# atakan-topaloglu/stable-virtual-camera

Hardware: AMD Instinct MI355X
Metric: denoising steps/sec, 1.3B Seva @ 21x576x576 views (higher is better)
Workload: dtype f16; 1 GPU; Seva 1.3B (1,263,968,004 params, random-init), one 21-view window per GPU, 576x576 px (latent 72x72), CFG batch 42, Euler-EDM step, MultiviewCFG(1.2) cfg 2.0; novel_views_per_sec = value x (T - 1 input view) / 50 steps per window; views=21, latent=72, windows=1

## Files before the change

include/seva_hip.h:

```cpp
#ifndef SEVA_HIP_H
#define SEVA_HIP_H

#include <stdint.h>

#ifdef __cplusplus
extern "C" {
#endif

typedef void* seva_stream_t;

#define SEVA_OK 0
#define SEVA_ERR_ARG (-1)
#define SEVA_ERR_LAUNCH (-2)
#define SEVA_ERR_UNSUPPORTED (-3)

const char* seva_last_error(void);
const char* seva_last_plan(void);
#define SEVA_ABI_VERSION 12
int seva_abi_version(void);
const char* seva_target_arch(void);

#define SEVA_CH_STATS_ROWS 64
#define SEVA_SPLITK_FLAGS 16384
#define SEVA_SPLITK_ERROR_SLOT 16383
#define SEVA_SPLITK_TILE_M 128
#define SEVA_SPLITK_TILE_N 160
#define SEVA_SPLITK_MAX_PIXELS 128
typedef struct seva_gemm_desc {
  const void* a;
  const void* w;
  const float* bias;
  const float* row_add;
  const float* residual;
  float* out_f32;
  void* out_f16;
  int64_t M, N, K;
  int64_t lda, ldr, ldo32, ldo16;
  int64_t rows_per_group;
  int64_t ld_row_add;
  int32_t mode;
  int32_t epilogue;
  int32_t n, ih, iw, cin, oh, ow, stride, upsample;
  float col_scale;
  int32_t col_scale_n;
  int32_t pad_br_only;
  const void* w_exp;
  void* out_f8;
  int64_t ldo8;
  float* ch_stats;
  float* splitk_ws;
  int64_t splitk_ws_bytes;
  const void* a2;
  int64_t lda2;
  int64_t K2;
  int64_t alg_K;
} seva_gemm_desc;
int seva_gemm_f16(const seva_gemm_desc* d, seva_stream_t stream);
int seva_gemm_f16_split_out(const seva_gemm_desc* d, seva_stream_t stream);
int seva_gemm_fp8(const seva_gemm_desc* d, seva_stream_t stream);

typedef struct seva_ff_desc {
  const void* a;
  const void* w1;
  const float* b1;
  const void* w2;
  const float* b2;
  const float* residual;
  float* out_f32;
  void* out_f16;
  int64_t M, lda, ldr, ldo32, ldo16;
  int32_t C;
  const float* ln_x;
  const float* ln_gamma;
  const float* ln_beta;
  int64_t ldx;
  float ln_eps;
  const void* w1_exp;
  const void* w2_exp;
} seva_ff_desc;
int seva_ff_fused_f16(const seva_ff_desc* d, seva_stream_t stream);
int seva_ff_fused_fp8(const seva_ff_desc* d, seva_stream_t stream);

#define SEVA_ATTN_LONG_MIN_LQ 2048
#define SEVA_ATTN_SPLIT_MIN_LK 6144
#define SEVA_ATTN_SPLIT_ROW_FLOATS 66
typedef struct seva_attn_desc {
  const void* q;
  const void* k;
  const void* v;
  void* out;
  int64_t q_sb0, q_sb1, q_sl;
  int64_t k_sb0, k_sb1, k_sl;
  int64_t o_sb0, o_sb1, o_sl;
  int32_t nb0, nb1;
  int32_t heads;
  int32_t lq, lk;
  float scale;
  int32_t q_prescaled;
  float* split_ws;
  int64_t split_ws_bytes;
} seva_attn_desc;
int seva_attention_f16(const seva_attn_desc* d, seva_stream_t stream);

int seva_attn_v_fp8_size(int32_t batch, int32_t heads, int32_t lk, int64_t* v8_bytes, int64_t* scale_bytes);
int seva_attn_quant_v_fp8(const seva_attn_desc* d, void* v8, uint8_t* v8_scale, seva_stream_t stream);
int seva_attention_pv8(const seva_attn_desc* d, const void* v8, const uint8_t* v8_scale, seva_stream_t stream);

#define SEVA_GN_WORKSPACE_SLABS 1024
typedef struct seva_groupnorm_desc {
  const float* x1;
  const float* x2;
  const float* gamma;
  const float* beta;
  const float* dense;
  const float* dense_w;
  const float* dense_b;
  void* out_f16;
  float* workspace;
  int32_t n, hw, c1, c2, groups, dense_c, silu;
  float eps;
  void* raw_f16;
  void* out_f8;
  int64_t ld_out_f8;
  const float* stats1;
  const float* stats2;
  int32_t split_out_f16;
  int32_t split_raw_f16;
} seva_groupnorm_desc;
int seva_groupnorm_f16(const seva_groupnorm_desc* d, seva_stream_t stream);

int seva_layernorm_f16(const float* x, const float* gamma, const float* beta, void* out_f16,
                       int64_t rows, int32_t c, float eps, seva_stream_t stream);
int seva_layernorm_f16_split(const float* x, const float* gamma, const float* beta, void* out_f16,
                             int64_t rows, int32_t c, float eps, seva_stream_t stream);
int seva_layernorm_fp8(const float* x, const float* gamma, const float* beta, void* out_f8, int64_t rows,
                       int32_t c, float eps, int64_t ld_out ,
                       seva_stream_t stream);

int seva_softmax_rows_f16(const float* x, int64_t ldx, void* out_f16, int64_t ldo, int64_t rows,
                          int32_t cols, int32_t cols_pad, float scale, seva_stream_t stream);

int seva_nchw_to_nhwc_f16(const float* x1, int32_t c1, const float* x2, int32_t c2,
                          const float* scale, void* out_f16, int32_t n, int32_t hw, int32_t cpad,
                          seva_stream_t stream);
int seva_nchw_to_nhwc_f16_split(const float* x1, int32_t c1, const float* x2, int32_t c2,
                                const float* scale, void* out_f16, int32_t n, int32_t hw, int32_t cpad,
                                seva_stream_t stream);
int seva_nhwc_to_nchw_f32(const float* x, int64_t ld, float* out, int32_t n, int32_t c,
                          int32_t hw, seva_stream_t stream);
int seva_cast_concat_f16(const float* x1, int32_t c1, const float* x2, int32_t c2, void* out_f16,
                         int64_t rows, seva_stream_t stream);
int seva_cast_concat_f16_split(const float* x1, int32_t c1, const float* x2, int32_t c2, void* out_f16,
                               int64_t rows, seva_stream_t stream);
int seva_bilinear_to_nhwc_f32(const float* src, float* out, int32_t n, int32_t c, int32_t sh,
                              int32_t sw, int32_t oh, int32_t ow, seva_stream_t stream);
int seva_timestep_embedding_f16(const int64_t* t, const float* freqs, void* out_f16, int32_t n,
                                int32_t dim, seva_stream_t stream);
int seva_silu_f16(const float* x, void* out_f16, int64_t count, seva_stream_t stream);
int seva_add_f32(const float* a, const float* b, float* out, int64_t count, seva_stream_t stream);

int seva_replace_blend_f32(const float* x, const float* replace, float* out, int32_t n, int32_t c,
                           int32_t hw, seva_stream_t stream);
int seva_denoiser_combine_f32(const float* net, const float* x, const float* c_out,
                              const float* c_skip, float* out, int32_t n, int64_t chw,
                              seva_stream_t stream);
int seva_add_noise_f32(const float* x, const float* eps, const float* noise_scale, float* out,
                       int32_t n, int64_t chw, seva_stream_t stream);
int seva_cfg_euler_f32(const float* x, const float* den2, const float* scale,
                       const float* sigma_hat, const float* dt, float* out, int32_t n, int64_t chw,
                       seva_stream_t stream);
int seva_cfg_multistep_f32(const float* x, const float* den, const float* scale, const float* old_den,
                           const float* a, const float* b, const float* c, float* out, float* den_out,
                           int32_t n, int64_t chw, seva_stream_t stream);

int seva_cfg_combine_f32(const float* den2, const float* scale, float* out, int32_t n, int64_t chw,
                         seva_stream_t stream);
int seva_euler_step_f32(const float* x, const float* den, const float* sigma_hat, const float* dt,
                        float* out, int32_t n, int64_t chw, seva_stream_t stream);
int seva_to_d_f32(const float* x, const float* den, const float* sigma, float* out, int32_t n,
                  int64_t chw, seva_stream_t stream);
int seva_scale_rows_f32(const float* x, const float* s, float* out, int32_t n, int64_t chw,
                        seva_stream_t stream);

int seva_plucker_f32(const float* kinv, const float* pose_inv, float* out, int32_t views, int32_t h,
                     int32_t w, seva_stream_t stream);
int seva_cond_concat_f32(const float* plucker, const uint8_t* mask, float* c_concat, float* uc_concat,
                         int32_t views, int32_t h, int32_t w, seva_stream_t stream);

int seva_layernorm_f32(const float* x, const float* gamma, const float* beta, float* out_f32, int64_t rows,
                       int32_t c, float eps, seva_stream_t stream);
int seva_clip_preprocess_f16(const float* x, void* patches_f16, int32_t n, int32_t H, int32_t W, int32_t out_size,
                             int32_t patch, int32_t ld_patches, const float* mean, const float* std,
                             int32_t antialias, seva_stream_t stream);
int seva_attention_small_f16(const void* q, const void* k, const void* v, void* out, int64_t q_sb, int64_t q_sl,
                             int64_t k_sb, int64_t k_sl, int64_t o_sb, int64_t o_sl, int32_t batch, int32_t heads,
                             int32_t L, int32_t head_dim, float scale, seva_stream_t stream);

typedef struct seva_image_desc {
  const void* src;
  const float* context_rgb;
  float* out;
  int64_t src_pitch_n;
  int64_t src_pitch_c;
  int64_t src_pitch_row;
  int64_t out_pitch_n;
  int32_t n, h, w, src_c;
  int32_t rh, rw;
  int32_t ct, cl;
  int32_t H, W;
  float pad_value, out_mul, out_add;
} seva_image_desc;
int seva_image_area_crop_u8(const seva_image_desc* d, seva_stream_t stream);
int seva_image_area_crop_f32(const seva_image_desc* d, seva_stream_t stream);
int seva_rgb_to_u8(const float* x, int64_t x_pitch_n, uint8_t* out, int32_t n, int32_t H, int32_t W,
                   seva_stream_t stream);

typedef struct seva_metrics_desc {
  const void* a;
  const void* b;
  int64_t* sse;
  double* ssim_sum;
  float* ssim_map;
  void* workspace;
  int64_t a_pitch_n;
  int64_t b_pitch_n;
  int64_t workspace_bytes;
  int32_t n, H, W;
  int32_t kind;
  int32_t ssim;
} seva_metrics_desc;
int seva_frame_metrics_size(int32_t n, int32_t H, int32_t W, int64_t* workspace_bytes);
int seva_frame_metrics(const seva_metrics_desc* d, seva_stream_t stream);

int seva_lpips_prepare_f16(const void* src, int64_t src_pitch_n, int32_t kind, void* out_f16, int32_t n, int32_t H,
                           int32_t W, seva_stream_t stream);
int seva_lpips_relu_pool_f16(const void* x, void* relu_out, void* pool_out, int32_t n, int32_t h, int32_t w, int32_t c,
                             seva_stream_t stream);
typedef struct seva_lpips_layer_desc {
  const void* fa;
  const void* fb;
  const float* w;
  double* out;
  void* workspace;
  int64_t a_pitch_n;
  int64_t b_pitch_n;
  int64_t workspace_bytes;
  int64_t hw;
  int32_t n, C;
} seva_lpips_layer_desc;
int seva_lpips_layer_size(int32_t n, int64_t hw, int64_t* workspace_bytes);
int seva_lpips_layer(const seva_lpips_layer_desc* d, seva_stream_t stream);

enum { SEVA_RANGE_F32 = 0, SEVA_RANGE_F16 = 1, SEVA_RANGE_E4M3 = 2 };
#define SEVA_RANGE_WORDS 72
#define SEVA_RANGE_WG_ELEMS 32768
#define SEVA_RANGE_MAX_WGS 2048
typedef struct seva_range_desc {
  const void* x;
  int32_t dtype;
  int64_t rows, cols, pitch;
  void* workspace;
  int64_t workspace_bytes;
  uint64_t* out;
} seva_range_desc;
int seva_tensor_range_size(int64_t rows, int64_t cols, int64_t* workspace_bytes);
int seva_tensor_range(const seva_range_desc* d, seva_stream_t stream);

int seva_set_knob(const char* name, int32_t value);
int seva_get_knob(const char* name, int32_t* value);

int seva_graph_begin(seva_stream_t stream);
int seva_graph_end(seva_stream_t stream, void** graph_exec_out);
int seva_graph_launch(void* graph_exec, seva_stream_t stream);
int seva_graph_destroy(void* graph_exec);

#define SEVA_PROF_CLASSES 5
int seva_prof_enable(int on);
int seva_prof_collect(double* ms, int64_t* launches, double* work, double* bytes);

#ifdef __cplusplus
}
#endif
#endif
```

stable-virtual-camera_amd/csrc/ff_fused.hip:

```cpp
#include "gemm_common.h"
#include "ff_fp8.h"

#include <atomic>

namespace {

struct FfArgs {
  const half_t* a;
  const half_t* w1;
  const float* b1;
  const half_t* w2;
  const float* b2;
  const float* residual;
  float* out_f32;
  half_t* out_f16;
  int64_t M, lda, ldr, ldo32, ldo16;
  int32_t tiles_m;
  const float* ln_x;
  const float* ln_gamma;
  const float* ln_beta;
  int64_t ldx;
  float ln_eps;
};

struct Ff8Args {
  FfArgs f;
  const uint8_t* w1_exp;
  const uint8_t* w2_exp;
};

static __device__ __forceinline__ void glds16_sv(const void* sbase, unsigned voff, unsigned lds_wave_base) {
  unsigned keep;
  asm volatile(
      "s_mov_b32 %0, m0\n\ts_mov_b32 m0, %3\n\ts_nop 0\n\tglobal_load_lds_dwordx4 %1, %2\n\ts_mov_b32 m0, %0"
      : "=&s"(keep)
      : "v"(voff), "s"(sbase), "s"(lds_wave_base)
      : "memory");
}


template <int C>
__global__ __launch_bounds__(512, 2) void ff_fused8_kernel(FfArgs p) {
  constexpr int KS = C / 32, NK1 = C / 64, NJ2 = C / 16, NJH = NJ2 / 2, NCH = C / 16;
  constexpr int W1_BYTES = 128 * 128, W2_BYTES = C * 128;
  constexpr int W2_PASSES = C / 64;
  constexpr int W2_PER_KT = (W2_PASSES + NK1 - 1) / NK1;
  static_assert(NJ2 % 2 == 0, "output blocks split over the two waves of a row group");

  extern __shared__ __attribute__((aligned(16))) char smem[];
  constexpr int W1_RING = 3;
  char* const lds_w1 = smem;
  char* const lds_w2 = smem + W1_RING * W1_BYTES;
  float* const lds_b1 = (float*)(smem + W1_RING * W1_BYTES + 2 * W2_BYTES);
  char* const lds_x = smem + W1_RING * W1_BYTES + 2 * W2_BYTES + 8 * C * 4;
  const unsigned lds_base_u32 = __builtin_amdgcn_readfirstlane(lds_addr_u32(smem));

  const int lane = threadIdx.x & 63;
  const int wave = __builtin_amdgcn_readfirstlane(threadIdx.x >> 6);
  const int mr = wave & 3, h = wave >> 2;
  const int fr = lane & 15, fg = lane >> 4;
  const int sr = lane >> 3, sp = lane & 7;

  const int tm = xcd_remap(blockIdx.x, p.tiles_m);
  const int64_t m0 = (int64_t)tm * 128 + mr * 32;

  half8_t areg[2][KS];
  if (p.ln_x) {
#pragma unroll
    for (int i = 0; i < 2; ++i) {
      int64_t m = m0 + 16 * i + fr;
      if (m >= p.M) m = p.M - 1;
      const float* xr = p.ln_x + m * p.ldx + 8 * fg;
      f32x4 v[KS][2];
#pragma unroll
      for (int ks = 0; ks < KS; ++ks) {
        v[ks][0] = first_read(*(const f32x4*)(xr + 32 * ks));
        v[ks][1] = first_read(*(const f32x4*)(xr + 32 * ks + 4));
      }
      float sum = 0.f;
#pragma unroll
      for (int ks = 0; ks < KS; ++ks)
#pragma unroll
        for (int e = 0; e < 2; ++e) sum += v[ks][e][0] + v[ks][e][1] + v[ks][e][2] + v[ks][e][3];
      sum += __shfl_xor(sum, 16, 64);
      asm volatile("" : "+v"(sum));
      sum += __shfl_xor(sum, 32, 64);
      asm volatile("" : "+v"(sum));
      const float mean = sum / (float)C;
      float ss = 0.f;
#pragma unroll
      for (int ks = 0; ks < KS; ++ks)
#pragma unroll
        for (int e = 0; e < 2; ++e)
#pragma unroll
          for (int r = 0; r < 4; ++r) {
            const float dlt = v[ks][e][r] - mean;
            ss += dlt * dlt;
          }
      ss += __shfl_xor(ss, 16, 64);
      asm volatile("" : "+v"(ss));
      ss += __shfl_xor(ss, 32, 64);
      asm volatile("" : "+v"(ss));
      const float rstd = rsqrtf(ss / (float)C + p.ln_eps);
#pragma unroll
      for (int ks = 0; ks < KS; ++ks) {
        half_t y[8];
#pragma unroll
        for (int e = 0; e < 2; ++e) {
          const f32x4 g4 = first_read(*(const f32x4*)(p.ln_gamma + 32 * ks + 8 * fg + 4 * e));
          const f32x4 b4 = first_read(*(const f32x4*)(p.ln_beta + 32 * ks + 8 * fg + 4 * e));
#pragma unroll
          for (int r = 0; r < 4; ++r) y[4 * e + r] = (half_t)((v[ks][e][r] - mean) * rstd * g4[r] + b4[r]);
        }
        areg[i][ks] = half8_t{y[0], y[1], y[2], y[3], y[4], y[5], y[6], y[7]};
      }
    }
  } else {
#pragma unroll
    for (int i = 0; i < 2; ++i) {
      int64_t m = m0 + 16 * i + fr;
      if (m >= p.M) m = p.M - 1;
      const half_t* ap = p.a + m * p.lda + 8 * fg;
#pragma unroll
      for (int ks = 0; ks < KS; ++ks) areg[i][ks] = *(const half8_t*)(ap + 32 * ks);
    }
  }
  f32x4 acc2[2][NJH];
#pragma unroll
  for (int i = 0; i < 2; ++i) {
    int64_t m = m0 + 16 * i + fr;
    if (m >= p.M) m = p.M - 1;
#pragma unroll
    for (int jj = 0; jj < NJH; ++jj)
      acc2[i][jj] = p.residual ? *(const f32x4*)(p.residual + m * p.ldr + 16 * (h * NJH + jj) + 4 * fg) : f32x4{0.f, 0.f, 0.f, 0.f};
  }
  for (int i = threadIdx.x; i < 2 * C; i += 512) *(f32x4*)(lds_b1 + 4 * i) = *(const f32x4*)(p.b1 + 4 * i);
#pragma unroll
  for (int i = 0; i < 2; ++i) {
#pragma unroll
    for (int ks = 0; ks < KS; ++ks) asm volatile("" : "+v"(areg[i][ks]));
#pragma unroll
    for (int jj = 0; jj < NJH; ++jj) asm volatile("" : "+v"(acc2[i][jj]));
  }

  auto w1_key = [](int row) { return ((row >> 1) & 1) | (((row >> 3) & 3) << 1); };
  const half_t* w1_src[2];
#pragma unroll
  for (int i = 0; i < 2; ++i) {
    const int row = wave * 16 + 8 * i + sr;
    w1_src[i] = p.w1 + (int64_t)row * C + (sp ^ w1_key(row)) * 8;
  }
  const half_t* w2_src[2];
#pragma unroll
  for (int i = 0; i < 2; ++i) {
    const int row = wave * (C / 8) + 8 * i + sr;
    w2_src[i] = p.w2 + (int64_t)row * (4 * C) + (sp ^ ((row >> 1) & 7)) * 8;
  }
  auto stage_w1 = [&](int buf, int hc, int kt) {
    const unsigned dst = lds_base_u32 + buf * W1_BYTES + wave * 16 * 128;
    const int64_t off = (int64_t)hc * 128 * C + kt * 64;
#pragma unroll
    for (int i = 0; i < 2; ++i) glds16_raw(w1_src[i] + off, dst + i * 1024);
  };
  auto stage_w2_part = [&](int buf, int hc, int part) {
    const unsigned dst = lds_base_u32 + W1_RING * W1_BYTES + buf * W2_BYTES + wave * (C / 8) * 128;
#pragma unroll
    for (int u = 0; u < W2_PER_KT; ++u) {
      const int i = part * W2_PER_KT + u;
      if (i < W2_PASSES) glds16_raw(w2_src[i & 1] + (int64_t)(i >> 1) * 16 * (4 * C) + hc * 64, dst + i * 1024);
    }
  };

  int w1_off[2], w2_off[2];
#pragma unroll
  for (int s = 0; s < 2; ++s) {
    const int rb = 64 * h + 8 * (fr >> 2) + (fr & 3);
    w1_off[s] = rb * 128 + (((4 * s + fg) ^ w1_key(rb)) << 4);
    const int r2 = 16 * (h * NJH) + fr;
    w2_off[s] = r2 * 128 + (((4 * s + fg) ^ ((r2 >> 1) & 7)) << 4);
  }
  char* const x_mine = lds_x + ((mr * 2 + h) * 2) * 1024 + lane * 16;
  const char* const x_q0 = lds_x + (mr * 2 * 2) * 1024 + lane * 16;

  constexpr int NTILES = NCH * NK1;
  auto stage_w1_seq = [&](int g) { stage_w1(g % W1_RING, g / NK1, g % NK1); };
  auto wait_all_but = [&](int n) {
    if (n >= 3) wait_vm<3>();
    else if (n == 2) wait_vm<2>();
    else if (n == 1) wait_vm<1>();
    else wait_vm<0>();
  };
  __syncthreads();
  stage_w1_seq(0);
#pragma unroll
  for (int part = 0; part < NK1; ++part) stage_w2_part(0, 0, part);
  if (NTILES > 1) stage_w1_seq(1);
  if (NTILES > 1) wait_vm<2>();
  else wait_vm<0>();
  lds_barrier();

  int g = 0;
  for (int hc = 0; hc < NCH; ++hc) {
    f32x4 acc1[2][4];
#pragma unroll
    for (int e = 0; e < 2; ++e) {
      const float* bp = lds_b1 + hc * 128 + 64 * h + 8 * fg + 4 * e;
      acc1[0][e] = acc1[1][e] = *(const f32x4*)bp;
      acc1[0][2 + e] = acc1[1][2 + e] = *(const f32x4*)(bp + 32);
    }
#pragma unroll
    for (int kt = 0; kt < NK1; ++kt) {
      int issued = 0;
      if (g + 2 < NTILES) {
        stage_w1_seq(g + 2);
        issued += 2;
      }
      if (hc + 1 < NCH && kt * W2_PER_KT < W2_PASSES) {
        stage_w2_part((hc + 1) & 1, hc + 1, kt);
        issued += (kt + 1) * W2_PER_KT <= W2_PASSES ? W2_PER_KT : W2_PASSES - kt * W2_PER_KT;
      }
      const char* const tb = lds_w1 + (g % W1_RING) * W1_BYTES;
      half8_t bfr[2][4];
#pragma unroll
      for (int s = 0; s < 2; ++s)
#pragma unroll
        for (int j = 0; j < 4; ++j) bfr[s][j] = *(const half8_t*)(tb + w1_off[s] + (32 * (j >> 1) + 4 * (j & 1)) * 128);
#pragma unroll
      for (int s = 0; s < 2; ++s)
#pragma unroll
        for (int i = 0; i < 2; ++i)
#pragma unroll
          for (int j = 0; j < 4; ++j)
            acc1[i][j] = __builtin_amdgcn_mfma_f32_16x16x32_f16(bfr[s][j], areg[i][2 * kt + s], acc1[i][j], 0, 0, 0);
      wait_all_but(issued);
      lds_barrier();
      ++g;
    }
#pragma unroll
    for (int i = 0; i < 2; ++i) {
      const f32x4 o0 = geglu4(acc1[i][0], acc1[i][2]);
      const f32x4 o1 = geglu4(acc1[i][1], acc1[i][3]);
      *(half8_t*)(x_mine + i * 1024) = half8_t{(half_t)o0[0], (half_t)o0[1], (half_t)o0[2], (half_t)o0[3],
                                               (half_t)o1[0], (half_t)o1[1], (half_t)o1[2], (half_t)o1[3]};
    }
    lds_barrier();
    half8_t hq[2][2];
#pragma unroll
    for (int q = 0; q < 2; ++q)
#pragma unroll
      for (int i = 0; i < 2; ++i) hq[q][i] = *(const half8_t*)(x_q0 + (q * 2 + i) * 1024);
    const char* const t2 = lds_w2 + (hc & 1) * W2_BYTES;
#pragma unroll
    for (int jj = 0; jj < NJH; ++jj) {
      const half8_t w0 = *(const half8_t*)(t2 + w2_off[0] + jj * (16 * 128));
      const half8_t w1f = *(const half8_t*)(t2 + w2_off[1] + jj * (16 * 128));
#pragma unroll
      for (int i = 0; i < 2; ++i) {
        acc2[i][jj] = __builtin_amdgcn_mfma_f32_16x16x32_f16(w0, hq[0][i], acc2[i][jj], 0, 0, 0);
        acc2[i][jj] = __builtin_amdgcn_mfma_f32_16x16x32_f16(w1f, hq[1][i], acc2[i][jj], 0, 0, 0);
      }
    }
    lds_barrier();
  }

#pragma unroll
  for (int i = 0; i < 2; ++i) {
    const int64_t m = m0 + 16 * i + fr;
    const bool ok = m < p.M;
#pragma unroll
    for (int jj = 0; jj < NJH; ++jj) {
      const int f = 16 * (h * NJH + jj) + 4 * fg;
      const f32x4 v = acc2[i][jj] + first_read(*(const f32x4*)(p.b2 + f));
      if (!ok) continue;
      if (p.out_f32) *(f32x4*)(p.out_f32 + m * p.ldo32 + f) = v;
      if (p.out_f16) *(half4_t*)(p.out_f16 + m * p.ldo16 + f) = to_f16x4(v);
    }
  }
}


template <int C>
__global__ __launch_bounds__(512, 2) void ff_fused8_fp8_kernel(Ff8Args q) {
  const FfArgs& p = q.f;
  constexpr int KP = FF8_KP(C), NK1 = KP / 128, NU = C / 64;
  constexpr int NJ2 = C / 16, NJH = NJ2 / 2, NCH = C / 16, NP = NCH / 2, NSC2 = (NJH + 3) / 4;
  constexpr int W1_BYTES = 128 * 128, W2_BYTES = C * 128;
  constexpr int W2_PASSES = C / 64;
  constexpr int W2_PER_KT = (W2_PASSES + 2 * NK1 - 1) / (2 * NK1);
  static_assert(NJ2 % 2 == 0 && NCH % 2 == 0, "output blocks split over two waves; chunks taken in pairs");
  static_assert(2 + W2_PER_KT <= 3, "wait_all_but counts at most 3 loads per K-tile");
  typedef int v4i_t __attribute__((ext_vector_type(4)));

  extern __shared__ __attribute__((aligned(16))) char smem[];
  constexpr int W1_RING = 3;
  char* const lds_w1 = smem;
  char* const lds_w2 = smem + W1_RING * W1_BYTES;
  float* const lds_b1 = (float*)(smem + W1_RING * W1_BYTES + 2 * W2_BYTES);
  int* const lds_s1 = (int*)(smem + W1_RING * W1_BYTES + 2 * W2_BYTES + 8 * C * 4);
  char* const lds_x = smem + W1_RING * W1_BYTES + 2 * W2_BYTES + 8 * C * 4 + NCH * 32 * 4;
  const unsigned lds_base_u32 = __builtin_amdgcn_readfirstlane(lds_addr_u32(smem));

  const int lane = threadIdx.x & 63;
  const int wave = __builtin_amdgcn_readfirstlane(threadIdx.x >> 6);
  const int mr = wave & 3, h = wave >> 2;
  const int fr = lane & 15, fg = lane >> 4;
  const int sr = lane >> 3, sp = lane & 7;

  const int tm = xcd_remap(blockIdx.x, p.tiles_m);
  const int64_t m0 = (int64_t)tm * 128 + mr * 32;

  half8_t areg[2][2 * NK1];
  if (p.ln_x) {
#pragma unroll
    for (int i = 0; i < 2; ++i) {
      int64_t m = m0 + 16 * i + fr;
      if (m >= p.M) m = p.M - 1;
      const float* xr = p.ln_x + m * p.ldx + 16 * fg;
      f32x4 v[NU][4];
#pragma unroll
      for (int u = 0; u < NU; ++u)
#pragma unroll
        for (int e = 0; e < 4; ++e) v[u][e] = first_read(*(const f32x4*)(xr + 64 * u + 4 * e));
      float sum = 0.f;
#pragma unroll
      for (int u = 0; u < NU; ++u)
#pragma unroll
        for (int e = 0; e < 4; ++e) sum += v[u][e][0] + v[u][e][1] + v[u][e][2] + v[u][e][3];
      sum += __shfl_xor(sum, 16, 64);
      asm volatile("" : "+v"(sum));
      sum += __shfl_xor(sum, 32, 64);
      asm volatile("" : "+v"(sum));
      const float mean = sum / (float)C;
      float ss = 0.f;
#pragma unroll
      for (int u = 0; u < NU; ++u)
#pragma unroll
        for (int e = 0; e < 4; ++e)
#pragma unroll
          for (int r = 0; r < 4; ++r) {
            const float dlt = v[u][e][r] - mean;
            ss += dlt * dlt;
          }
      ss += __shfl_xor(ss, 16, 64);
      asm volatile("" : "+v"(ss));
      ss += __shfl_xor(ss, 32, 64);
      asm volatile("" : "+v"(ss));
      const float rstd = rsqrtf(ss / (float)C + p.ln_eps);
#pragma unroll
      for (int u = 0; u < 2 * NK1; ++u) {
        if (u >= NU) {
          areg[i][u] = half8_t{};
          continue;
        }
        v4i_t w;
#pragma unroll
        for (int e = 0; e < 4; ++e) {
          const f32x4 g4 = first_read(*(const f32x4*)(p.ln_gamma + 64 * u + 16 * fg + 4 * e));
          const f32x4 b4 = first_read(*(const f32x4*)(p.ln_beta + 64 * u + 16 * fg + 4 * e));
          float y[4];
#pragma unroll
          for (int r = 0; r < 4; ++r) y[r] = (v[u][e][r] - mean) * rstd * g4[r] + b4[r];
          w[e] = pack_fp8x4(y[0], y[1], y[2], y[3]);
        }
        areg[i][u] = __builtin_bit_cast(half8_t, w);
      }
    }
  } else {
#pragma unroll
    for (int i = 0; i < 2; ++i) {
      int64_t m = m0 + 16 * i + fr;
      if (m >= p.M) m = p.M - 1;
      const uint8_t* ap = (const uint8_t*)p.a + m * p.lda + 16 * fg;
#pragma unroll
      for (int u = 0; u < 2 * NK1; ++u) areg[i][u] = u < NU ? *(const half8_t*)(ap + 64 * u) : half8_t{};
    }
  }
  f32x4 acc2[2][NJH];
#pragma unroll
  for (int i = 0; i < 2; ++i)
#pragma unroll
    for (int jj = 0; jj < NJH; ++jj) acc2[i][jj] = f32x4{0.f, 0.f, 0.f, 0.f};
  for (int i = threadIdx.x; i < 2 * C; i += 512) *(f32x4*)(lds_b1 + 4 * i) = *(const f32x4*)(p.b1 + 4 * i);
  for (int idx = threadIdx.x; idx < NCH * 32; idx += 512) {
    const int hc = idx >> 5, hh = (idx >> 4) & 1, f = idx & 15;
    const int rb = hc * 128 + 64 * hh + 8 * (f >> 2) + (f & 3);
    lds_s1[idx] = (int)q.w1_exp[rb] | ((int)q.w1_exp[rb + 4] << 8) | ((int)q.w1_exp[rb + 32] << 16) | ((int)q.w1_exp[rb + 36] << 24);
  }
  int wsc2[NSC2];
#pragma unroll
  for (int w = 0; w < NSC2; ++w) wsc2[w] = 0;
#pragma unroll
  for (int jj = 0; jj < NJH; ++jj) wsc2[jj >> 2] |= (int)q.w2_exp[16 * (h * NJH + jj) + fr] << (8 * (jj & 3));
#pragma unroll
  for (int i = 0; i < 2; ++i) {
#pragma unroll
    for (int u = 0; u < NU; ++u) asm volatile("" : "+v"(areg[i][u]));
#pragma unroll
    for (int jj = 0; jj < NJH; ++jj) asm volatile("" : "+v"(acc2[i][jj]));
  }
#pragma unroll
  for (int w = 0; w < NSC2; ++w) asm volatile("" : "+v"(wsc2[w]));

  auto w1_key = [](int row) { return ((row >> 1) & 1) | (((row >> 3) & 3) << 1); };
  unsigned w1_voff[2];
#pragma unroll
  for (int i = 0; i < 2; ++i) {
    const int row = wave * 16 + 8 * i + sr;
    w1_voff[i] = (unsigned)(row * KP + (sp ^ w1_key(row)) * 16);
  }
  unsigned w2_voff[2];
#pragma unroll
  for (int i = 0; i < 2; ++i) {
    const int row = wave * (C / 8) + 8 * i + sr;
    w2_voff[i] = (unsigned)(row * (4 * C) + (sp ^ ((row >> 1) & 7)) * 16);
  }
  auto stage_w1 = [&](int buf, int hc, int kt) {
    const unsigned dst = lds_base_u32 + buf * W1_BYTES + wave * 16 * 128;
    const uint8_t* const base = (const uint8_t*)p.w1 + (int64_t)hc * 128 * KP + kt * 128;
#pragma unroll
    for (int i = 0; i < 2; ++i) glds16_sv(base, w1_voff[i], dst + i * 1024);
  };
  auto stage_w2_part = [&](int buf, int pp, int part) {
    const unsigned dst = lds_base_u32 + W1_RING * W1_BYTES + buf * W2_BYTES + wave * (C / 8) * 128;
#pragma unroll
    for (int u = 0; u < W2_PER_KT; ++u) {
      const int i = part * W2_PER_KT + u;
      if (i < W2_PASSES)
        glds16_sv((const uint8_t*)p.w2 + (int64_t)(i >> 1) * 16 * (4 * C) + pp * 128, w2_voff[i & 1], dst + i * 1024);
    }
  };

  int w1_off[2], w2_off[2];
#pragma unroll
  for (int s = 0; s < 2; ++s) {
    const int rb = 64 * h + 8 * (fr >> 2) + (fr & 3);
    w1_off[s] = rb * 128 + (((4 * s + fg) ^ w1_key(rb)) << 4);
    const int r2 = 16 * (h * NJH) + fr;
    w2_off[s] = r2 * 128 + (((4 * s + fg) ^ ((r2 >> 1) & 7)) << 4);
  }
  char* const x_mine = lds_x + ((mr * 2 + h) * 2) * 1024 + lane * 16;
  const char* const x_q0 = lds_x + (mr * 2 * 2) * 1024 + lane * 16;

  constexpr int NTILES = NCH * NK1;
  auto stage_w1_seq = [&](int g) { stage_w1(g % W1_RING, g / NK1, g % NK1); };
  auto wait_all_but = [&](int n) {
    if (n >= 3) wait_vm<3>();
    else if (n == 2) wait_vm<2>();
    else if (n == 1) wait_vm<1>();
    else wait_vm<0>();
  };
  __syncthreads();
  stage_w1_seq(0);
#pragma unroll
  for (int part = 0; part < 2 * NK1; ++part) stage_w2_part(0, 0, part);
  stage_w1_seq(1);
  wait_vm<2>();
  lds_barrier();

  int g = 0;
  for (int pp = 0; pp < NP; ++pp) {
    v4i_t hx[2];
#pragma unroll
    for (int c = 0; c < 2; ++c) {
      const int hc = 2 * pp + c;
      f32x4 acc1[2][4];
#pragma unroll
      for (int i = 0; i < 2; ++i)
#pragma unroll
        for (int j = 0; j < 4; ++j) acc1[i][j] = f32x4{0.f, 0.f, 0.f, 0.f};
      const int sc1 = lds_s1[hc * 32 + h * 16 + fr];
#pragma unroll
      for (int kt = 0; kt < NK1; ++kt) {
        int issued = 0;
        if (g + 2 < NTILES) {
          stage_w1_seq(g + 2);
          issued += 2;
        }
        const int kk = c * NK1 + kt;
        if (pp + 1 < NP && kk * W2_PER_KT < W2_PASSES) {
          stage_w2_part((pp + 1) & 1, pp + 1, kk);
          issued += (kk + 1) * W2_PER_KT <= W2_PASSES ? W2_PER_KT : W2_PASSES - kk * W2_PER_KT;
        }
        const char* const tb = lds_w1 + (g % W1_RING) * W1_BYTES;
#pragma unroll
        for (int jp = 0; jp < 2; ++jp) {
          half8_t bfr[2][2];
#pragma unroll
          for (int s = 0; s < 2; ++s)
#pragma unroll
            for (int e = 0; e < 2; ++e) bfr[s][e] = *(const half8_t*)(tb + w1_off[s] + (32 * jp + 4 * e) * 128);
#pragma unroll
          for (int i = 0; i < 2; ++i)
#pragma unroll
            for (int e = 0; e < 2; ++e)
              acc1[i][2 * jp + e] = mfma_f8(2 * jp + e, bfr[0][e], bfr[1][e], areg[i][2 * kt], areg[i][2 * kt + 1], acc1[i][2 * jp + e], sc1);
          if (jp == 0) __builtin_amdgcn_sched_barrier(0);
        }
#pragma unroll
        for (int i = 0; i < 2; ++i)
#pragma unroll
          for (int j = 0; j < 4; ++j) asm volatile("" : "+v"(acc1[i][j]));
        wait_all_but(issued);
        lds_barrier();
        ++g;
      }
      f32x4 bias[4];
#pragma unroll
      for (int e = 0; e < 2; ++e) {
        const float* bp = lds_b1 + hc * 128 + 64 * h + 8 * fg + 4 * e;
        bias[e] = first_read(*(const f32x4*)bp);
        bias[2 + e] = first_read(*(const f32x4*)(bp + 32));
      }
#pragma unroll
      for (int i = 0; i < 2; ++i) {
        const f32x4 o0 = geglu4(acc1[i][0] + bias[0], acc1[i][2] + bias[2]);
        const f32x4 o1 = geglu4(acc1[i][1] + bias[1], acc1[i][3] + bias[3]);
        hx[i][2 * c] = pack_fp8x4(o0[0], o0[1], o0[2], o0[3]);
        hx[i][2 * c + 1] = pack_fp8x4(o1[0], o1[1], o1[2], o1[3]);
      }
    }
#pragma unroll
    for (int i = 0; i < 2; ++i) *(v4i_t*)(x_mine + i * 1024) = hx[i];
    lds_barrier();
    half8_t hq[2][2];
#pragma unroll
    for (int qq = 0; qq < 2; ++qq)
#pragma unroll
      for (int i = 0; i < 2; ++i) hq[qq][i] = *(const half8_t*)(x_q0 + (qq * 2 + i) * 1024);
    const char* const t2 = lds_w2 + (pp & 1) * W2_BYTES;
#pragma unroll
    for (int jj = 0; jj < NJH; ++jj) {
      const half8_t w0 = *(const half8_t*)(t2 + w2_off[0] + jj * (16 * 128));
      const half8_t w1f = *(const half8_t*)(t2 + w2_off[1] + jj * (16 * 128));
#pragma unroll
      for (int i = 0; i < 2; ++i) acc2[i][jj] = mfma_f8(jj, w0, w1f, hq[0][i], hq[1][i], acc2[i][jj], wsc2[jj >> 2]);
    }
#pragma unroll
    for (int i = 0; i < 2; ++i)
#pragma unroll
      for (int jj = 0; jj < NJH; ++jj) asm volatile("" : "+v"(acc2[i][jj]));
    lds_barrier();
  }

#pragma unroll
  for (int i = 0; i < 2; ++i) {
    const int64_t m = m0 + 16 * i + fr;
    const bool ok = m < p.M;
#pragma unroll
    for (int jj = 0; jj < NJH; ++jj) {
      const int f = 16 * (h * NJH + jj) + 4 * fg;
      if (!ok) continue;
      f32x4 v = acc2[i][jj] + first_read(*(const f32x4*)(p.b2 + f));
      if (p.residual) v += first_read(*(const f32x4*)(p.residual + m * p.ldr + f));
      if (p.out_f32) *(f32x4*)(p.out_f32 + m * p.ldo32 + f) = v;
      if (p.out_f16) *(half4_t*)(p.out_f16 + m * p.ldo16 + f) = to_f16x4(v);
    }
  }
}

template <bool FP8>
int validate_ff(const seva_ff_desc* d, const char* pre) {
  SEVA_REQUIRE(d != nullptr, "%s: null desc", pre);
  SEVA_REQUIRE(d->C == 64 || d->C == 128 || d->C == 256 || d->C == 320, "%s: C=%d unsupported (64, 128, 256, 320)", pre, d->C);
  if constexpr (FP8) {
    SEVA_REQUIRE(d->a || d->ln_x, "%s: neither a nor ln_x given", pre);
    SEVA_REQUIRE(d->w1 && d->b1 && d->w2 && d->b2, "%s: null operand", pre);
    SEVA_REQUIRE(d->w1_exp && d->w2_exp, "%s: w1_exp and w2_exp (per-row E8M0 scale bytes) are required", pre);
  } else {
    SEVA_REQUIRE((d->a || d->ln_x) && d->w1 && d->b1 && d->w2 && d->b2, "%s: null operand", pre);
  }
  SEVA_REQUIRE(!d->ln_x || (d->ln_gamma && d->ln_beta && d->ldx >= d->C && d->ldx % 4 == 0 &&
                            ((uintptr_t)d->ln_x | (uintptr_t)d->ln_gamma | (uintptr_t)d->ln_beta) % 16 == 0),
               "%s: LayerNorm prologue needs gamma, beta, a row pitch >= C (multiple of 4), 16-byte aligned pointers", pre);
  SEVA_REQUIRE(d->out_f32 || d->out_f16, "%s: no output", pre);
  SEVA_REQUIRE(d->M > 0, "%s: empty problem", pre);
  if constexpr (FP8) {
    SEVA_REQUIRE(d->ln_x || (d->lda >= d->C && d->lda % 16 == 0), "%s: lda=%lld invalid (bytes, >= C, multiple of 16)", pre, (long long)d->lda);
  } else {
    SEVA_REQUIRE(d->ln_x || (d->lda >= d->C && d->lda % 8 == 0), "%s: lda=%lld invalid", pre, (long long)d->lda);
  }
  SEVA_REQUIRE((!d->residual || d->ldr % 4 == 0) && (!d->out_f32 || d->ldo32 % 4 == 0) && (!d->out_f16 || d->ldo16 % 4 == 0),
               "%s: row pitches must be multiples of 4", pre);
  SEVA_REQUIRE(((uintptr_t)(FP8 && d->ln_x ? nullptr : d->a) | (uintptr_t)d->w1 | (uintptr_t)d->b1 | (uintptr_t)d->w2 | (uintptr_t)d->b2 |
                (uintptr_t)d->residual | (uintptr_t)d->out_f32 | (uintptr_t)d->out_f16) % 16 == 0,
               "%s: pointers must be 16-byte aligned", pre);
  SEVA_REQUIRE((d->M + 127) / 128 <= 0x7fffffff, "%s: too many rows", pre);
  return 0;
}

FfArgs ff_args(const seva_ff_desc* d) {
  FfArgs a{};
  a.a = (const half_t*)d->a; a.w1 = (const half_t*)d->w1; a.b1 = d->b1; a.w2 = (const half_t*)d->w2; a.b2 = d->b2;
  a.residual = d->residual; a.out_f32 = d->out_f32; a.out_f16 = (half_t*)d->out_f16;
  a.M = d->M; a.lda = d->lda; a.ldr = d->ldr; a.ldo32 = d->ldo32; a.ldo16 = d->ldo16;
  a.ln_x = d->ln_x; a.ln_gamma = d->ln_gamma; a.ln_beta = d->ln_beta; a.ldx = d->ldx; a.ln_eps = d->ln_eps;
  a.tiles_m = (int)((d->M + 127) / 128);
  return a;
}

struct FfWork { double flops, bytes; };
FfWork ff_work(const seva_ff_desc* d, double a_bytes, double w_bytes) {
  const double C = (double)d->C, M = (double)d->M;
  return {2.0 * M * C * (8.0 * C) + 2.0 * M * (4.0 * C) * C,
          M * C * ((d->ln_x ? 4.0 : a_bytes) + (d->residual ? 4.0 : 0.0) + (d->out_f32 ? 4.0 : 0.0) + (d->out_f16 ? 2.0 : 0.0)) + w_bytes};
}

template <class Args>
int ff_launch(void (*kernel)(Args), const char* name, int lds, std::atomic<uint64_t>& attr_devs, const Args& a, int tiles_m, hipStream_t s) {
  seva_max_dynamic_lds_once(attr_devs, lds, {(const void*)kernel});
  hipLaunchKernelGGL(kernel, dim3((unsigned)tiles_m), dim3(512), lds, s, a);
  return seva_check_launch(name);
}
template <int C>
int ff_launch8(const FfArgs& a, hipStream_t s) {
  static std::atomic<uint64_t> attr_devs{0};
  return ff_launch(ff_fused8_kernel<C>, "ff_fused8_kernel", 3 * 128 * 128 + 2 * C * 128 + 8 * C * 4 + 16 * 1024, attr_devs, a, a.tiles_m, s);
}
template <int C>
int ff_launch8_fp8(const Ff8Args& a, hipStream_t s) {
  constexpr int lds = 3 * 128 * 128 + 2 * C * 128 + 8 * C * 4 + (C / 16) * 32 * 4 + 16 * 1024;
  static_assert(lds <= 160 * 1024, "LDS budget of one workgroup per CU");
  static std::atomic<uint64_t> attr_devs{0};
  return ff_launch(ff_fused8_fp8_kernel<C>, "ff_fused8_fp8_kernel", lds, attr_devs, a, a.f.tiles_m, s);
}

}

extern "C" int seva_ff_fused_f16(const seva_ff_desc* d, seva_stream_t stream) {
  if (const int rc = validate_ff<false>(d, "ff_fused")) return rc;
  const FfArgs a = ff_args(d);
  hipStream_t s = (hipStream_t)stream;
  const double C = (double)d->C;
  const FfWork w = ff_work(d, 2.0, 2.0 * (8.0 * C * C + 4.0 * C * C));
  SevaProfScope prof(0, w.flops, s, w.bytes);
  switch (d->C) {
    case 64: return ff_launch8<64>(a, s);
    case 128: return ff_launch8<128>(a, s);
    case 256: return ff_launch8<256>(a, s);
    default: return ff_launch8<320>(a, s);
  }
}

extern "C" int seva_ff_fused_fp8(const seva_ff_desc* d, seva_stream_t stream) {
  if (const int rc = validate_ff<true>(d, "ff_fused_fp8")) return rc;
  Ff8Args a{ff_args(d), (const uint8_t*)d->w1_exp, (const uint8_t*)d->w2_exp};
  hipStream_t s = (hipStream_t)stream;
  const double C = (double)d->C;
  const FfWork w = ff_work(d, 1.0, 8.0 * C * FF8_KP(d->C) + 4.0 * C * C);
  SevaProfScope prof(0, w.flops, s, w.bytes);
  switch (d->C) {
    case 64: return ff_launch8_fp8<64>(a, s);
    case 128: return ff_launch8_fp8<128>(a, s);
    case 256: return ff_launch8_fp8<256>(a, s);
    default: return ff_launch8_fp8<320>(a, s);
  }
}
```

stable-virtual-camera_amd/csrc/norm.hip:

```cpp
#include "seva_common.h"

#include <stdlib.h>

namespace {

constexpr int GN_THREADS = 256;
constexpr int GN_MAX_THREADS = 1024;
constexpr int GN_MAX_SLABS = SEVA_GN_WORKSPACE_SLABS;
constexpr int GN_BASE_SLABS = 64;
constexpr int GN_MAX_GROUPS = 32;
constexpr int GN_MAX_DENSE = 8;

struct GnArgs {
  const float* x1;
  const float* x2;
  const float* gamma;
  const float* beta;
  const float* dense;
  const float* dense_w;
  const float* dense_b;
  half_t* out;
  uint8_t* out8;
  int64_t ld8;
  half_t* raw_out;
  int32_t split_out, split_raw;
  float* ws;
  const float* stats1;
  const float* stats2;
  int32_t n, hw, c1, c2, groups, dense_c, silu;
  int32_t nslab_stats;
  int32_t qpb;
  int64_t final_off;
  float eps;
};

struct GnMap {
  int cq, tpp, pl_count, pl, q0, qstep;
  bool active;
  __device__ GnMap(int C) {
    const int nthreads = blockDim.x;
    cq = C >> 2;
    tpp = cq < nthreads ? cq : nthreads;
    pl_count = nthreads / tpp;
    const int t = threadIdx.x;
    pl = t / tpp;
    q0 = t - pl * tpp;
    qstep = tpp;
    active = pl < pl_count;
  }
};

__device__ __forceinline__ f32x4 load_quad(const GnArgs& p, int n, int pix, int c) {
  if (c < p.c1) return *(const f32x4*)(p.x1 + ((int64_t)n * p.hw + pix) * p.c1 + c);
  return *(const f32x4*)(p.x2 + ((int64_t)n * p.hw + pix) * p.c2 + (c - p.c1));
}

__global__ __launch_bounds__(GN_MAX_THREADS) void gn_stats_kernel(GnArgs p) {
  extern __shared__ __attribute__((aligned(16))) float lds[];
  const int C = p.c1 + p.c2;
  const GnMap mp(C);
  const int n = blockIdx.y, slab = blockIdx.x, nslab = gridDim.x;
  const int p_begin = (int)((int64_t)slab * p.hw / nslab);
  const int p_end = (int)((int64_t)(slab + 1) * p.hw / nslab);
  float* const lsum = lds;
  float* const lsq = lds + mp.pl_count * C;
  if (mp.active) {
    for (int q = mp.q0; q < mp.cq; q += mp.qstep) {
      f32x4 s = {0.f, 0.f, 0.f, 0.f}, ss = {0.f, 0.f, 0.f, 0.f};
      for (int pix = p_begin + mp.pl; pix < p_end; pix += mp.pl_count) {
        const f32x4 v = first_read(load_quad(p, n, pix, q * 4));
        s += v;
        ss += v * v;
      }
      *(f32x4*)(lsum + mp.pl * C + q * 4) = s;
      *(f32x4*)(lsq + mp.pl * C + q * 4) = ss;
    }
  }
  __syncthreads();
  const int g = threadIdx.x;
  if (g < p.groups) {
    const int cpg = C / p.groups;
    float s = 0.f, ss = 0.f;
    for (int pl = 0; pl < mp.pl_count; ++pl)
      for (int c = g * cpg; c < (g + 1) * cpg; ++c) {
        s += first_read(lsum[pl * C + c]);
        ss += first_read(lsq[pl * C + c]);
      }
    float* o = p.ws + (((int64_t)n * nslab + slab) * p.groups + g) * 2;
    o[0] = s;
    o[1] = ss;
  }
}

__global__ void gn_finalize_kernel(GnArgs p) {
  const int n = blockIdx.x, g = blockIdx.y, l = threadIdx.x;
  const int C = p.c1 + p.c2, cpg = C / p.groups;
  double s = 0.0, ss = 0.0;
  for (int sl = l; sl < p.nslab_stats; sl += 64) {
    const float* o = p.ws + (((int64_t)n * p.nslab_stats + sl) * p.groups + g) * 2;
    s += (double)o[0];
    ss += (double)o[1];
  }
#pragma unroll
  for (int off = 32; off > 0; off >>= 1) {
    s += __shfl_xor(s, off, 64);
    ss += __shfl_xor(ss, off, 64);
  }
  if (l != 0) return;
  const double cnt = (double)cpg * (double)p.hw;
  const double mean = s / cnt;
  double var = ss / cnt - mean * mean;
  if (var < 0.0) var = 0.0;
  float* f = p.ws + p.final_off + ((int64_t)n * p.groups + g) * 2;
  f[0] = (float)mean;
  f[1] = (float)(1.0 / sqrt(var + (double)p.eps));
}

__global__ __launch_bounds__(256) void gn_finalize_ch_kernel(GnArgs p) {
  __shared__ double red[4][2];
  const int n = blockIdx.x, g = blockIdx.y, t = threadIdx.x;
  const int C = p.c1 + p.c2, cpg = C / p.groups;
  static_assert(SEVA_CH_STATS_ROWS == 64, "row blocks of the producers' statistics");
  const int nb = p.hw >> 6;
  const int64_t rb0 = (int64_t)n * nb;
  const int total = cpg * nb;
  double s = 0.0, ss = 0.0;
  for (int idx = t; idx < total; idx += 256) {
    const int b = idx / cpg, c = g * cpg + (idx - b * cpg);
    const bool first = c < p.c1;
    const int cs = first ? p.c1 : p.c2, cl = first ? c : c - p.c1;
    const float* o = (first ? p.stats1 : p.stats2) + (rb0 + b) * 2 * cs + cl;
    s += (double)o[0];
    ss += (double)o[cs];
  }
#pragma unroll
  for (int off = 32; off > 0; off >>= 1) {
    s += __shfl_xor(s, off, 64);
    ss += __shfl_xor(ss, off, 64);
  }
  if ((t & 63) == 0) {
    red[t >> 6][0] = s;
    red[t >> 6][1] = ss;
  }
  __syncthreads();
  if (t != 0) return;
  s = ((red[0][0] + red[1][0]) + red[2][0]) + red[3][0];
  ss = ((red[0][1] + red[1][1]) + red[2][1]) + red[3][1];
  const double cnt = (double)cpg * (double)p.hw;
  const double mean = s / cnt;
  double var = ss / cnt - mean * mean;
  if (var < 0.0) var = 0.0;
  float* f = p.ws + p.final_off + ((int64_t)n * p.groups + g) * 2;
  f[0] = (float)mean;
  f[1] = (float)(1.0 / sqrt(var + (double)p.eps));
}

template <bool DENSE, bool DC6 = false, bool SPLIT = false>
__global__ __launch_bounds__(GN_THREADS) void gn_apply_kernel(GnArgs p) {
  constexpr int ND = DC6 ? 6 : GN_MAX_DENSE;
  __shared__ float g_mean[GN_MAX_GROUPS], g_rstd[GN_MAX_GROUPS];
  const int C = p.c1 + p.c2;
  const int n = blockIdx.y, slab = blockIdx.x, nslab = gridDim.x;
  const int cpg = C / p.groups;
  const int cq = C >> 2;
  int pl, pl_count, q;
  bool active;
  if (gridDim.z == 1) {
    pl_count = blockDim.x / cq;
    pl = threadIdx.x / cq;
    q = threadIdx.x - pl * cq;
    active = pl < pl_count;
  } else {
    pl_count = 1;
    pl = 0;
    q = blockIdx.z * p.qpb + threadIdx.x;
    active = (int)threadIdx.x < p.qpb && q < cq;
  }
  if ((int)threadIdx.x < p.groups) {
    const float* f = p.ws + p.final_off + ((int64_t)n * p.groups + threadIdx.x) * 2;
    g_mean[threadIdx.x] = f[0];
    g_rstd[threadIdx.x] = f[1];
  }
  __syncthreads();
  if (!active) return;
  const int p_begin = (int)((int64_t)slab * p.hw / nslab);
  const int p_end = (int)((int64_t)(slab + 1) * p.hw / nslab);
  const int dc = DENSE ? (DC6 ? 6 : p.dense_c) : 0;
  {
    const int c0 = q * 4;
    float a[4], b[4];
    f32x2 wmod[4][ND], bmod[4];
#pragma unroll
    for (int r = 0; r < 4; ++r) {
      const int c = c0 + r, g = c / cpg;
      a[r] = first_read(g_rstd[g]) * first_read(p.gamma[c]);
      b[r] = first_read(p.beta[c]) - first_read(g_mean[g]) * a[r];
      bmod[r] = f32x2{1.0f + (dc ? first_read(p.dense_b[c]) : 0.f), dc ? first_read(p.dense_b[C + c]) : 0.f};
#pragma unroll
      for (int j = 0; j < ND; ++j) wmod[r][j] = f32x2{0.f, 0.f};
    }
    if (DENSE && DC6) {
      f32x4 ws4[6], wh4[6];
#pragma unroll
      for (int t = 0; t < 6; ++t) {
        ws4[t] = first_read(*(const f32x4*)(p.dense_w + (int64_t)c0 * 6 + 4 * t));
        wh4[t] = first_read(*(const f32x4*)(p.dense_w + (int64_t)(C + c0) * 6 + 4 * t));
      }
#pragma unroll
      for (int r = 0; r < 4; ++r)
#pragma unroll
        for (int j = 0; j < 6; ++j) {
          const int e = 6 * r + j;
          wmod[r][j] = f32x2{ws4[e >> 2][e & 3], wh4[e >> 2][e & 3]};
        }
    } else if (DENSE) {
#pragma unroll
      for (int r = 0; r < 4; ++r)
#pragma unroll
        for (int j = 0; j < ND; ++j) {
          const int c = c0 + r;
          const int jj = j < dc ? j : (dc > 0 ? dc - 1 : 0);
          const float w0 = p.dense_w[(int64_t)c * dc + jj];
          const float w1 = p.dense_w[(int64_t)(C + c) * dc + jj];
          wmod[r][j] = f32x2{j < dc ? w0 : 0.f, j < dc ? w1 : 0.f};
        }
    }
    constexpr int U = DENSE ? 3 : 2;
    for (int pix0 = p_begin + pl; pix0 < p_end; pix0 += U * pl_count) {
      f32x4 v[U];
      float dn[U][ND];
#pragma unroll
      for (int u = 0; u < U; ++u) {
        int pix = pix0 + u * pl_count;
        if (pix >= p_end) pix = p_end - 1;
        v[u] = load_quad(p, n, pix, c0);
        if (dc) {
          const float* dp = p.dense + ((int64_t)n * p.hw + pix) * dc;
#pragma unroll
          for (int j = 0; j < ND; ++j) dn[u][j] = (j < dc) ? dp[j] : 0.f;
        }
      }
      f32x2 dn2[U][ND];
      if (dc) {
#pragma unroll
        for (int u = 0; u < U; ++u)
#pragma unroll
          for (int j = 0; j < ND; ++j) {
            dn2[u][j] = f32x2{dn[u][j], dn[u][j]};
            asm volatile("" : "+v"(dn2[u][j]));
          }
      }
#pragma unroll
      for (int u = 0; u < U; ++u) {
        const int pix = pix0 + u * pl_count;
        half4_t h;
        float y4[4];
#pragma unroll
        for (int r = 0; r < 4; ++r) {
          float y = v[u][r] * a[r] + b[r];
          if (p.silu) y = silu_f(y);
          if (dc) {
            f32x2 m = bmod[r];
#pragma unroll
            for (int j = 0; j < ND; ++j) m = __builtin_elementwise_fma(wmod[r][j], dn2[u][j], m);
            y = y * m[0] + m[1];
          }
          h[r] = (half_t)y;
          y4[r] = y;
        }
        if (pix < p_end) {
          const int64_t ldo = (SPLIT && p.split_out) ? 2 * C : C, ldr = (SPLIT && p.split_raw) ? 2 * C : C;
          if (p.out) {
            *(half4_t*)(p.out + ((int64_t)n * p.hw + pix) * ldo + c0) = h;
            if (SPLIT && p.split_out) {
              *(half4_t*)(p.out + ((int64_t)n * p.hw + pix) * ldo + C + c0) = lo_f16x4(f32x4{y4[0], y4[1], y4[2], y4[3]}, h);
            }
          }
          if (p.out8) *(int*)(p.out8 + ((int64_t)n * p.hw + pix) * p.ld8 + c0) = pack_fp8x4(y4[0], y4[1], y4[2], y4[3]);
          if (p.raw_out) {
            const half4_t hr = to_f16x4(v[u]);
            *(half4_t*)(p.raw_out + ((int64_t)n * p.hw + pix) * ldr + c0) = hr;
            if (SPLIT && p.split_raw) *(half4_t*)(p.raw_out + ((int64_t)n * p.hw + pix) * ldr + C + c0) = lo_f16x4(v[u], hr);
          }
        }
      }
    }
  }
}

constexpr int LN_MAXV = 20;

__device__ __forceinline__ float group16_sum(float v) {
#pragma unroll
  for (int o = 8; o > 0; o >>= 1) v += __shfl_xor(v, o, 64);
  return v;
}

template <int NV, int LN_ROWS, int OUT = 0, bool SPLIT = false>
__global__ __launch_bounds__(256) void layernorm_kernel(const float* __restrict__ x,
                                                        const float* __restrict__ gamma,
                                                        const float* __restrict__ beta,
                                                        half_t* __restrict__ out, int64_t rows,
                                                        int c, float eps, int64_t ld_out) {
  const int sub = threadIdx.x & 15;
  const int cq = c >> 2;
  const int64_t base = (int64_t)blockIdx.x * (16 * LN_ROWS) + (threadIdx.x >> 4);
  constexpr bool HOIST = NV <= 10;
  f32x4 gm[HOIST ? NV : 1], bt[HOIST ? NV : 1];
  if (HOIST) {
#pragma unroll
    for (int k = 0; k < NV; ++k) {
      const int i = sub + 16 * k < cq ? sub + 16 * k : cq - 1;
      gm[HOIST ? k : 0] = first_read(*(const f32x4*)(gamma + i * 4));
      bt[HOIST ? k : 0] = first_read(*(const f32x4*)(beta + i * 4));
    }
  }
  auto load_row = [&](int64_t row, f32x4 (&v)[NV]) {
    if (row >= rows) row = rows - 1;
    const float* xr = x + row * c;
#pragma unroll
    for (int k = 0; k < NV; ++k) {
      const int i = sub + 16 * k < cq ? sub + 16 * k : cq - 1;
      v[k] = *(const f32x4*)(xr + i * 4);
    }
  };
  f32x4 v[NV], nxt[NV];
  load_row(base, v);
#pragma unroll
  for (int it = 0; it < LN_ROWS; ++it) {
    const int64_t row = base + 16 * it;
    if (it + 1 < LN_ROWS) load_row(row + 16, nxt);
    float s = 0.f;
#pragma unroll
    for (int k = 0; k < NV; ++k)
      if (sub + 16 * k < cq) s += v[k][0] + v[k][1] + v[k][2] + v[k][3];
    const float mean = group16_sum(s) / (float)c;
    float ss = 0.f;
#pragma unroll
    for (int k = 0; k < NV; ++k)
      if (sub + 16 * k < cq) {
#pragma unroll
        for (int r = 0; r < 4; ++r) {
          const float d = v[k][r] - mean;
          ss += d * d;
        }
      }
    const float rstd = rsqrtf(group16_sum(ss) / (float)c + eps);
    if (row < rows) {
      half_t* orow = out + row * ld_out;
#pragma unroll
      for (int k = 0; k < NV; ++k) {
        const int i = sub + 16 * k;
        if (i < cq) {
          const f32x4 g4 = HOIST ? gm[HOIST ? k : 0] : first_read(*(const f32x4*)(gamma + i * 4));
          const f32x4 b4 = HOIST ? bt[HOIST ? k : 0] : first_read(*(const f32x4*)(beta + i * 4));
          if constexpr (OUT != 0) {
            float y[4];
#pragma unroll
            for (int r = 0; r < 4; ++r) y[r] = (v[k][r] - mean) * rstd * g4[r] + b4[r];
            if constexpr (OUT == 1) *(int*)((uint8_t*)out + row * ld_out + i * 4) = pack_fp8x4(y[0], y[1], y[2], y[3]);
            else *(f32x4*)((float*)out + row * ld_out + i * 4) = f32x4{y[0], y[1], y[2], y[3]};
          } else {
            half4_t h, l;
#pragma unroll
            for (int r = 0; r < 4; ++r) {
              const float y = (v[k][r] - mean) * rstd * g4[r] + b4[r];
              h[r] = (half_t)y;
              if constexpr (SPLIT) l[r] = (half_t)(y - (float)h[r]);
            }
            *(half4_t*)(orow + i * 4) = h;
            if constexpr (SPLIT) *(half4_t*)(orow + c + i * 4) = l;
          }
        }
      }
    }
    if (it + 1 < LN_ROWS) {
#pragma unroll
      for (int k = 0; k < NV; ++k) v[k] = nxt[k];
    }
  }
}

__global__ __launch_bounds__(256) void softmax_rows_kernel(const float* __restrict__ x, int64_t ldx,
                                                           half_t* __restrict__ out, int64_t ldo,
                                                           int cols, int cols_pad, float scale_log2) {
  __shared__ float red[4];
  const float* xr = x + (int64_t)blockIdx.x * ldx;
  half_t* orow = out + (int64_t)blockIdx.x * ldo;
  const int lane = threadIdx.x & 63, wave = threadIdx.x >> 6;
  float mx = -1e30f;
  for (int c = threadIdx.x; c < cols; c += 256) mx = fmaxf(mx, first_read(xr[c]) * scale_log2);
  mx = wave_max(mx);
  if (lane == 0) red[wave] = mx;
  __syncthreads();
  mx = fmaxf(fmaxf(red[0], red[1]), fmaxf(red[2], red[3]));
  __syncthreads();
  float s = 0.f;
  for (int c = threadIdx.x; c < cols; c += 256) s += __builtin_amdgcn_exp2f(first_read(xr[c]) * scale_log2 - mx);
  s = wave_sum(s);
  if (lane == 0) red[wave] = s;
  __syncthreads();
  const float inv = 1.0f / (red[0] + red[1] + red[2] + red[3]);
  for (int c = threadIdx.x; c < cols_pad; c += 256)
    orow[c] = (half_t)(c < cols ? __builtin_amdgcn_exp2f(first_read(xr[c]) * scale_log2 - mx) * inv : 0.f);
}

int clampi(int v, int lo, int hi) { return v < lo ? lo : (v > hi ? hi : v); }

}

extern "C" int seva_groupnorm_f16(const seva_groupnorm_desc* d, seva_stream_t stream) {
  SEVA_REQUIRE(d != nullptr, "groupnorm: null desc");
  SEVA_REQUIRE(d->x1 && d->gamma && d->beta && (d->out_f16 || d->out_f8) && d->workspace, "groupnorm: null pointer");
  SEVA_REQUIRE(d->n > 0 && d->hw > 0 && d->c1 > 0 && d->c2 >= 0, "groupnorm: bad shape");
  SEVA_REQUIRE(d->c2 == 0 || d->x2 != nullptr, "groupnorm: c2 > 0 needs x2");
  const int C = d->c1 + d->c2;
  SEVA_REQUIRE(d->c1 % 4 == 0 && d->c2 % 4 == 0, "groupnorm: c1=%d c2=%d must be multiples of 4", d->c1, d->c2);
  SEVA_REQUIRE(d->groups > 0 && d->groups <= GN_MAX_GROUPS && C % d->groups == 0,
               "groupnorm: %d channels / %d groups unsupported", C, d->groups);
  SEVA_REQUIRE(!d->dense || (d->dense_c > 0 && d->dense_c <= GN_MAX_DENSE && d->dense_w && d->dense_b),
               "groupnorm: bad dense modulation args (dense_c=%d)", d->dense_c);
  SEVA_REQUIRE(C <= 4 * GN_MAX_THREADS, "groupnorm: C=%d too large", C);
  GnArgs a{};
  a.x1 = d->x1; a.x2 = d->x2; a.gamma = d->gamma; a.beta = d->beta;
  a.dense = d->dense; a.dense_w = d->dense_w; a.dense_b = d->dense_b;
  a.out = (half_t*)d->out_f16; a.out8 = (uint8_t*)d->out_f8; a.raw_out = (half_t*)d->raw_f16; a.ws = d->workspace;
  a.ld8 = d->ld_out_f8 > 0 ? d->ld_out_f8 : C;
  SEVA_REQUIRE(a.ld8 >= C && a.ld8 % 4 == 0, "groupnorm: ld_out_f8=%lld invalid", (long long)a.ld8);
  a.n = d->n; a.hw = d->hw; a.c1 = d->c1; a.c2 = d->c2; a.groups = d->groups;
  a.dense_c = d->dense_c; a.silu = d->silu; a.eps = d->eps;
  a.stats1 = d->stats1; a.stats2 = d->stats2;
  a.split_out = d->split_out_f16 != 0; a.split_raw = d->split_raw_f16 != 0;
  SEVA_REQUIRE((!a.split_out || d->out_f16) && (!a.split_raw || d->raw_f16), "groupnorm: split_* needs the output it splits");
  SEVA_REQUIRE(!d->stats2 || d->stats1, "groupnorm: stats2 without stats1");
  if (d->stats1) {
    SEVA_REQUIRE(d->hw % SEVA_CH_STATS_ROWS == 0, "groupnorm: producer statistics need hw %% 64 == 0 (hw=%d)", d->hw);
    SEVA_REQUIRE(d->c2 == 0 || d->stats2, "groupnorm: statistics must be given for BOTH sources (or none)");
  }
  const int cq = C / 4;
  const int nthreads = cq <= GN_THREADS ? GN_THREADS : (cq >= GN_MAX_THREADS ? GN_MAX_THREADS : 64 * ((cq + 63) / 64));
  const int tpp = cq < nthreads ? cq : nthreads;
  const int plc = nthreads / tpp;
  const int slab_cap = clampi(d->hw / 128, GN_BASE_SLABS - 1, GN_MAX_SLABS - 1);
  a.nslab_stats = clampi(d->hw / (plc * 16), 1, slab_cap);
  a.final_off = (int64_t)d->n * (GN_MAX_SLABS - 1) * d->groups * 2;
  const int plc_apply = cq <= GN_THREADS ? GN_THREADS / cq : 1;
  const int zchunks = cq <= GN_THREADS ? 1 : (cq + GN_THREADS - 1) / GN_THREADS;
  a.qpb = (cq + zchunks - 1) / zchunks;
  int apply_threads = zchunks == 1 ? plc_apply * cq : a.qpb;
  if (apply_threads < 64) apply_threads = 64;
  int min_iter = d->dense ? 24 : 4;
  if (g_seva_knobs.gn_min_iter > 0) min_iter = g_seva_knobs.gn_min_iter;
  const int nslab_apply = clampi(8192 / (d->n * zchunks), 1, clampi(d->hw / (min_iter * plc_apply), 1, 1024));
  hipStream_t s = (hipStream_t)stream;
  const double bytes = (double)d->n * d->hw * C * ((d->stats1 ? 0.0 : 4.0) + 4.0 + 2.0);
  SevaProfScope prof(3, bytes, s);
  const size_t lds = (size_t)plc * C * 2 * sizeof(float);
  int rc;
  if (a.stats1) {
    hipLaunchKernelGGL(gn_finalize_ch_kernel, dim3(d->n, d->groups), dim3(256), 0, s, a);
    rc = seva_check_launch("gn_finalize_ch_kernel");
    if (rc) return rc;
  } else {
    hipLaunchKernelGGL(gn_stats_kernel, dim3(a.nslab_stats, d->n), dim3(nthreads), lds, s, a);
    rc = seva_check_launch("gn_stats_kernel");
    if (rc) return rc;
    hipLaunchKernelGGL(gn_finalize_kernel, dim3(d->n, d->groups), dim3(64), 0, s, a);
    rc = seva_check_launch("gn_finalize_kernel");
    if (rc) return rc;
  }
  const bool split = a.split_out || a.split_raw;
  if (split && d->dense && d->dense_c == 6)
    hipLaunchKernelGGL((gn_apply_kernel<true, true, true>), dim3(nslab_apply, d->n, zchunks), dim3(apply_threads), 0, s, a);
  else if (split && !d->dense)
    hipLaunchKernelGGL((gn_apply_kernel<false, false, true>), dim3(nslab_apply, d->n, zchunks), dim3(apply_threads), 0, s, a);
  else if (split) {
    seva_set_error("groupnorm: split-precision outputs with a %d-component modulation are not instantiated", d->dense_c);
    return SEVA_ERR_ARG;
  } else if (d->dense && d->dense_c == 6)
    hipLaunchKernelGGL((gn_apply_kernel<true, true>), dim3(nslab_apply, d->n, zchunks), dim3(apply_threads), 0, s, a);
  else if (d->dense)
    hipLaunchKernelGGL(gn_apply_kernel<true>, dim3(nslab_apply, d->n, zchunks), dim3(apply_threads), 0, s, a);
  else
    hipLaunchKernelGGL(gn_apply_kernel<false>, dim3(nslab_apply, d->n, zchunks), dim3(apply_threads), 0, s, a);
  return seva_check_launch("gn_apply_kernel");
}

namespace {
template <int OUT, bool SPLIT = false>
int layernorm_entry(const float* x, const float* gamma, const float* beta, void* out, int64_t rows, int32_t c, float eps,
                    seva_stream_t stream, int64_t ld_out = 0) {
  SEVA_REQUIRE(x && gamma && beta && out, "layernorm: null pointer");
  if (ld_out <= 0) ld_out = SPLIT ? 2 * (int64_t)c : c;
  SEVA_REQUIRE(ld_out >= c && ld_out % 4 == 0, "layernorm: output row pitch %lld invalid", (long long)ld_out);
  SEVA_REQUIRE(rows > 0 && c > 0 && c % 4 == 0 && c <= 16 * 4 * LN_MAXV,
               "layernorm: rows=%lld c=%d unsupported", (long long)rows, c);
  hipStream_t s = (hipStream_t)stream;
  SevaProfScope prof(3, (double)rows * c * (OUT == 1 ? 5.0 : OUT == 2 || SPLIT ? 8.0 : 6.0), s);
  const int lr = rows >= 64 * 1024 ? 4 : 1;
  const int64_t blocks = (rows + 16 * lr - 1) / (16 * lr);
  SEVA_REQUIRE(blocks <= 0x7fffffff, "layernorm: too many rows");
  const int nv = (c / 4 + 15) / 16;
#define SEVA_LN_LAUNCH(NV)                                                                                  \
  do {                                                                                                      \
    if (lr == 4)                                                                                            \
      hipLaunchKernelGGL((layernorm_kernel<NV, 4, OUT, SPLIT>), dim3((unsigned)blocks), dim3(256), 0, s, x, gamma,  \
                         beta, (half_t*)out, rows, c, eps, ld_out);                                         \
    else                                                                                                    \
      hipLaunchKernelGGL((layernorm_kernel<NV, 1, OUT, SPLIT>), dim3((unsigned)blocks), dim3(256), 0, s, x, gamma,  \
                         beta, (half_t*)out, rows, c, eps, ld_out);                                         \
  } while (0)
  if (nv <= 2) SEVA_LN_LAUNCH(2);
  else if (nv <= 5) SEVA_LN_LAUNCH(5);
  else if (nv <= 10) SEVA_LN_LAUNCH(10);
  else SEVA_LN_LAUNCH(20);
#undef SEVA_LN_LAUNCH
  return seva_check_launch("layernorm_kernel");
}
}

extern "C" int seva_layernorm_f16(const float* x, const float* gamma, const float* beta,
                                  void* out_f16, int64_t rows, int32_t c, float eps,
                                  seva_stream_t stream) {
  return layernorm_entry<0>(x, gamma, beta, out_f16, rows, c, eps, stream);
}

extern "C" int seva_layernorm_f16_split(const float* x, const float* gamma, const float* beta,
                                        void* out_f16, int64_t rows, int32_t c, float eps,
                                        seva_stream_t stream) {
  return layernorm_entry<0, true>(x, gamma, beta, out_f16, rows, c, eps, stream);
}

extern "C" int seva_layernorm_fp8(const float* x, const float* gamma, const float* beta,
                                  void* out_f8, int64_t rows, int32_t c, float eps, int64_t ld_out,
                                  seva_stream_t stream) {
  return layernorm_entry<1>(x, gamma, beta, out_f8, rows, c, eps, stream, ld_out);
}

extern "C" int seva_layernorm_f32(const float* x, const float* gamma, const float* beta,
                                  float* out_f32, int64_t rows, int32_t c, float eps,
                                  seva_stream_t stream) {
  return layernorm_entry<2>(x, gamma, beta, out_f32, rows, c, eps, stream);
}

extern "C" int seva_softmax_rows_f16(const float* x, int64_t ldx, void* out_f16, int64_t ldo,
                                     int64_t rows, int32_t cols, int32_t cols_pad, float scale,
                                     seva_stream_t stream) {
  SEVA_REQUIRE(x && out_f16 && rows > 0 && cols > 0 && cols_pad >= cols && ldx >= cols && ldo >= cols_pad,
               "softmax_rows: bad args");
  SEVA_REQUIRE(rows <= 0x7fffffff, "softmax_rows: too many rows");
  hipStream_t s = (hipStream_t)stream;
  SevaProfScope prof(3, (double)rows * cols * 6.0, s);
  hipLaunchKernelGGL(softmax_rows_kernel, dim3((unsigned)rows), dim3(256), 0, s, x, ldx,
                     (half_t*)out_f16, ldo, cols, cols_pad, scale * 1.44269504088896340736f);
  return seva_check_launch("softmax_rows_kernel");
}
```

stable-virtual-camera_amd/seva/_engine.py:

```python

from __future__ import annotations

import math
import os

import torch

from . import _native, audit, ops
from ._arch import Layout
from ._native import SevaNativeError, require_cuda
from .ops import audit_mark
from .ops import SPLITK_ERROR_SLOT, SPLITK_MAX_PIXELS, splitk_tiles, splitk_workspace_numel

F16, F32, U8 = torch.float16, torch.float32, torch.uint8
QK_SCALE_LOG2E = 0.125 * 1.4426950408889634
CIN_PAD = 64


def _pad128(k: int) -> int:
    return 128 * ((k + 127) // 128)


def pack_conv3x3(w: torch.Tensor, cin_pad: int | None = None) -> torch.Tensor:
    cout, cin = w.shape[:2]
    cin_pad = cin_pad or cin
    out = torch.zeros((cout, 3, 3, cin_pad), dtype=F16, device=w.device)
    out[..., :cin] = w.permute(0, 2, 3, 1).to(F16)
    return out.reshape(cout, 9 * cin_pad).contiguous()


def combine_up_phases(w: torch.Tensor, dtype: torch.dtype = F16) -> torch.Tensor:
    fold = ((0,), (1, 2)), ((0, 1), (2,))
    w64 = w.double()
    cout, cin = w.shape[:2]
    out = torch.empty((4, cout, 2, 2, cin), dtype=dtype, device=w.device)
    for py in range(2):
        for px in range(2):
            for a in range(2):
                for b in range(2):
                    out[2 * py + px, :, a, b] = w64[:, :, list(fold[py][a])][:, :, :, list(fold[px][b])].sum((2, 3)).to(dtype)
    return out.reshape(4, cout, 4 * cin).contiguous()


def interleave_geglu(w: torch.Tensor, b: torch.Tensor):
    nh = w.shape[0] // 2
    g = nh // 32
    wi = torch.stack([w[:nh].reshape(g, 32, -1), w[nh:].reshape(g, 32, -1)], 1).reshape(2 * nh, -1)
    bi = torch.stack([b[:nh].reshape(g, 32), b[nh:].reshape(g, 32)], 1).reshape(2 * nh)
    return wi.contiguous(), bi.contiguous()


SPLIT_TOKENS = ("stem", "head", "skip", "skip_deep", "conv", "resample", "proj_in", "proj_out", "qkv", "ff")
SPLIT_ALL = frozenset(t for t in SPLIT_TOKENS if t != "skip_deep")
SPLIT_DEFAULT = "stem,head,skip_deep"


def parse_split(spec, strict: bool = False) -> set:
    toks = [t.strip() for t in (spec.split(",") if isinstance(spec, str) else list(spec))]
    toks = [t for t in toks if t]
    if strict:
        bad = [t for t in toks if t not in SPLIT_TOKENS + ("all", "none")]
        if bad:
            raise ValueError(f"unknown split-precision token(s) {bad} (any of {', '.join(SPLIT_TOKENS)}, or all / none)")
    out = set(toks)
    if "all" in out:
        out = (out - {"all"}) | SPLIT_ALL
    return out


def dup_k(w: torch.Tensor) -> torch.Tensor:
    return torch.cat([w, w], 1).contiguous()


class _Arena:

    def __init__(self, device):
        self.device = device
        self.bufs: dict = {}
        audit.register_arena(self)

    def get(self, name: str, shape, dtype, zero: bool = False) -> torch.Tensor:
        key = (name, tuple(int(s) for s in shape), dtype)
        t = self.bufs.get(key)
        if t is None:
            t = self.bufs[key] = (torch.zeros if zero else torch.empty)(key[1], dtype=dtype, device=self.device)
        return t

    def nbytes(self) -> int:
        return sum(t.numel() * t.element_size() for t in self.bufs.values())


def env_flag(name: str, rule: str, default: bool = False) -> bool:
    v = os.environ.get(name)
    return default if v is None else (v != "0" if rule == "not0" else v == "1")


def env_int(name: str, default: int) -> int:
    return int(os.environ.get(name, default))


class _EngineBase:

    NEEDS_GPU = ""

    @staticmethod
    def _resolve_device(module):
        params = list(module.parameters())
        if not params or params[0].device.type != "cuda":
            return None
        _native.load()
        return params[0].device

    def __init__(self, module, group_norms: bool = True):
        self.device = self._resolve_device(module)
        if self.device is None:
            raise SevaNativeError(self.NEEDS_GPU)
        self.arena = _Arena(self.device)
        if group_norms:
            self.gn_fused_stats = env_int("SEVA_GN_FUSED_STATS", 1)
            self._stats: dict = {}

    def _buf(self, name, shape, dtype, zero=False):
        return self.arena.get(name, shape, dtype, zero)

    def _stats_buf(self, name, rows, hw, c):
        if not self.gn_fused_stats or hw % ops.STATS_ROWS or c < 128 or c % 4:
            return None
        if self.gn_fused_stats < 2 and (hw // 128) * ((c + 159) // 160) < 16:
            return None
        return self._buf("st:" + name, ops.channel_stats_shape(rows, c), F32)

    def _produced(self, out, st):
        if st is None:
            self._stats.pop(out.data_ptr(), None)
        else:
            self._stats[out.data_ptr()] = st

    def _gn_stats(self, x1, x2=None):
        s1 = self._stats.get(x1.data_ptr())
        s2 = None if x2 is None else self._stats.get(x2.data_ptr())
        if s1 is None or (x2 is not None and s2 is None):
            return None, None
        return s1, s2


class SevaEngine(_EngineBase):
    NEEDS_GPU = "Seva.forward runs only on an AMD GPU: move the module to a cuda device first (there is no CPU fallback)."
    split: frozenset = frozenset()
    _resolve_device = staticmethod(_EngineBase._resolve_device)

    def __init__(self, model, precision: str | None = None, attention: str | None = None, ff: str | None = None, split=None):
        super().__init__(model)
        self.precision = precision or os.environ.get("SEVA_PRECISION", "f16")
        if self.precision not in ("f16", "fp8"):
            raise ValueError(f"unknown precision {self.precision!r} (f16 | fp8)")
        self.fp8 = self.precision == "fp8"
        self.attention = self._fp8_option("attention", attention, "SEVA_FP8_ATTENTION")
        self.pv8 = self.attention == "fp8"
        self.fp8_pad = env_flag("SEVA_FP8_PAD", "is1")
        self.ff_fused = env_flag("SEVA_FF_FUSED", "not0", True)
        self.ff = self._fp8_option("ff", ff, "SEVA_FP8_FF")
        self.ff8 = self.ff == "fp8"
        self.conv_splitk = env_flag("SEVA_CONV_SPLITK", "not0", True)
        self.attn_split = env_flag("SEVA_ATTN_SPLIT_KV", "not0", True)
        self.attn_split_max = max(2, min(4, env_int("SEVA_ATTN_SPLIT", 2)))
        self.fold_skip = env_flag("SEVA_FOLD_SKIP", "not0") and not self.fp8
        if split is not None:
            if self.fp8:
                raise ValueError('split precision needs precision "f16" (the fp8 mode has no split operands)')
            self.split = parse_split(split, strict=True)
        else:
            self.split = parse_split(os.environ.get("SEVA_SPLIT_PRECISION", SPLIT_DEFAULT)) if not self.fp8 else set()
        self.p = model.params
        self.layout: Layout = model._layout
        self._pack(model)
        self.use_graph = env_flag("SEVA_HIPGRAPH", "not0", True)
        self._graphs: dict = {}
        self.slice_frames = env_int("SEVA_SLICE_FRAMES", 0)
        self.slice_min_bytes = int(float(os.environ.get("SEVA_SLICE_MIN_MB", "96")) * (1 << 20))
        self.slice_attn = env_flag("SEVA_SLICE_ATTN", "is1")

    def _fp8_option(self, name: str, value, switch: str) -> str:
        if value is None:
            value = "fp8" if self.fp8 and env_flag(switch, "is1") else "f16"
        if value not in ("f16", "fp8"):
            raise ValueError(f"unknown {name} {value!r} (f16 | fp8)")
        if value == "fp8" and not self.fp8:
            raise ValueError(f'{name}="fp8" needs precision "fp8" (the f16 parity mode stays pure)')
        return value

    def _ff_fused_fp8(self, c: int) -> bool:
        return self.ff8 and self.ff_fused and c in ops.FF_FUSED_CHANNELS and c % 128 != 0

    def _split_skip(self, cout: int) -> bool:
        return "skip" in self.split or ("skip_deep" in self.split and cout >= 2 * self.p.model_channels)

    def _pack(self, model) -> None:
        sd = {k: v.detach() for k, v in model.state_dict().items()}
        dev = self.device
        W: dict[str, torch.Tensor] = {}

        def f16(k):
            return sd[k].to(device=dev, dtype=F16).contiguous()

        def f32(k):
            return sd[k].to(device=dev, dtype=F32).contiguous()

        mc = self.p.model_channels
        half = mc // 2
        W["freqs"] = torch.exp(
            -math.log(10000) * torch.arange(start=0, end=half, dtype=torch.float32) / half
        ).to(dev)
        for k in ("time_embed.0", "time_embed.2"):
            W[k + ".w"], W[k + ".b"] = f16(k + ".weight"), f32(k + ".bias")

        emb_w, emb_b, ctx_w, ctx_b = [], [], [], []
        self.emb_off: dict[str, int] = {}
        self.ctx_off: dict[str, int] = {}
        emb_total = ctx_total = 0

        def q8(name, w):
            if not (self.fp8 and w.shape[0] % 16 == 0 and w.shape[0] > 32):
                return
            k = w.shape[1]
            kp = _pad128(k)
            if kp != k and (not self.fp8_pad or kp * 4 > k * 5):
                return
            if kp != k:
                w = torch.cat([w, w.new_zeros((w.shape[0], kp - k))], 1)
            W[name + "8"], W[name + "8e"] = ops.quantize_weight_fp8(w)

        sp = self.split

        def pack_attn_self(pfx):
            def qkv(conv):
                return torch.cat([conv(pfx + ".to_q.weight"), conv(pfx + ".to_k.weight"), conv(pfx + ".to_v.weight")], 0)

            W[pfx + ".qkv"] = dup_k(qkv(f16)) if "qkv" in sp else qkv(f16)
            if self.fp8:
                q8(pfx + ".qkv", qkv(f32))
            W[pfx + ".out.w"], W[pfx + ".out.b"] = f16(pfx + ".to_out.0.weight"), f32(pfx + ".to_out.0.bias")

        def pack_attn_cross(pfx):
            nonlocal ctx_total
            wv, wo, bo = f32(pfx + ".to_v.weight"), f32(pfx + ".to_out.0.weight"), f32(pfx + ".to_out.0.bias")
            ctx_w.append((wo.double() @ wv.double()).to(F16))
            ctx_b.append(bo)
            self.ctx_off[pfx] = ctx_total
            ctx_total += wo.shape[0]
            W[pfx + ".q"] = f16(pfx + ".to_q.weight")
            W[pfx + ".kv"] = torch.cat([f16(pfx + ".to_k.weight"), f16(pfx + ".to_v.weight")], 0).contiguous()
            W[pfx + ".out.w"], W[pfx + ".out.b"] = f16(pfx + ".to_out.0.weight"), bo

        def pack_ff(pfx):
            b1 = f32(pfx + ".net.0.proj.bias")
            wi, bi = interleave_geglu(f16(pfx + ".net.0.proj.weight"), b1)
            W[pfx + ".w1"], W[pfx + ".b1"] = wi, bi
            W[pfx + ".w2"], W[pfx + ".b2"] = f16(pfx + ".net.2.weight"), f32(pfx + ".net.2.bias")
            if "ff" in sp:
                W[pfx + ".w1"], W[pfx + ".w2"] = dup_k(W[pfx + ".w1"]), dup_k(W[pfx + ".w2"])
            if not self.fp8:
                return
            wi32 = interleave_geglu(f32(pfx + ".net.0.proj.weight"), b1)[0]
            if self._ff_fused_fp8(wi.shape[1]):
                W[pfx + ".w1f8"], W[pfx + ".w1f8e"], W[pfx + ".w2f8"], W[pfx + ".w2f8e"] = ops.pack_ff_fp8(wi32, f32(pfx + ".net.2.weight"))
            else:
                q8(pfx + ".w1", wi32)
                if pfx + ".w18" in W:
                    q8(pfx + ".w2", f32(pfx + ".net.2.weight"))

        def pack_ln(pfx):
            W[pfx + ".g"], W[pfx + ".b"] = f32(pfx + ".weight"), f32(pfx + ".bias")

        for spec in self.layout.all_specs():
            pfx = spec.prefix
            if spec.kind == "conv":
                wc = f32(pfx + ".weight")
                if "stem" in self.split and 2 * spec.cin <= CIN_PAD:
                    wc = dup_k(wc)
                W[pfx + ".w"] = pack_conv3x3(wc, CIN_PAD * ((wc.shape[1] + CIN_PAD - 1) // CIN_PAD))
                W[pfx + ".b"] = f32(pfx + ".bias")
            elif spec.kind == "res":
                assert spec.cin % 64 == 0 and spec.cout % 64 == 0, "channel counts must be multiples of 64"
                pack_ln(pfx + ".in_layers.0")
                pack_ln(pfx + ".out_layers.0")
                wc1, wc2 = f32(pfx + ".in_layers.2.weight"), f32(pfx + ".out_layers.3.weight")
                W[pfx + ".conv1.w"] = pack_conv3x3(dup_k(wc1) if "conv" in sp else wc1)
                W[pfx + ".conv1.b"] = f32(pfx + ".in_layers.2.bias")
                W[pfx + ".conv2.w"] = pack_conv3x3(dup_k(wc2) if "conv" in sp else wc2)
                W[pfx + ".conv2.b"] = f32(pfx + ".out_layers.3.bias")
                if self.fp8:
                    for tag, wc, ch in (("conv1", wc1, spec.cin), ("conv2", wc2, spec.cout)):
                        cp = _pad128(ch)
                        if cp == ch or (self.fp8_pad and cp * 4 <= ch * 5):
                            q8(f"{pfx}.{tag}.w", pack_conv3x3(wc, cp).float())
                W[pfx + ".dense.w"] = f32(pfx + ".dense_emb_layers.0.weight").reshape(2 * spec.cin, -1).contiguous()
                W[pfx + ".dense.b"] = f32(pfx + ".dense_emb_layers.0.bias")
                emb_w.append(f16(pfx + ".emb_layers.1.weight"))
                emb_b.append(f32(pfx + ".emb_layers.1.bias"))
                self.emb_off[pfx] = emb_total
                emb_total += spec.cout
                if spec.cin != spec.cout:
                    ws = f16(pfx + ".skip_connection.weight").reshape(spec.cout, spec.cin)
                    W[pfx + ".skip.w"] = dup_k(ws) if self._split_skip(spec.cout) else ws.contiguous()
                    W[pfx + ".skip.b"] = f32(pfx + ".skip_connection.bias")
                    if self.fold_skip:
                        W[pfx + ".conv2.wf"] = torch.cat([W[pfx + ".conv2.w"], W[pfx + ".skip.w"]], 1).contiguous()
                        W[pfx + ".conv2.bf"] = (W[pfx + ".conv2.b"] + W[pfx + ".skip.b"]).contiguous()
            elif spec.kind == "mvt":
                pack_ln(pfx + ".norm")
                W[pfx + ".proj_in.w"], W[pfx + ".proj_in.b"] = f16(pfx + ".proj_in.weight"), f32(pfx + ".proj_in.bias")
                W[pfx + ".proj_out.w"], W[pfx + ".proj_out.b"] = f16(pfx + ".proj_out.weight"), f32(pfx + ".proj_out.bias")
                if "proj_in" in sp:
                    W[pfx + ".proj_in.w"] = dup_k(W[pfx + ".proj_in.w"])
                if "proj_out" in sp:
                    W[pfx + ".proj_out.w"] = dup_k(W[pfx + ".proj_out.w"])
                for i in range(spec.depth):
                    b = f"{pfx}.transformer_blocks.{i}"
                    pack_attn_self(b + ".attn1")
                    pack_attn_cross(b + ".attn2")
                    pack_ff(b + ".ff")
                    for n in ("norm1", "norm2", "norm3"):
                        pack_ln(f"{b}.{n}")
                    m = f"{pfx}.time_mix_blocks.{i}"
                    pack_attn_self(m + ".attn1")
                    pack_attn_cross(m + ".attn2")
                    pack_ff(m + ".ff_in")
                    pack_ff(m + ".ff")
                    for n in ("norm_in", "norm1", "norm2", "norm3"):
                        pack_ln(f"{m}.{n}")
            elif spec.kind == "down":
                wr = f32(pfx + ".op.weight")
                W[pfx + ".w"], W[pfx + ".b"] = pack_conv3x3(dup_k(wr) if "resample" in sp else wr), f32(pfx + ".op.bias")
            elif spec.kind == "up":
                wr = f32(pfx + ".conv.weight")
                if "resample" in sp:
                    wr = dup_k(wr)
                W[pfx + ".w"], W[pfx + ".b"] = pack_conv3x3(wr), f32(pfx + ".conv.bias")
                W[pfx + ".w4"] = combine_up_phases(wr)
        pack_ln("out.0")
        wh = f32("out.2.weight")
        W["out.2.w"] = pack_conv3x3(dup_k(wh) if "head" in self.split else wh)
        W["out.2.b"] = f32("out.2.bias")
        W["emb_all.w"], W["emb_all.b"] = torch.cat(emb_w, 0).contiguous(), torch.cat(emb_b, 0).contiguous()
        W["ctx_all.w"], W["ctx_all.b"] = torch.cat(ctx_w, 0).contiguous(), torch.cat(ctx_b, 0).contiguous()
        self.emb_total, self.ctx_total = emb_total, ctx_total
        self.W = W

    def _sk(self, rows=0, hw=0, c=0):
        if not self.conv_splitk:
            return None
        tiles = max(512, splitk_tiles(rows, c)) if hw and hw <= SPLITK_MAX_PIXELS else 512
        tiles = min(tiles, SPLITK_ERROR_SLOT - 1)
        return self._buf("sk_ws", (splitk_workspace_numel(tiles),), F32, zero=True)

    def _ln(self, x, pfx, rows, c, fp8=False, split=False):
        if split:
            out = self._buf("ln16s", (rows, 2 * c), F16)
            ops.layernorm_split(x, self.W[pfx + ".g"], self.W[pfx + ".b"], out)
            return out
        if fp8:
            out = self._buf("ln8", (rows, _pad128(c)), U8, zero=True)
        else:
            out = self._buf("ln16", (rows, c), F16)
        ops.layernorm(x, self.W[pfx + ".g"], self.W[pfx + ".b"], out)
        return out

    def _slice_rows(self, rows: int, c: int, unit: int) -> int:
        if self.slice_frames <= 0 or rows * c * 2 < self.slice_min_bytes:
            return rows
        step = self.slice_frames * unit
        return step if step < rows else rows

    def _ff(self, x32, ln_pfx, ff_pfx, rows, c, *, residual, out_f32=None, out_f16=None, unit=1):
        W = self.W
        if ff_pfx + ".w1f8" in W:
            ops.ff_fused_fp8(None, W[ff_pfx + ".w1f8"], W[ff_pfx + ".w1f8e"], W[ff_pfx + ".b1"], W[ff_pfx + ".w2f8"],
                             W[ff_pfx + ".w2f8e"], W[ff_pfx + ".b2"], residual=residual, out_f32=out_f32, out_f16=out_f16,
                             ln_x=x32, ln_gamma=W[ln_pfx + ".g"], ln_beta=W[ln_pfx + ".b"], ln_eps=1e-5)
            return
        if ff_pfx + ".w18" in W:
            a8 = self._ln(x32, ln_pfx, rows, c, fp8=True)
            h8 = self._buf("ffh8", (rows, 4 * c), U8)
            ops.gemm(a8, W[ff_pfx + ".w18"], w_exp=W[ff_pfx + ".w18e"], bias=W[ff_pfx + ".b1"], out_f8=h8, geglu=True)
            ops.gemm(h8, W[ff_pfx + ".w28"], w_exp=W[ff_pfx + ".w28e"], bias=W[ff_pfx + ".b2"], residual=residual,
                     out_f32=out_f32, out_f16=out_f16)
            return
        sp_ff = "ff" in self.split
        sp_o16 = out_f16 is not None and "proj_out" in self.split
        if sp_ff or sp_o16:
            if self._slice_rows(rows, c, unit) < rows:
                raise SevaNativeError("split-precision feed-forwards do not run frame-sliced (SEVA_SLICE_FRAMES)")
            a = self._ln(x32, ln_pfx, rows, c, split=sp_ff)
            hidden = self._buf("ffhs" if sp_ff else "ffh", (rows, (8 if sp_ff else 4) * c), F16)
            (ops.gemm_split_out if sp_ff else ops.gemm)(a, W[ff_pfx + ".w1"], bias=W[ff_pfx + ".b1"], out_f16=hidden, geglu=True,
                                                      alg_k=c if sp_ff else 0)
            (ops.gemm_split_out if sp_o16 else ops.gemm)(hidden, W[ff_pfx + ".w2"], bias=W[ff_pfx + ".b2"], residual=residual,
                                                       out_f32=out_f32, out_f16=out_f16, alg_k=4 * c if sp_ff else 0)
            return
        if self.ff_fused and c in ops.FF_FUSED_CHANNELS:
            ops.ff_fused(None, W[ff_pfx + ".w1"], W[ff_pfx + ".b1"], W[ff_pfx + ".w2"], W[ff_pfx + ".b2"],
                         residual=residual, out_f32=out_f32, out_f16=out_f16,
                         ln_x=x32, ln_gamma=W[ln_pfx + ".g"], ln_beta=W[ln_pfx + ".b"], ln_eps=1e-5)
            return
        step = self._slice_rows(rows, c, unit)
        a_buf = self._buf("ln16", (step, c), F16)
        h_buf = self._buf("ffh", (step, 4 * c), F16)
        for r0 in range(0, rows, step):
            r1 = min(r0 + step, rows)
            a, hidden = a_buf[: r1 - r0], h_buf[: r1 - r0]
            ops.layernorm(x32[r0:r1], W[ln_pfx + ".g"], W[ln_pfx + ".b"], a)
            ops.gemm(a, W[ff_pfx + ".w1"], bias=W[ff_pfx + ".b1"], out_f16=hidden, geglu=True)
            ops.gemm(hidden, W[ff_pfx + ".w2"], bias=W[ff_pfx + ".b2"],
                     residual=None if residual is None else residual[r0:r1],
                     out_f32=None if out_f32 is None else out_f32[r0:r1],
                     out_f16=None if out_f16 is None else out_f16[r0:r1])

    def _resblock(self, spec, x1, x2, n, h, w, dense, emb_all):
        audit_mark(spec.prefix)
        W, pfx, hw = self.W, spec.prefix, h * w
        cin, cout = spec.cin, spec.cout
        f8_1, f8_2 = pfx + ".conv1.w8" in W, pfx + ".conv2.w8" in W
        sp_conv = "conv" in self.split
        k1, k2 = (2 * cin, 2 * cout) if sp_conv else (cin, cout)
        a16 = None if f8_1 else self._buf("gn16", (n, hw, k1), F16)
        cin8, cout8 = _pad128(cin), _pad128(cout)
        a8 = self._buf("gn8", (n, hw, cin8), U8, zero=True) if f8_1 else None
        sp_skip = cin != cout and self._split_skip(cout)
        xs16 = self._buf("skip16", (n * hw, (2 if sp_skip else 1) * cin), F16) if cin != cout else None
        s1, s2 = self._gn_stats(x1, x2)
        ops.groupnorm(x1, x2, W[pfx + ".in_layers.0.g"], W[pfx + ".in_layers.0.b"], a16, self.gn_ws,
                      eps=1e-5, silu=True, dense=dense, dense_w=W[pfx + ".dense.w"], dense_b=W[pfx + ".dense.b"],
                      raw_f16=xs16, out_f8=a8, stats1=s1, stats2=s2, split_raw=sp_skip, split_out=sp_conv)
        hmid = self._buf("res_mid", (n, hw, cout), F32)
        st_mid = self._stats_buf("res_mid", n * hw, hw, cout)
        off = self.emb_off[pfx]
        if f8_1:
            ops.conv3x3(a8.view(n, h, w, cin8), W[pfx + ".conv1.w8"], w_exp=W[pfx + ".conv1.w8e"], bias=W[pfx + ".conv1.b"],
                        row_add=emb_all[:, off:], rows_per_group=hw, ld_row_add=self.emb_total, out_f32=hmid, ch_stats=st_mid)
        else:
            ops.conv3x3(a16.view(n, h, w, k1), W[pfx + ".conv1.w"], bias=W[pfx + ".conv1.b"],
                        row_add=emb_all[:, off:], rows_per_group=hw, ld_row_add=self.emb_total, out_f32=hmid, ch_stats=st_mid,
                        splitk_ws=self._sk(n * hw, hw, cout), alg_k=9 * cin if sp_conv else 0)
        b16 = None if f8_2 else self._buf("gn16", (n, hw, k2), F16)
        b8 = self._buf("gn8", (n, hw, cout8), U8, zero=True) if f8_2 else None
        ops.groupnorm(hmid, None, W[pfx + ".out_layers.0.g"], W[pfx + ".out_layers.0.b"], b16, self.gn_ws,
                      eps=1e-5, silu=True, out_f8=b8, stats1=st_mid, split_out=sp_conv)
        fold = cin != cout and self.fold_skip and not f8_2 and (hw > 128 or not self.conv_splitk)
        if fold:
            res = None
        elif cin != cout:
            res = self._buf("skip32", (n * hw, cout), F32)
            ops.gemm(xs16, W[pfx + ".skip.w"], bias=W[pfx + ".skip.b"], out_f32=res, alg_k=cin)
        else:
            assert x2 is None
            res = x1
        out = self._buf("out:" + pfx, (n, hw, cout), F32)
        st_out = self._stats_buf("out:" + pfx, n * hw, hw, cout)
        if fold:
            ops.conv3x3(b16.view(n, h, w, k2), W[pfx + ".conv2.wf"], bias=W[pfx + ".conv2.bf"], a2=xs16, out_f32=out,
                        ch_stats=st_out)
        elif f8_2:
            ops.conv3x3(b8.view(n, h, w, cout8), W[pfx + ".conv2.w8"], w_exp=W[pfx + ".conv2.w8e"], bias=W[pfx + ".conv2.b"],
                        residual=res, out_f32=out, ch_stats=st_out)
        else:
            ops.conv3x3(b16.view(n, h, w, k2), W[pfx + ".conv2.w"], bias=W[pfx + ".conv2.b"],
                        residual=res, out_f32=out, ch_stats=st_out, splitk_ws=self._sk(n * hw, hw, cout),
                        alg_k=9 * cout if sp_conv else 0)
        self._produced(out, st_out)
        return out

    def _self_attention(self, x32, ln_pfx, at_pfx, rows, c, heads, *, regime, n, hw, T, residual,
                        row_add, rpg, ldra, out_f32):
        W = self.W
        c3 = 3 * c
        sp_qkv = "qkv" in self.split
        if sp_qkv and regime == "frame" and self.slice_attn and self._slice_rows(rows, c, hw) < rows:
            raise SevaNativeError("the split-precision QKV projection does not run frame-sliced (SEVA_SLICE_ATTN)")
        if regime == "frame" and self.slice_attn and self._slice_rows(rows, c, hw) < rows:
            step = self._slice_rows(rows, c, hw)
            a_buf = self._buf("ln16", (step, c), F16)
            qkv_buf = self._buf("qkv", (step, c3), F16)
            att_buf = self._buf("att", (step, c), F16)
            for r0 in range(0, rows, step):
                r1 = min(r0 + step, rows)
                nr, f0, nf = r1 - r0, r0 // hw, (r1 - r0) // hw
                a, qkv, att = a_buf[:nr], qkv_buf[:nr], att_buf[:nr]
                ops.layernorm(x32[r0:r1], W[ln_pfx + ".g"], W[ln_pfx + ".b"], a)
                ops.gemm(a, W[at_pfx + ".qkv"], out_f16=qkv, col_scale=QK_SCALE_LOG2E, col_scale_n=c)
                ops.attention(qkv[:, :c], qkv[:, c:2 * c], qkv[:, 2 * c:], att, nb0=nf, nb1=1, heads=heads, lq=hw, lk=hw,
                              q_strides=(hw * c3, 0, c3), k_strides=(hw * c3, 0, c3), o_strides=(hw * c, 0, c),
                              q_prescaled=True)
                ops.gemm(att, W[at_pfx + ".out.w"], bias=W[at_pfx + ".out.b"], residual=residual[r0:r1],
                         row_add=None if row_add is None else row_add[f0:], rows_per_group=rpg, ld_row_add=ldra,
                         out_f32=out_f32[r0:r1])
            return
        qkv = self._buf("qkv", (rows, 3 * c), F16)
        if at_pfx + ".qkv8" in W:
            a8 = self._ln(x32, ln_pfx, rows, c, fp8=True)
            ops.gemm(a8, W[at_pfx + ".qkv8"], w_exp=W[at_pfx + ".qkv8e"], out_f16=qkv, col_scale=QK_SCALE_LOG2E, col_scale_n=c)
        else:
            a = self._ln(x32, ln_pfx, rows, c, split=sp_qkv)
            ops.gemm(a, W[at_pfx + ".qkv"], out_f16=qkv, col_scale=QK_SCALE_LOG2E, col_scale_n=c, alg_k=c if sp_qkv else 0)
        att = self._buf("att", (rows, c), F16)
        q, k, v = qkv[:, :c], qkv[:, c:2 * c], qkv[:, 2 * c:]
        if regime == "frame":
            self._attention_long(q, k, v, att, nb0=n, heads=heads, L=hw, q_strides=(hw * c3, 0, c3),
                                 k_strides=(hw * c3, 0, c3), o_strides=(hw * c, 0, c), split_ws=None)
        elif regime == "joint":
            sws = None
            if self.attn_split and T * hw >= ops.ATTN_SPLIT_MIN_LK:
                sws = self._buf("attn_split", (ops.attention_split_workspace_numel(n // T, heads, T * hw, self.attn_split_max),), F32)
            self._attention_long(q, k, v, att, nb0=n // T, heads=heads, L=T * hw, q_strides=(T * hw * c3, 0, c3),
                                 k_strides=(T * hw * c3, 0, c3), o_strides=(T * hw * c, 0, c), split_ws=sws)
        else:
            ops.attention(q, k, v, att, nb0=n // T, nb1=hw, heads=heads, lq=T, lk=T,
                          q_strides=(T * hw * c3, c3, hw * c3), k_strides=(T * hw * c3, c3, hw * c3),
                          o_strides=(T * hw * c, c, hw * c), q_prescaled=True)
        ops.gemm(att, W[at_pfx + ".out.w"], bias=W[at_pfx + ".out.b"], residual=residual,
                 row_add=row_add, rows_per_group=rpg, ld_row_add=ldra, out_f32=out_f32)

    def _attention_long(self, q, k, v, att, *, nb0, heads, L, q_strides, k_strides, o_strides, split_ws):
        if self.pv8 and L >= ops.PV8_MIN_LQ:
            ws = self._buf("v_fp8", (ops.v_fp8_workspace_numel(nb0, heads, L),), U8)
            ops.quantize_v_fp8(v, ws, nb0=nb0, nb1=1, heads=heads, lk=L, k_strides=k_strides)
            ops.attention_pv8(q, k, ws, att, nb0=nb0, nb1=1, heads=heads, lq=L, lk=L, q_strides=q_strides,
                              k_strides=k_strides, o_strides=o_strides, split_ws=split_ws)
            return
        ops.attention(q, k, v, att, nb0=nb0, nb1=1, heads=heads, lq=L, lk=L, q_strides=q_strides, k_strides=k_strides,
                      o_strides=o_strides, q_prescaled=True, split_ws=split_ws)

    def _cross_attention_general(self, x32, ln_pfx, at_pfx, rows, c, heads, ctx16, lc, *, nb0, nb1,
                                 lq, q_strides, o_strides, ctx_batch_stride, out_f32):
        W = self.W
        a = self._ln(x32, ln_pfx, rows, c)
        q = self._buf("xq", (rows, c), F16)
        ops.gemm(a, W[at_pfx + ".q"], out_f16=q)
        kv = self._buf("xkv", (ctx16.shape[0], 2 * c), F16)
        ops.gemm(ctx16, W[at_pfx + ".kv"], out_f16=kv)
        att = self._buf("att", (rows, c), F16)
        ops.attention(q, kv[:, :c], kv[:, c:], att, nb0=nb0, nb1=nb1, heads=heads, lq=lq, lk=lc,
                      q_strides=q_strides, k_strides=(ctx_batch_stride * 2 * c, 0, 2 * c),
                      o_strides=o_strides)
        ops.gemm(att, W[at_pfx + ".out.w"], bias=W[at_pfx + ".out.b"], residual=x32, out_f32=out_f32)

    def _transformer(self, spec, x, n, h, w, T, ctxvec, ctx16, lc):
        audit_mark(spec.prefix)
        W, pfx, hw, c, heads = self.W, spec.prefix, h * w, spec.channels, spec.heads
        rows = n * hw
        sp_in, sp_out = "proj_in" in self.split, "proj_out" in self.split
        cs = 2 * c if sp_in else c
        g16 = self._buf("gn16", (n, hw, cs), F16)
        ops.groupnorm(x, None, W[pfx + ".norm.g"], W[pfx + ".norm.b"], g16, self.gn_ws, eps=1e-6, silu=False,
                      stats1=self._gn_stats(x)[0], split_out=sp_in)
        cur = self._buf("t_h", (rows, c), F32)
        ops.gemm(g16.view(rows, cs), W[pfx + ".proj_in.w"], bias=W[pfx + ".proj_in.b"], out_f32=cur, alg_k=c if sp_in else 0)
        collapse = lc == 1
        ldra_frame, ldra_scene = self.ctx_total, T * self.ctx_total
        last16 = None
        for i in range(spec.depth):
            b = f"{pfx}.transformer_blocks.{i}"
            m = f"{pfx}.time_mix_blocks.{i}"
            regime = "joint" if spec.joint else "frame"
            audit_mark(b)
            h1 = self._buf("t_h1", (rows, c), F32)
            if collapse:
                ra = ctxvec[:, self.ctx_off[b + ".attn2"]:]
                rpg, ldra = (T * hw, ldra_scene) if spec.joint else (hw, ldra_frame)
                self._self_attention(cur, b + ".norm1", b + ".attn1", rows, c, heads, regime=regime, n=n,
                                     hw=hw, T=T, residual=cur, row_add=ra, rpg=rpg, ldra=ldra, out_f32=h1)
            else:
                h0 = self._buf("t_h0", (rows, c), F32)
                self._self_attention(cur, b + ".norm1", b + ".attn1", rows, c, heads, regime=regime, n=n,
                                     hw=hw, T=T, residual=cur, row_add=None, rpg=0, ldra=0, out_f32=h0)
                if spec.joint:
                    self._cross_attention_general(
                        h0, b + ".norm2", b + ".attn2", rows, c, heads, ctx16, lc, nb0=n // T, nb1=1,
                        lq=T * hw, q_strides=(T * hw * c, 0, c), o_strides=(T * hw * c, 0, c),
                        ctx_batch_stride=T * lc, out_f32=h1)
                else:
                    self._cross_attention_general(
                        h0, b + ".norm2", b + ".attn2", rows, c, heads, ctx16, lc, nb0=n, nb1=1, lq=hw,
                        q_strides=(hw * c, 0, c), o_strides=(hw * c, 0, c), ctx_batch_stride=lc, out_f32=h1)
            h2 = self._buf("t_h2", (rows, c), F32)
            self._ff(h1, b + ".norm3", b + ".ff", rows, c, residual=h1, out_f32=h2, unit=hw)
            audit_mark(m)
            m1 = self._buf("t_m1", (rows, c), F32)
            self._ff(h2, m + ".norm_in", m + ".ff_in", rows, c, residual=h2, out_f32=m1, unit=hw)
            m2 = self._buf("t_m2", (rows, c), F32)
            if collapse:
                ra = ctxvec[:, self.ctx_off[m + ".attn2"]:]
                self._self_attention(m1, m + ".norm1", m + ".attn1", rows, c, heads, regime="temporal", n=n,
                                     hw=hw, T=T, residual=m1, row_add=ra, rpg=T * hw, ldra=ldra_scene, out_f32=m2)
            else:
                m0 = self._buf("t_m0", (rows, c), F32)
                self._self_attention(m1, m + ".norm1", m + ".attn1", rows, c, heads, regime="temporal", n=n,
                                     hw=hw, T=T, residual=m1, row_add=None, rpg=0, ldra=0, out_f32=m0)
                self._cross_attention_general(
                    m0, m + ".norm2", m + ".attn2", rows, c, heads, ctx16, lc, nb0=n // T, nb1=hw, lq=T,
                    q_strides=(T * hw * c, c, hw * c), o_strides=(T * hw * c, c, hw * c),
                    ctx_batch_stride=T * lc, out_f32=m2)
            final = i == spec.depth - 1
            nxt = None if final else self._buf("t_h", (rows, c), F32)
            last16 = self._buf("t_h16", (rows, 2 * c if sp_out else c), F16)
            self._ff(m2, m + ".norm3", m + ".ff", rows, c, residual=h2, out_f32=nxt, out_f16=last16, unit=hw)
            cur = nxt
        audit_mark(pfx)
        out = self._buf("out:" + pfx, (n, hw, c), F32)
        st_out = self._stats_buf("out:" + pfx, rows, hw, c)
        ops.gemm(last16, W[pfx + ".proj_out.w"], bias=W[pfx + ".proj_out.b"], residual=x.view(rows, c),
                 out_f32=out.view(rows, c), ch_stats=st_out, alg_k=c if sp_out else 0)
        self._produced(out, st_out)
        return out

    def _resample(self, spec, x, n, h, w):
        audit_mark(spec.prefix)
        c = spec.channels
        sp_rs = "resample" in self.split
        x16 = self._buf("rs16", (n, h, w, 2 * c if sp_rs else c), F16)
        (ops.cast_concat_f16_split if sp_rs else ops.cast_concat_f16)(x, None, x16)
        alg_k = 9 * c if sp_rs else 0
        if spec.kind == "down":
            oh, ow = (h - 1) // 2 + 1, (w - 1) // 2 + 1
            out = self._buf("out:" + spec.prefix, (n, oh * ow, c), F32)
            st_out = self._stats_buf("out:" + spec.prefix, n * oh * ow, oh * ow, c)
            ops.conv3x3(x16, self.W[spec.prefix + ".w"], stride=2, bias=self.W[spec.prefix + ".b"], out_f32=out, ch_stats=st_out,
                        splitk_ws=self._sk(n * oh * ow, oh * ow, c), alg_k=alg_k)
        else:
            oh, ow = 2 * h, 2 * w
            out = self._buf("out:" + spec.prefix, (n, oh * ow, c), F32)
            phases = getattr(ops, "conv3x3_up_phases", None)
            if phases is not None and c % 160 == 0 and env_flag("SEVA_UPSAMPLE_PHASES", "not0", True):
                st_out = None
                phases(x16, self.W[spec.prefix + ".w4"], bias=self.W[spec.prefix + ".b"], out_f32=out, ch_stats=None, alg_k=9 * c)
            else:
                st_out = self._stats_buf("out:" + spec.prefix, n * oh * ow, oh * ow, c)
                ops.conv3x3(x16, self.W[spec.prefix + ".w"], upsample=True, bias=self.W[spec.prefix + ".b"], out_f32=out,
                            ch_stats=st_out, alg_k=alg_k)
        self._produced(out, st_out)
        return out, oh, ow

    @torch.no_grad()
    def forward_graphed(self, x, concat, t, y, dense_y, num_frames):
        require_cuda(x, t, y, dense_y)
        if concat is not None and concat.numel() == 0:
            concat = None
        key = (tuple(x.shape), None if concat is None else tuple(concat.shape), tuple(y.shape),
               tuple(dense_y.shape), int(num_frames))
        ent = self._graphs.get(key)
        if ent is None:
            with torch.inference_mode(False):
                st = {
                    "x": torch.empty(x.shape, dtype=F32, device=self.device),
                    "concat": None if concat is None else torch.empty(concat.shape, dtype=F32, device=self.device),
                    "t": torch.empty(t.shape, dtype=torch.int64, device=self.device),
                    "y": torch.empty(y.shape, dtype=F32, device=self.device),
                    "dense": torch.empty(dense_y.shape, dtype=F32, device=self.device),
                }
                out = torch.empty((x.shape[0], self.p.out_channels) + tuple(x.shape[2:]), dtype=F32, device=self.device)
            self._copy_inputs(st, x, concat, t, y, dense_y)
            self.forward(st["x"], st["concat"], st["t"], st["y"], st["dense"], num_frames, out=out)
            side = torch.cuda.Stream(device=self.device)
            side.wait_stream(torch.cuda.current_stream(self.device))
            graph = ops.Graph()
            with torch.cuda.stream(side):
                graph.capture_begin(self.device)
                try:
                    self.forward(st["x"], st["concat"], st["t"], st["y"], st["dense"], num_frames, out=out)
                except BaseException:
                    try:
                        graph.capture_end(self.device)
                    except Exception:
                        pass
                    self.use_graph = False
                    raise
                graph.capture_end(self.device)
            torch.cuda.current_stream(self.device).wait_stream(side)
            ent = (graph, st, out)
            self._graphs[key] = ent
        graph, st, out = ent
        self._copy_inputs(st, x, concat, t, y, dense_y)
        graph.launch(self.device)
        return out.clone()

    @staticmethod
    def _copy_inputs(st, x, concat, t, y, dense_y):
        st["x"].copy_(x)
        if st["concat"] is not None:
            st["concat"].copy_(concat)
        st["t"].copy_(t)
        st["y"].copy_(y)
        st["dense"].copy_(dense_y)

    @audit.first_call
    def __call__(self, x, concat, t, y, dense_y, num_frames):
        if self.use_graph and not _native.network_eager_forced() and not torch.cuda.is_current_stream_capturing():
            return self.forward_graphed(x, concat, t, y, dense_y, num_frames)
        return self.forward(x, concat, t, y, dense_y, num_frames)

    @torch.no_grad()
    def forward(self, x, concat, t, y, dense_y, num_frames, out=None):
        require_cuda(x, t, y, dense_y)
        W, p, lay = self.W, self.p, self.layout
        x = x.to(F32).contiguous()
        concat = None if concat is None or concat.numel() == 0 else concat.to(F32).contiguous()
        dense_y = dense_y.to(F32).contiguous()
        n, cx, h, w = x.shape
        T = int(num_frames)
        cin = cx + (concat.shape[1] if concat is not None else 0)
        if cin != p.in_channels:
            raise ValueError(f"expected {p.in_channels} input channels, got {cin}")
        if n % T:
            raise ValueError(f"batch {n} is not a multiple of num_frames {T}")
        assert y.ndim == 3
        lc = y.shape[1]
        t = t.to(torch.int64).contiguous()
        self.gn_ws = self._buf("gn_ws", (n * ops.GN_WORKSPACE_SLABS * 32 * 2,), F32)
        self._stats = {}

        audit_mark("time_embed")
        mc, ed = p.model_channels, lay.time_embed_dim
        te16 = self._buf("te16", (n, mc), F16)
        ops.timestep_embedding_f16(t, W["freqs"], te16)
        e1 = self._buf("te_h", (n, ed), F32)
        ops.gemm(te16, W["time_embed.0.w"], bias=W["time_embed.0.b"], out_f32=e1)
        e1a = self._buf("te_h16", (n, ed), F16)
        ops.silu_f16(e1, e1a)
        emb = self._buf("emb", (n, ed), F32)
        ops.gemm(e1a, W["time_embed.2.w"], bias=W["time_embed.2.b"], out_f32=emb)
        emb_a = self._buf("emb16", (n, ed), F16)
        ops.silu_f16(emb, emb_a)
        emb_all = self._buf("emb_all", (n, self.emb_total), F32)
        ops.gemm(emb_a, W["emb_all.w"], bias=W["emb_all.b"], out_f32=emb_all)
        ctx16 = self._buf("ctx16", (n * lc, y.shape[2]), F16)
        ops.cast_concat_f16(y.to(F32).contiguous().view(n * lc, -1), None, ctx16)
        ctxvec = None
        if lc == 1:
            ctxvec = self._buf("ctxvec", (n, self.ctx_total), F32)
            ops.gemm(ctx16, W["ctx_all.w"], bias=W["ctx_all.b"], out_f32=ctxvec)

        dense_cache: dict = {}

        def dense_at(hh, ww):
            key = (hh, ww)
            if key not in dense_cache:
                d = self._buf("dense", (n, hh * ww, dense_y.shape[1]), F32)
                ops.bilinear_to_nhwc(dense_y, d, hh, ww)
                dense_cache[key] = d
            return dense_cache[key]

        stem = lay.input_blocks[0][0]
        audit_mark(stem.prefix)
        sp_stem = "stem" in self.split and 2 * cin <= CIN_PAD
        cpad = CIN_PAD * (((2 if sp_stem else 1) * cin + CIN_PAD - 1) // CIN_PAD)
        x16 = self._buf("x16", (n, h, w, cpad), F16)
        ops.nchw_to_nhwc_f16(x, concat, x16, split=sp_stem)
        cur = self._buf("out:" + stem.prefix, (n, h * w, stem.cout), F32)
        st_stem = self._stats_buf("out:" + stem.prefix, n * h * w, h * w, stem.cout)
        ops.conv3x3(x16, W[stem.prefix + ".w"], bias=W[stem.prefix + ".b"], out_f32=cur, ch_stats=st_stem,
                    alg_k=9 * cin)
        self._produced(cur, st_stem)
        ch, cw = h, w
        hs = [(cur, ch, cw)]

        def run(block, cur, x2, ch, cw):
            for spec in block:
                if spec.kind == "res":
                    cur = self._resblock(spec, cur, x2, n, ch, cw, dense_at(ch, cw), emb_all)
                    x2 = None
                elif spec.kind == "mvt":
                    cur = self._transformer(spec, cur, n, ch, cw, T, ctxvec, ctx16, lc)
                else:
                    cur, ch, cw = self._resample(spec, cur, n, ch, cw)
            return cur, ch, cw

        for block in lay.input_blocks[1:]:
            cur, ch, cw = run(block, cur, None, ch, cw)
            hs.append((cur, ch, cw))
        cur, ch, cw = run(lay.middle, cur, None, ch, cw)
        for block in lay.output_blocks:
            skip, sh, sw = hs.pop()
            assert (sh, sw) == (ch, cw)
            cur, ch, cw = run(block, cur, skip, ch, cw)

        audit_mark("out")
        cfin = lay.final_channels
        sp_head = "head" in self.split
        cf2 = (2 if sp_head else 1) * cfin
        g16 = self._buf("gn16", (n, ch * cw, cf2), F16)
        ops.groupnorm(cur, None, W["out.0.g"], W["out.0.b"], g16, self.gn_ws, eps=1e-5, silu=True,
                      stats1=self._gn_stats(cur)[0], split_out=sp_head)
        o_nhwc = self._buf("head", (n, ch * cw, p.out_channels), F32)
        ops.conv3x3(g16.view(n, ch, cw, cf2), W["out.2.w"], bias=W["out.2.b"], out_f32=o_nhwc, alg_k=9 * cfin)
        if out is None:
            out = torch.empty((n, p.out_channels, ch, cw), dtype=F32, device=self.device)
        ops.nhwc_to_nchw_f32(o_nhwc, out)
        return out
```

stable-virtual-camera_amd/seva/_native.py:

```python

from __future__ import annotations

import ctypes as C
import os
from ctypes import POINTER, c_char_p, c_double, c_float, c_int, c_int32, c_int64, c_void_p

import torch

_HERE = os.path.dirname(os.path.abspath(__file__))
LIB_PATH = os.environ.get("SEVA_HIP_LIB") or os.path.join(os.path.dirname(_HERE), "libseva_hip.so")
ABI_VERSION = 12
PROF_CLASSES = 5
PROF_NAMES = ("gemm", "conv", "attention", "norm", "elementwise")


class SevaNativeError(RuntimeError):
    pass


class GemmDesc(C.Structure):
    _fields_ = [
        ("a", c_void_p), ("w", c_void_p), ("bias", c_void_p), ("row_add", c_void_p),
        ("residual", c_void_p), ("out_f32", c_void_p), ("out_f16", c_void_p),
        ("M", c_int64), ("N", c_int64), ("K", c_int64),
        ("lda", c_int64), ("ldr", c_int64), ("ldo32", c_int64), ("ldo16", c_int64),
        ("rows_per_group", c_int64), ("ld_row_add", c_int64),
        ("mode", c_int32), ("epilogue", c_int32),
        ("n", c_int32), ("ih", c_int32), ("iw", c_int32), ("cin", c_int32),
        ("oh", c_int32), ("ow", c_int32), ("stride", c_int32), ("upsample", c_int32),
        ("col_scale", c_float), ("col_scale_n", c_int32), ("pad_br_only", c_int32),
        ("w_exp", c_void_p), ("out_f8", c_void_p), ("ldo8", c_int64),
        ("ch_stats", c_void_p), ("splitk_ws", c_void_p), ("splitk_ws_bytes", c_int64),
        ("a2", c_void_p), ("lda2", c_int64), ("K2", c_int64),
        ("alg_K", c_int64),
    ]


class FfDesc(C.Structure):
    _fields_ = [
        ("a", c_void_p), ("w1", c_void_p), ("b1", c_void_p), ("w2", c_void_p), ("b2", c_void_p),
        ("residual", c_void_p), ("out_f32", c_void_p), ("out_f16", c_void_p),
        ("M", c_int64), ("lda", c_int64), ("ldr", c_int64), ("ldo32", c_int64), ("ldo16", c_int64),
        ("C", c_int32),
        ("ln_x", c_void_p), ("ln_gamma", c_void_p), ("ln_beta", c_void_p), ("ldx", c_int64), ("ln_eps", c_float),
        ("w1_exp", c_void_p), ("w2_exp", c_void_p),
    ]


class AttnDesc(C.Structure):
    _fields_ = [
        ("q", c_void_p), ("k", c_void_p), ("v", c_void_p), ("out", c_void_p),
        ("q_sb0", c_int64), ("q_sb1", c_int64), ("q_sl", c_int64),
        ("k_sb0", c_int64), ("k_sb1", c_int64), ("k_sl", c_int64),
        ("o_sb0", c_int64), ("o_sb1", c_int64), ("o_sl", c_int64),
        ("nb0", c_int32), ("nb1", c_int32), ("heads", c_int32),
        ("lq", c_int32), ("lk", c_int32), ("scale", c_float), ("q_prescaled", c_int32),
        ("split_ws", c_void_p), ("split_ws_bytes", c_int64),
    ]


class GroupNormDesc(C.Structure):
    _fields_ = [
        ("x1", c_void_p), ("x2", c_void_p), ("gamma", c_void_p), ("beta", c_void_p),
        ("dense", c_void_p), ("dense_w", c_void_p), ("dense_b", c_void_p),
        ("out_f16", c_void_p), ("workspace", c_void_p),
        ("n", c_int32), ("hw", c_int32), ("c1", c_int32), ("c2", c_int32),
        ("groups", c_int32), ("dense_c", c_int32), ("silu", c_int32), ("eps", c_float),
        ("raw_f16", c_void_p), ("out_f8", c_void_p), ("ld_out_f8", c_int64),
        ("stats1", c_void_p), ("stats2", c_void_p),
        ("split_out_f16", c_int32), ("split_raw_f16", c_int32),
    ]


class ImageDesc(C.Structure):
    _fields_ = [
        ("src", c_void_p), ("context_rgb", c_void_p), ("out", c_void_p),
        ("src_pitch_n", c_int64), ("src_pitch_c", c_int64), ("src_pitch_row", c_int64), ("out_pitch_n", c_int64),
        ("n", c_int32), ("h", c_int32), ("w", c_int32), ("src_c", c_int32),
        ("rh", c_int32), ("rw", c_int32), ("ct", c_int32), ("cl", c_int32), ("H", c_int32), ("W", c_int32),
        ("pad_value", c_float), ("out_mul", c_float), ("out_add", c_float),
    ]


class MetricsDesc(C.Structure):
    _fields_ = [
        ("a", c_void_p), ("b", c_void_p), ("sse", c_void_p), ("ssim_sum", c_void_p), ("ssim_map", c_void_p),
        ("workspace", c_void_p),
        ("a_pitch_n", c_int64), ("b_pitch_n", c_int64), ("workspace_bytes", c_int64),
        ("n", c_int32), ("H", c_int32), ("W", c_int32), ("kind", c_int32), ("ssim", c_int32),
    ]


class LpipsLayerDesc(C.Structure):
    _fields_ = [
        ("fa", c_void_p), ("fb", c_void_p), ("w", c_void_p), ("out", c_void_p), ("workspace", c_void_p),
        ("a_pitch_n", c_int64), ("b_pitch_n", c_int64), ("workspace_bytes", c_int64), ("hw", c_int64),
        ("n", c_int32), ("C", c_int32),
    ]


class RangeDesc(C.Structure):
    _fields_ = [
        ("x", c_void_p), ("dtype", c_int32), ("rows", c_int64), ("cols", c_int64), ("pitch", c_int64),
        ("workspace", c_void_p), ("workspace_bytes", c_int64), ("out", c_void_p),
    ]


SYMBOLS = {
    "seva_last_error": (c_char_p, []),
    "seva_last_plan": (c_char_p, []),
    "seva_abi_version": (c_int, []),
    "seva_target_arch": (c_char_p, []),
    "seva_gemm_f16": (c_int, [POINTER(GemmDesc), c_void_p]),
    "seva_gemm_f16_split_out": (c_int, [POINTER(GemmDesc), c_void_p]),
    "seva_gemm_fp8": (c_int, [POINTER(GemmDesc), c_void_p]),
    "seva_ff_fused_f16": (c_int, [POINTER(FfDesc), c_void_p]),
    "seva_ff_fused_fp8": (c_int, [POINTER(FfDesc), c_void_p]),
    "seva_attention_f16": (c_int, [POINTER(AttnDesc), c_void_p]),
    "seva_attn_v_fp8_size": (c_int, [c_int32, c_int32, c_int32, POINTER(c_int64), POINTER(c_int64)]),
    "seva_attn_quant_v_fp8": (c_int, [POINTER(AttnDesc), c_void_p, c_void_p, c_void_p]),
    "seva_attention_pv8": (c_int, [POINTER(AttnDesc), c_void_p, c_void_p, c_void_p]),
    "seva_groupnorm_f16": (c_int, [POINTER(GroupNormDesc), c_void_p]),
    "seva_layernorm_f16": (c_int, [c_void_p, c_void_p, c_void_p, c_void_p, c_int64, c_int32, c_float, c_void_p]),
    "seva_layernorm_f16_split": (c_int, [c_void_p, c_void_p, c_void_p, c_void_p, c_int64, c_int32, c_float, c_void_p]),
    "seva_layernorm_fp8": (c_int, [c_void_p, c_void_p, c_void_p, c_void_p, c_int64, c_int32, c_float, c_int64, c_void_p]),
    "seva_layernorm_f32": (c_int, [c_void_p, c_void_p, c_void_p, c_void_p, c_int64, c_int32, c_float, c_void_p]),
    "seva_clip_preprocess_f16": (c_int, [c_void_p, c_void_p, c_int32, c_int32, c_int32, c_int32, c_int32, c_int32,
                                         c_void_p, c_void_p, c_int32, c_void_p]),
    "seva_attention_small_f16": (c_int, [c_void_p, c_void_p, c_void_p, c_void_p, c_int64, c_int64, c_int64, c_int64,
                                         c_int64, c_int64, c_int32, c_int32, c_int32, c_int32, c_float, c_void_p]),
    "seva_softmax_rows_f16": (c_int, [c_void_p, c_int64, c_void_p, c_int64, c_int64, c_int32, c_int32, c_float, c_void_p]),
    "seva_nchw_to_nhwc_f16": (c_int, [c_void_p, c_int32, c_void_p, c_int32, c_void_p, c_void_p, c_int32, c_int32, c_int32, c_void_p]),
    "seva_nchw_to_nhwc_f16_split": (c_int, [c_void_p, c_int32, c_void_p, c_int32, c_void_p, c_void_p, c_int32, c_int32, c_int32, c_void_p]),
    "seva_nhwc_to_nchw_f32": (c_int, [c_void_p, c_int64, c_void_p, c_int32, c_int32, c_int32, c_void_p]),
    "seva_cast_concat_f16": (c_int, [c_void_p, c_int32, c_void_p, c_int32, c_void_p, c_int64, c_void_p]),
    "seva_cast_concat_f16_split": (c_int, [c_void_p, c_int32, c_void_p, c_int32, c_void_p, c_int64, c_void_p]),
    "seva_bilinear_to_nhwc_f32": (c_int, [c_void_p, c_void_p, c_int32, c_int32, c_int32, c_int32, c_int32, c_int32, c_void_p]),
    "seva_timestep_embedding_f16": (c_int, [c_void_p, c_void_p, c_void_p, c_int32, c_int32, c_void_p]),
    "seva_silu_f16": (c_int, [c_void_p, c_void_p, c_int64, c_void_p]),
    "seva_add_f32": (c_int, [c_void_p, c_void_p, c_void_p, c_int64, c_void_p]),
    "seva_replace_blend_f32": (c_int, [c_void_p, c_void_p, c_void_p, c_int32, c_int32, c_int32, c_void_p]),
    "seva_denoiser_combine_f32": (c_int, [c_void_p, c_void_p, c_void_p, c_void_p, c_void_p, c_int32, c_int64, c_void_p]),
    "seva_add_noise_f32": (c_int, [c_void_p, c_void_p, c_void_p, c_void_p, c_int32, c_int64, c_void_p]),
    "seva_cfg_euler_f32": (c_int, [c_void_p, c_void_p, c_void_p, c_void_p, c_void_p, c_void_p, c_int32, c_int64, c_void_p]),
    "seva_cfg_multistep_f32": (c_int, [c_void_p, c_void_p, c_void_p, c_void_p, c_void_p, c_void_p, c_void_p, c_void_p, c_void_p,
                                       c_int32, c_int64, c_void_p]),
    "seva_cfg_combine_f32": (c_int, [c_void_p, c_void_p, c_void_p, c_int32, c_int64, c_void_p]),
    "seva_euler_step_f32": (c_int, [c_void_p, c_void_p, c_void_p, c_void_p, c_void_p, c_int32, c_int64, c_void_p]),
    "seva_to_d_f32": (c_int, [c_void_p, c_void_p, c_void_p, c_void_p, c_int32, c_int64, c_void_p]),
    "seva_scale_rows_f32": (c_int, [c_void_p, c_void_p, c_void_p, c_int32, c_int64, c_void_p]),
    "seva_plucker_f32": (c_int, [c_void_p, c_void_p, c_void_p, c_int32, c_int32, c_int32, c_void_p]),
    "seva_cond_concat_f32": (c_int, [c_void_p, c_void_p, c_void_p, c_void_p, c_int32, c_int32, c_int32, c_void_p]),
    "seva_image_area_crop_u8": (c_int, [POINTER(ImageDesc), c_void_p]),
    "seva_image_area_crop_f32": (c_int, [POINTER(ImageDesc), c_void_p]),
    "seva_rgb_to_u8": (c_int, [c_void_p, c_int64, c_void_p, c_int32, c_int32, c_int32, c_void_p]),
    "seva_frame_metrics_size": (c_int, [c_int32, c_int32, c_int32, POINTER(c_int64)]),
    "seva_frame_metrics": (c_int, [POINTER(MetricsDesc), c_void_p]),
    "seva_lpips_prepare_f16": (c_int, [c_void_p, c_int64, c_int32, c_void_p, c_int32, c_int32, c_int32, c_void_p]),
    "seva_lpips_relu_pool_f16": (c_int, [c_void_p, c_void_p, c_void_p, c_int32, c_int32, c_int32, c_int32, c_void_p]),
    "seva_lpips_layer_size": (c_int, [c_int32, c_int64, POINTER(c_int64)]),
    "seva_lpips_layer": (c_int, [POINTER(LpipsLayerDesc), c_void_p]),
    "seva_tensor_range_size": (c_int, [c_int64, c_int64, POINTER(c_int64)]),
    "seva_tensor_range": (c_int, [POINTER(RangeDesc), c_void_p]),
    "seva_set_knob": (c_int, [c_char_p, c_int32]),
    "seva_get_knob": (c_int, [c_char_p, POINTER(c_int32)]),
    "seva_graph_begin": (c_int, [c_void_p]),
    "seva_graph_end": (c_int, [c_void_p, POINTER(c_void_p)]),
    "seva_graph_launch": (c_int, [c_void_p, c_void_p]),
    "seva_graph_destroy": (c_int, [c_void_p]),
    "seva_prof_enable": (c_int, [c_int]),
    "seva_prof_collect": (c_int, [POINTER(c_double), POINTER(c_int64), POINTER(c_double), POINTER(c_double)]),
}

_lib = None

_EAGER_DEPTH = 0


class eager_network:
    def __enter__(self):
        global _EAGER_DEPTH
        _EAGER_DEPTH += 1

    def __exit__(self, *exc):
        global _EAGER_DEPTH
        _EAGER_DEPTH -= 1
        return False


def network_eager_forced() -> bool:
    return _EAGER_DEPTH > 0


def load() -> C.CDLL:
    global _lib
    if _lib is not None:
        return _lib
    if not os.path.exists(LIB_PATH):
        raise SevaNativeError(
            f"{LIB_PATH} not found: build it with `make -C stable-virtual-camera_amd/csrc` "
            "(or `python -c 'import __graft_entry__ as g; g.build()'`). There is no CPU fallback."
        )
    try:
        lib = C.CDLL(LIB_PATH)
    except OSError as e:
        raise SevaNativeError(f"cannot load {LIB_PATH}: {e}") from e
    for name, (res, args) in SYMBOLS.items():
        try:
            fn = getattr(lib, name)
        except AttributeError as e:
            raise SevaNativeError(f"{LIB_PATH} does not export {name}") from e
        fn.restype = res
        fn.argtypes = args
    if lib.seva_abi_version() != ABI_VERSION:
        raise SevaNativeError(
            f"ABI mismatch: library {lib.seva_abi_version()} vs binding {ABI_VERSION}"
        )
    _lib = lib
    return lib


def check(rc: int, what: str = "") -> None:
    if rc != 0:
        msg = load().seva_last_error().decode("utf-8", "replace")
        raise SevaNativeError(f"{what or 'seva native call'} failed (rc={rc}): {msg}")


def stream_ptr(device=None) -> int:
    return torch.cuda.current_stream(device).cuda_stream


def ptr(t: torch.Tensor | None) -> int | None:
    return None if t is None else t.data_ptr()


def require_cuda(*tensors: torch.Tensor) -> None:
    for t in tensors:
        if t is not None and not t.is_cuda:
            raise SevaNativeError(
                "seva HIP operators need tensors on an AMD GPU (cuda device); "
                "there is no CPU fallback path."
            )
```

stable-virtual-camera_amd/seva/ops.py:

```python

from __future__ import annotations

import ctypes as C
import functools
import inspect

import torch

from . import _native as nv
from ._native import AttnDesc, GemmDesc, GroupNormDesc, ImageDesc, LpipsLayerDesc, MetricsDesc, check, ptr, require_cuda, stream_ptr

F16, F32 = torch.float16, torch.float32
U8 = torch.uint8


def _lib():
    return nv.load()


RANGE_WORDS = 72
RANGE_WG_ELEMS = 32768
RANGE_MAX_WGS = 2048
RANGE_DTYPES = {F32: 0, F16: 1, U8: 2}

AUDITED: dict = {}
NOT_AUDITED = {
    "tensor_range": "the audit's own instrument (uint64 words)",
    "tensor_range_workspace_numel": "size query",
    "_up_phases": "shared body of conv3x3_up_phases / conv3x3_up_phases128, which are audited",
    "_v_fp8_parts": "size query",
    "rgb_to_u8": "uint8 output",
    "frame_metrics_workspace_numel": "size query",
    "frame_metrics": "integer and fp64 sums",
    "lpips_layer_workspace_numel": "size query",
    "lpips_layer": "fp64 sums",
    "set_knob": "knob",
    "get_knob": "knob",
    "last_plan": "plan name of the last launch",
    "prof_enable": "profiling switch",
    "prof_collect": "profiling counters",
}
_AUDIT = None


def audit_mark(scope: str) -> None:
    if _AUDIT is not None:
        _AUDIT.scope = scope


def _audited(*outputs: str):
    def deco(fn):
        AUDITED[fn.__name__] = outputs
        sig = inspect.signature(fn)

        @functools.wraps(fn)
        def wrapper(*a, **kw):
            if _AUDIT is None:
                return fn(*a, **kw)
            r = fn(*a, **kw)
            bound = sig.bind(*a, **kw)
            bound.apply_defaults()
            audit_outputs(fn.__name__, bound.arguments)
            return r

        return wrapper

    return deco


def audit_outputs(op: str, a: dict) -> None:
    if _AUDIT is None:
        return
    for name in AUDITED[op]:
        t = a.get(name)
        if t is not None:
            for label, off, rows, cols, pitch in _audit_views(op, name, t, a):
                _AUDIT.output(op, label, t, off, rows, cols, pitch)


def _as_2d(t: torch.Tensor) -> list:
    if t.dim() == 0 or t.numel() == 0:
        return [] if t.numel() == 0 else [(0, 1, 1, 1)]
    assert t.stride(-1) == 1 or t.shape[-1] == 1, "audited outputs have unit inner stride"
    shape, stride = list(t.shape), list(t.stride())
    cols, j = 1, len(shape) - 1
    while j >= 0 and (shape[j] == 1 or stride[j] == cols):
        cols *= shape[j]
        j -= 1
    if j < 0:
        return [(0, t.numel() // shape[-1], shape[-1], shape[-1])]
    if all(shape[i + 1] == 1 or stride[i] == stride[i + 1] * shape[i + 1] for i in range(j)):
        rows = 1
        for i in range(j + 1):
            rows *= shape[i]
        return [(0, rows, cols, stride[j])]
    return [(i * stride[0] + o, r, c, p) for i in range(shape[0]) for o, r, c, p in _as_2d(t[i])]


def _audit_views(op: str, name: str, t: torch.Tensor, a: dict) -> list:
    def lastdim(cols, split=False, rows=None):
        rows = t.numel() // t.shape[-1] if rows is None else rows
        pitch = t.stride(-2) if t.dim() >= 2 else t.shape[-1]
        if split:
            return [(name + ".hi", 0, rows, cols, pitch), (name + ".lo", cols, rows, cols, pitch)]
        return [(name, 0, rows, cols, pitch)]

    if op == "gemm":
        no = a["w"].shape[0] // (2 if a["geglu"] else 1)
        return lastdim(no, split=a["split_out"] and name == "out_f16", rows=a["a"].shape[0])
    if op == "conv3x3":
        return lastdim(a["w"].shape[0])
    if op in ("conv3x3_up_phases", "conv3x3_up_phases128"):
        return lastdim(a["w4"].shape[1])
    if op in ("ff_fused", "ff_fused_fp8"):
        return lastdim(a["w2"].shape[0])
    if op == "groupnorm":
        c = a["x1"].shape[2] + (a["x2"].shape[2] if a["x2"] is not None else 0)
        return lastdim(c, split=(name == "out_f16" and a["split_out"]) or (name == "raw_f16" and a["split_raw"]),
                       rows=a["x1"].shape[0] * a["x1"].shape[1])
    if op == "layernorm":
        c = a["x"].shape[-1]
        return lastdim(c, rows=a["x"].numel() // c)
    if op in ("layernorm_split", "cast_concat_f16_split"):
        return lastdim(t.shape[-1] // 2, split=True)
    if op == "nchw_to_nhwc_f16":
        return lastdim(a["x1"].shape[1] + (a["x2"].shape[1] if a["x2"] is not None else 0), split=a["split"])
    if op == "softmax_rows":
        return lastdim(a["cols"])
    if op == "clip_preprocess":
        return lastdim(3 * a["patch"] * a["patch"])
    if op == "quantize_v_fp8":
        return [(name, 0, 1, _v_fp8_parts(a["nb0"] * a["nb1"], a["heads"], a["lk"])[0], t.numel())]
    return [(name, off, rows, cols, pitch) for off, rows, cols, pitch in _as_2d(t)]


def _size_query(fn, *dims: int) -> int:
    size = C.c_int64()
    check(fn(*(int(d) for d in dims), C.byref(size)), fn.__name__)
    return size.value


def _workspace(workspace: torch.Tensor | None, need: int, device, who: str) -> torch.Tensor:
    if workspace is None:
        workspace = torch.empty(need, dtype=U8, device=device)
    assert workspace.dtype == U8 and workspace.is_contiguous() and workspace.numel() >= need, f"{who} workspace too small"
    return workspace


def _dense_planes(x: torch.Tensor, what: str) -> None:
    H, W = x.shape[2:]
    assert x.stride(3) == 1 and x.stride(2) == W and x.stride(1) == H * W, f"{what} planes must be dense"


def _frame_layout(x: torch.Tensor) -> tuple[int, int, int, int]:
    if x.dtype == U8:
        n, H, W, c = x.shape
        assert c == 3 and x.stride(3) == 1 and x.stride(2) == 3 and x.stride(1) == 3 * W, "uint8 frames: (n,H,W,3) with dense images"
        return 0, n, H, W
    n, c, H, W = x.shape
    assert c == 3 and x.stride(3) == 1 and x.stride(2) == W and x.stride(1) == H * W, "fp32 frames: (n,3,H,W) with dense planes"
    return 1, n, H, W


def tensor_range_workspace_numel(rows: int, cols: int) -> int:
    return _size_query(_lib().seva_tensor_range_size, rows, cols)


def tensor_range(x: torch.Tensor, out: torch.Tensor | None = None, *, rows: int | None = None, cols: int | None = None,
                 workspace: torch.Tensor | None = None) -> torch.Tensor:
    require_cuda(x, out, workspace)
    if x.dtype not in RANGE_DTYPES:
        raise nv.SevaNativeError(f"tensor_range: dtype {x.dtype} (float32, float16, or uint8 holding e4m3 bytes)")
    if x.dim() == 1:
        x = x.unsqueeze(0)
    if x.dim() != 2 or (x.stride(1) != 1 and x.shape[1] != 1):
        raise nv.SevaNativeError(f"tensor_range: a 2-D view with unit inner stride (got shape {tuple(x.shape)}, strides {x.stride()})")
    rows = x.shape[0] if rows is None else int(rows)
    cols = x.shape[1] if cols is None else int(cols)
    if not (0 < rows <= x.shape[0] and 0 < cols <= x.shape[1]):
        raise nv.SevaNativeError(f"tensor_range: rows x cols = {rows} x {cols} outside the view {tuple(x.shape)}")
    pitch = x.stride(0) if rows > 1 else cols
    if pitch < cols:
        raise nv.SevaNativeError(f"tensor_range: row pitch {pitch} below cols {cols} (overlapping rows)")
    if out is None:
        out = torch.empty(RANGE_WORDS, dtype=torch.int64, device=x.device)
    assert out.dtype == torch.int64 and out.numel() == RANGE_WORDS and out.is_contiguous()
    workspace = _workspace(workspace, tensor_range_workspace_numel(rows, cols), x.device, "tensor_range")
    d = nv.RangeDesc()
    d.x, d.dtype, d.rows, d.cols, d.pitch = x.data_ptr(), RANGE_DTYPES[x.dtype], rows, cols, pitch
    d.workspace, d.workspace_bytes, d.out = workspace.data_ptr(), workspace.numel(), out.data_ptr()
    check(_lib().seva_tensor_range(C.byref(d), stream_ptr(x.device)), "seva_tensor_range")
    return out


@_audited("out_f32", "out_f16", "out_f8")
def gemm(
    a: torch.Tensor,
    w: torch.Tensor,
    *,
    bias: torch.Tensor | None = None,
    row_add: torch.Tensor | None = None,
    rows_per_group: int = 0,
    ld_row_add: int = 0,
    residual: torch.Tensor | None = None,
    out_f32: torch.Tensor | None = None,
    out_f16: torch.Tensor | None = None,
    geglu: bool = False,
    col_scale: float = 1.0,
    col_scale_n: int = 0,
    w_exp: torch.Tensor | None = None,
    out_f8: torch.Tensor | None = None,
    ch_stats: torch.Tensor | None = None,
    splitk_ws: torch.Tensor | None = None,
    alg_k: int = 0,
    split_out: bool = False,
) -> None:
    fp8 = w_exp is not None
    require_cuda(a, w)
    if split_out and (fp8 or out_f8 is not None or ch_stats is not None or out_f16 is None):
        raise ValueError("gemm(split_out=True) is the f16 GEMM with an out_f16 (no fp8 operands, out_f8 or ch_stats)")
    assert a.dim() == 2 and w.dim() == 2 and a.dtype == w.dtype == (U8 if fp8 else F16)
    M, K = a.shape
    N = w.shape[0]
    d = _gemm_desc(a, w, (M, N, K), lda=a.stride(0), pitch_dim=0, fp8=fp8, geglu=geglu, col_scale=col_scale, col_scale_n=col_scale_n,
                   bias=bias, row_add=row_add, rows_per_group=rows_per_group, ld_row_add=ld_row_add, residual=residual, out_f32=out_f32,
                   out_f16=out_f16, w_exp=w_exp, out_f8=out_f8, ch_stats=ch_stats, splitk_ws=splitk_ws, alg_k=alg_k)
    if fp8:
        assert w_exp.dtype == U8 and w_exp.numel() == N and (out_f8 is None or out_f8.dtype == U8)
        check(_lib().seva_gemm_fp8(C.byref(d), stream_ptr(a.device)), "seva_gemm_fp8")
    elif split_out:
        assert out_f16.dtype == F16 and out_f16.stride(-1) == 1
        check(_lib().seva_gemm_f16_split_out(C.byref(d), stream_ptr(w.device)), "seva_gemm_f16_split_out")
    else:
        assert out_f8 is None
        check(_lib().seva_gemm_f16(C.byref(d), stream_ptr(w.device)), "seva_gemm_f16")


def gemm_split_out(a: torch.Tensor, w: torch.Tensor, **kw) -> None:
    gemm(a, w, split_out=True, **kw)


STATS_ROWS = 64


def channel_stats_shape(rows: int, channels: int) -> tuple[int, int, int]:
    return ((rows + STATS_ROWS - 1) // STATS_ROWS, 2, channels)


SPLITK_FLAGS = 16384
SPLITK_ERROR_SLOT = 16383
SPLITK_TILE_M = 128
SPLITK_TILE_N = 160
SPLITK_MAX_PIXELS = 128
_handoff_ws: dict = {}


def _register_handoff_ws(ws: torch.Tensor) -> None:
    if ws.data_ptr() not in _handoff_ws:
        import weakref

        _handoff_ws[ws.data_ptr()] = weakref.ref(ws)


def check_handoffs() -> None:
    bad = []
    for key, ref in list(_handoff_ws.items()):
        ws = ref()
        if ws is None or ws.data_ptr() != key:
            _handoff_ws.pop(key, None)
            continue
        if torch.cuda.is_current_stream_capturing():
            return
        n = int(ws[SPLITK_ERROR_SLOT:SPLITK_ERROR_SLOT + 1].view(torch.int32).item())
        if n:
            ws[:SPLITK_FLAGS].zero_()
            bad.append(n)
    if bad:
        raise nv.SevaNativeError(
            f"split-K hand-off: {sum(bad)} consumer workgroup(s) gave up waiting for their producer; the outputs of the "
            "affected launches are wrong (flags re-armed; rerun, or set SEVA_CONV_SPLITK=0)")


def splitk_tiles(rows: int, channels: int) -> int:
    return ((rows + SPLITK_TILE_M - 1) // SPLITK_TILE_M) * ((channels + 127) // 128)


def splitk_workspace_numel(tiles: int) -> int:
    return SPLITK_FLAGS + tiles * SPLITK_TILE_M * SPLITK_TILE_N


def splitk_workspace(max_rows: int, max_channels: int, device) -> torch.Tensor:
    return torch.zeros(splitk_workspace_numel(max(512, splitk_tiles(max_rows, max_channels))), dtype=F32, device=device)


def _stats_ptr(ch_stats, M, N, out_f32):
    if ch_stats is None:
        return None
    assert out_f32 is not None and ch_stats.dtype == F32 and ch_stats.is_contiguous()
    assert ch_stats.numel() >= ((M + STATS_ROWS - 1) // STATS_ROWS) * 2 * N
    return ch_stats.data_ptr()


def _pitch(t, dim: int) -> int:
    return t.stride(dim) if t is not None else 0


def _gemm_desc(a, w, mnk, *, lda, pitch_dim, conv=None, a2=None, fp8=False, geglu=False, col_scale=0.0, col_scale_n=0, bias=None,
               row_add=None, rows_per_group=0, ld_row_add=0, residual=None, out_f32=None, out_f16=None, w_exp=None, out_f8=None,
               ch_stats=None, splitk_ws=None, alg_k=0) -> GemmDesc:
    d = GemmDesc()
    d.a, d.w = a.data_ptr(), w.data_ptr()
    d.bias, d.row_add, d.residual = ptr(bias), ptr(row_add), ptr(residual)
    d.out_f32, d.out_f16 = ptr(out_f32), ptr(out_f16)
    d.M, d.N, d.K = mnk
    d.alg_K = alg_k
    d.lda = lda
    d.ldr, d.ldo32, d.ldo16 = _pitch(residual, pitch_dim), _pitch(out_f32, pitch_dim), _pitch(out_f16, pitch_dim)
    d.rows_per_group, d.ld_row_add = rows_per_group, ld_row_add
    d.mode, d.epilogue = 0 if conv is None else 1, 1 if geglu else 0
    d.col_scale, d.col_scale_n = col_scale, col_scale_n
    if conv is not None:
        d.n, d.ih, d.iw, d.cin, d.oh, d.ow, d.stride, d.upsample, d.pad_br_only = conv
    if a2 is not None:
        d.a2, d.lda2, d.K2 = a2.data_ptr(), a2.stride(0), a2.shape[1]
    d.ch_stats = _stats_ptr(ch_stats, mnk[0], mnk[1], out_f32)
    if splitk_ws is not None and not fp8:
        assert splitk_ws.dtype == F32 and splitk_ws.is_contiguous()
        d.splitk_ws, d.splitk_ws_bytes = splitk_ws.data_ptr(), splitk_ws.numel() * 4
        _register_handoff_ws(splitk_ws)
    if fp8:
        d.w_exp, d.out_f8, d.ldo8 = w_exp.data_ptr(), ptr(out_f8), _pitch(out_f8, pitch_dim)
    return d


FF_FUSED_CHANNELS = (64, 128, 256, 320)


def _ff_desc(a, w1, b1, w2, b2, M, c, residual, out_f32, out_f16, ln_x, ln_gamma, ln_beta, ln_eps, w1_exp=None, w2_exp=None) -> nv.FfDesc:
    d = nv.FfDesc()
    d.w1, d.b1, d.w2, d.b2 = w1.data_ptr(), b1.data_ptr(), w2.data_ptr(), b2.data_ptr()
    d.w1_exp, d.w2_exp = ptr(w1_exp), ptr(w2_exp)
    if ln_x is not None:
        d.ln_x, d.ln_gamma, d.ln_beta, d.ldx, d.ln_eps = ln_x.data_ptr(), ln_gamma.data_ptr(), ln_beta.data_ptr(), ln_x.stride(0), ln_eps
    else:
        d.a, d.lda = ptr(a), a.stride(0)
    d.residual, d.out_f32, d.out_f16 = ptr(residual), ptr(out_f32), ptr(out_f16)
    d.M, d.C = M, c
    d.ldr, d.ldo32, d.ldo16 = _pitch(residual, 0), _pitch(out_f32, 0), _pitch(out_f16, 0)
    return d


@_audited("out_f32", "out_f16")
def ff_fused(a: torch.Tensor | None, w1: torch.Tensor, b1: torch.Tensor, w2: torch.Tensor, b2: torch.Tensor, *,
             residual: torch.Tensor | None = None, out_f32: torch.Tensor | None = None,
             out_f16: torch.Tensor | None = None, ln_x: torch.Tensor | None = None,
             ln_gamma: torch.Tensor | None = None, ln_beta: torch.Tensor | None = None, ln_eps: float = 1e-5) -> None:
    src = ln_x if ln_x is not None else a
    require_cuda(src, w1, w2)
    M, c = src.shape
    assert (ln_x is not None and ln_x.dtype == F32 and ln_gamma is not None and ln_beta is not None) or a.dtype == F16
    assert w1.dtype == F16 and w2.dtype == F16 and w1.shape == (8 * c, c) and w2.shape == (c, 4 * c)
    assert w1.is_contiguous() and w2.is_contiguous() and c in FF_FUSED_CHANNELS
    d = _ff_desc(a, w1, b1, w2, b2, M, c, residual, out_f32, out_f16, ln_x, ln_gamma, ln_beta, ln_eps)
    check(_lib().seva_ff_fused_f16(C.byref(d), stream_ptr(src.device)), "seva_ff_fused_f16")


FF8_STEP = 128


def ff8_feature_of(pos: torch.Tensor) -> torch.Tensor:
    return 64 * ((pos >> 3) & 1) + 32 * (pos >> 6) + 8 * ((pos >> 4) & 3) + (pos & 7)


def pack_ff_fp8(w1: torch.Tensor, w2: torch.Tensor):
    c = w1.shape[1]
    assert w1.shape == (8 * c, c) and w2.shape == (c, 4 * c) and c in FF_FUSED_CHANNELS
    kp = (c + 127) // 128 * 128
    w1p = torch.cat([w1.float(), w1.new_zeros((8 * c, kp - c), dtype=torch.float32)], 1) if kp != c else w1.float()
    w1_8, w1_exp = quantize_weight_fp8(w1p)
    w2_8, w2_exp = quantize_weight_fp8(w2)
    perm = (torch.arange(4 * c, device=w2.device) // FF8_STEP) * FF8_STEP + ff8_feature_of(torch.arange(4 * c, device=w2.device) % FF8_STEP)
    return w1_8, w1_exp, w2_8[:, perm].contiguous(), w2_exp


@_audited("out_f32", "out_f16")
def ff_fused_fp8(a: torch.Tensor | None, w1: torch.Tensor, w1_exp: torch.Tensor, b1: torch.Tensor, w2: torch.Tensor,
                 w2_exp: torch.Tensor, b2: torch.Tensor, *, residual: torch.Tensor | None = None,
                 out_f32: torch.Tensor | None = None, out_f16: torch.Tensor | None = None, ln_x: torch.Tensor | None = None,
                 ln_gamma: torch.Tensor | None = None, ln_beta: torch.Tensor | None = None, ln_eps: float = 1e-5) -> None:
    src = ln_x if ln_x is not None else a
    require_cuda(src, w1, w2)
    M = src.shape[0]
    c = w2.shape[0]
    kp = (c + 127) // 128 * 128
    assert (ln_x is not None and ln_x.dtype == F32 and ln_x.shape[1] == c and ln_gamma is not None and ln_beta is not None) or \
        (a is not None and a.dtype == U8 and a.shape[1] >= c and a.stride(1) == 1)
    assert w1.dtype == U8 and w2.dtype == U8 and w1.shape == (8 * c, kp) and w2.shape == (c, 4 * c)
    assert w1_exp.dtype == U8 and w2_exp.dtype == U8 and w1_exp.numel() == 8 * c and w2_exp.numel() == c
    assert w1.is_contiguous() and w2.is_contiguous() and c in FF_FUSED_CHANNELS
    d = _ff_desc(a, w1, b1, w2, b2, M, c, residual, out_f32, out_f16, ln_x, ln_gamma, ln_beta, ln_eps, w1_exp, w2_exp)
    check(_lib().seva_ff_fused_fp8(C.byref(d), stream_ptr(src.device)), "seva_ff_fused_fp8")


@_audited("out_f32", "out_f16", "out_f8")
def conv3x3(
    x: torch.Tensor,
    w: torch.Tensor,
    *,
    stride: int = 1,
    upsample: bool = False,
    bias: torch.Tensor | None = None,
    row_add: torch.Tensor | None = None,
    rows_per_group: int = 0,
    ld_row_add: int = 0,
    residual: torch.Tensor | None = None,
    out_f32: torch.Tensor | None = None,
    out_f16: torch.Tensor | None = None,
    pad_br_only: bool = False,
    w_exp: torch.Tensor | None = None,
    ch_stats: torch.Tensor | None = None,
    splitk_ws: torch.Tensor | None = None,
    a2: torch.Tensor | None = None,
    alg_k: int = 0,
    out_f8: torch.Tensor | None = None,
) -> None:
    require_cuda(x, w)
    fp8 = w_exp is not None
    assert x.dtype == w.dtype == (U8 if fp8 else F16) and x.dim() == 4 and x.is_contiguous()
    n, ih, iw, cin = x.shape
    eh, ew = (2 * ih, 2 * iw) if upsample else (ih, iw)
    ps = 1 if pad_br_only else 2
    oh, ow = (eh + ps - 3) // stride + 1, (ew + ps - 3) // stride + 1
    M, N, K = n * oh * ow, w.shape[0], 9 * cin
    if a2 is not None:
        assert not fp8 and not upsample and a2.dtype == F16 and a2.dim() == 2 and a2.stride(1) == 1 and a2.shape[0] == M
        K += a2.shape[1]
    assert w.shape[1] == K
    if fp8:
        assert w_exp.dtype == U8 and w_exp.numel() == N
        if out_f8 is not None:
            assert out_f8.dtype == U8 and out_f8.stride(-1) == 1 and out_f8.shape[-1] >= N
            assert not upsample, "out_f8 and the fused upsample are not available together"
    else:
        assert out_f8 is None, "out_f8 belongs to the fp8 conv (w_exp)"
    d = _gemm_desc(x, w, (M, N, K), lda=cin, pitch_dim=-2, a2=a2, fp8=fp8, bias=bias, row_add=row_add, rows_per_group=rows_per_group,
                   ld_row_add=ld_row_add, residual=residual, out_f32=out_f32, out_f16=out_f16, w_exp=w_exp, out_f8=out_f8,
                   ch_stats=ch_stats, splitk_ws=splitk_ws, alg_k=alg_k,
                   conv=(n, ih, iw, cin, oh, ow, stride, 1 if upsample else 0, 1 if pad_br_only else 0))
    if fp8:
        check(_lib().seva_gemm_fp8(C.byref(d), stream_ptr(x.device)), "seva_gemm_fp8(conv)")
    else:
        check(_lib().seva_gemm_f16(C.byref(d), stream_ptr(x.device)), "seva_gemm_f16(conv)")


def _up_phases(name: str, code: int, what: str, x, w4, bias, out_f32, ch_stats, alg_k) -> None:
    require_cuda(x, w4)
    assert x.dtype == w4.dtype == F16 and x.dim() == 4 and x.is_contiguous() and w4.is_contiguous()
    n, ih, iw, cin = x.shape
    assert w4.dim() == 3 and w4.shape[0] == 4 and w4.shape[2] == 4 * cin, "w4: [4, cout, 4 * cin]"
    if code == 2 and ch_stats is not None:
        raise ValueError(f"{name} emits no GroupNorm statistics (ch_stats must be None)")
    if out_f32 is None:
        raise ValueError(f"{name} needs out_f32")
    oh, ow = 2 * ih, 2 * iw
    d = _gemm_desc(x, w4, (n * oh * ow, w4.shape[1], 4 * cin), lda=cin, pitch_dim=-2, conv=(n, ih, iw, cin, oh, ow, 1, code, 0),
                   bias=bias, out_f32=out_f32, ch_stats=ch_stats, alg_k=alg_k)
    check(_lib().seva_gemm_f16(C.byref(d), stream_ptr(x.device)), what)


@_audited("out_f32")
def conv3x3_up_phases(x: torch.Tensor, w4: torch.Tensor, *, bias: torch.Tensor | None = None, out_f32: torch.Tensor | None = None,
                      ch_stats: torch.Tensor | None = None, alg_k: int = 0) -> None:
    _up_phases("conv3x3_up_phases", 2, "seva_gemm_f16(conv, upsample phases)", x, w4, bias, out_f32, ch_stats, alg_k)


@_audited("out_f32")
def conv3x3_up_phases128(x: torch.Tensor, w4: torch.Tensor, *, bias: torch.Tensor | None = None, out_f32: torch.Tensor | None = None,
                         ch_stats: torch.Tensor | None = None, alg_k: int = 0) -> None:
    _up_phases("conv3x3_up_phases128", 4, "seva_gemm_f16(conv, upsample phases, 128 columns)", x, w4, bias, out_f32, ch_stats, alg_k)


@_audited("out")
def attention(
    q: torch.Tensor,
    k: torch.Tensor,
    v: torch.Tensor,
    out: torch.Tensor,
    *,
    nb0: int,
    nb1: int,
    heads: int,
    lq: int,
    lk: int,
    q_strides: tuple[int, int, int],
    k_strides: tuple[int, int, int],
    o_strides: tuple[int, int, int],
    scale: float = 0.125,
    q_prescaled: bool = False,
    split_ws: torch.Tensor | None = None,
) -> None:
    require_cuda(q, k, v, out)
    d = _attn_desc(q, k, v, out, nb0, nb1, heads, lq, lk, q_strides, k_strides, o_strides, split_ws, scale, q_prescaled)
    check(_lib().seva_attention_f16(C.byref(d), stream_ptr(q.device)), "seva_attention_f16")


ATTN_SPLIT_MIN_LK = 6144
ATTN_SPLIT_ROW_FLOATS = 66


def attention_split_workspace_numel(batch: int, heads: int, lq: int, nsplit: int = 2) -> int:
    return nsplit * batch * heads * lq * ATTN_SPLIT_ROW_FLOATS


PV8_MIN_LQ = 2048


def _v_fp8_parts(batch: int, heads: int, lk: int) -> tuple[int, int]:
    v8, sc = C.c_int64(), C.c_int64()
    check(_lib().seva_attn_v_fp8_size(batch, heads, lk, C.byref(v8), C.byref(sc)), "seva_attn_v_fp8_size")
    return v8.value, sc.value


def v_fp8_workspace_numel(batch: int, heads: int, lk: int) -> int:
    v8, sc = _v_fp8_parts(batch, heads, lk)
    return v8 + sc


def _v_fp8_ptrs(ws: torch.Tensor, batch: int, heads: int, lk: int) -> tuple[int, int]:
    v8, sc = _v_fp8_parts(batch, heads, lk)
    assert ws.dtype == U8 and ws.is_contiguous() and ws.numel() >= v8 + sc, "v_fp8 workspace too small"
    return ws.data_ptr(), ws.data_ptr() + v8


def _attn_desc(q, k, v, out, nb0, nb1, heads, lq, lk, q_strides, k_strides, o_strides, split_ws, scale=0.0, q_prescaled=True) -> AttnDesc:
    d = AttnDesc()
    d.q, d.k, d.v, d.out = ptr(q), ptr(k), ptr(v), ptr(out)
    d.q_sb0, d.q_sb1, d.q_sl = q_strides
    d.k_sb0, d.k_sb1, d.k_sl = k_strides
    d.o_sb0, d.o_sb1, d.o_sl = o_strides
    d.nb0, d.nb1, d.heads, d.lq, d.lk, d.scale = nb0, nb1, heads, lq, lk, scale
    d.q_prescaled = 1 if q_prescaled else 0
    if split_ws is not None:
        assert split_ws.dtype == F32 and split_ws.is_contiguous()
        d.split_ws, d.split_ws_bytes = split_ws.data_ptr(), split_ws.numel() * 4
    return d


@_audited("ws")
def quantize_v_fp8(v: torch.Tensor, ws: torch.Tensor, *, nb0: int, nb1: int, heads: int, lk: int,
                   k_strides: tuple[int, int, int]) -> None:
    require_cuda(v, ws)
    v8, sc = _v_fp8_ptrs(ws, nb0 * nb1, heads, lk)
    d = _attn_desc(None, None, v, None, nb0, nb1, heads, lk, lk, (0, 0, 0), k_strides, (0, 0, 0), None)
    check(_lib().seva_attn_quant_v_fp8(C.byref(d), v8, sc, stream_ptr(v.device)), "seva_attn_quant_v_fp8")


@_audited("out")
def attention_pv8(q: torch.Tensor, k: torch.Tensor, ws: torch.Tensor, out: torch.Tensor, *, nb0: int, nb1: int, heads: int,
                  lq: int, lk: int, q_strides: tuple[int, int, int], k_strides: tuple[int, int, int],
                  o_strides: tuple[int, int, int], split_ws: torch.Tensor | None = None) -> None:
    require_cuda(q, k, ws, out)
    v8, sc = _v_fp8_ptrs(ws, nb0 * nb1, heads, lk)
    d = _attn_desc(q, k, None, out, nb0, nb1, heads, lq, lk, q_strides, k_strides, o_strides, split_ws)
    check(_lib().seva_attention_pv8(C.byref(d), v8, sc, stream_ptr(q.device)), "seva_attention_pv8")


GN_WORKSPACE_SLABS = 1024


def groupnorm_workspace(n: int, device) -> torch.Tensor:
    return torch.empty(n * GN_WORKSPACE_SLABS * 32 * 2, dtype=F32, device=device)


@_audited("out_f16", "raw_f16", "out_f8")
def groupnorm(
    x1: torch.Tensor,
    x2: torch.Tensor | None,
    gamma: torch.Tensor,
    beta: torch.Tensor,
    out_f16: torch.Tensor,
    workspace: torch.Tensor,
    *,
    groups: int = 32,
    eps: float = 1e-5,
    silu: bool = False,
    dense: torch.Tensor | None = None,
    dense_w: torch.Tensor | None = None,
    dense_b: torch.Tensor | None = None,
    raw_f16: torch.Tensor | None = None,
    out_f8: torch.Tensor | None = None,
    stats1: torch.Tensor | None = None,
    stats2: torch.Tensor | None = None,
    split_out: bool = False,
    split_raw: bool = False,
) -> None:
    require_cuda(x1, out_f16 if out_f16 is not None else out_f8)
    n, hw, c1 = x1.shape
    c2 = x2.shape[2] if x2 is not None else 0
    d = GroupNormDesc()
    d.x1, d.x2, d.gamma, d.beta = x1.data_ptr(), ptr(x2), gamma.data_ptr(), beta.data_ptr()
    d.dense, d.dense_w, d.dense_b = ptr(dense), ptr(dense_w), ptr(dense_b)
    d.out_f16, d.workspace = ptr(out_f16), workspace.data_ptr()
    d.out_f8 = ptr(out_f8)
    if out_f8 is not None:
        assert out_f8.dtype == U8 and out_f8.is_contiguous() and out_f8.shape[:2] == (n, hw) and out_f8.shape[2] >= c1 + c2
        d.ld_out_f8 = out_f8.shape[2]
    d.n, d.hw, d.c1, d.c2, d.groups = n, hw, c1, c2, groups
    d.dense_c = dense.shape[-1] if dense is not None else 0
    d.silu, d.eps = 1 if silu else 0, eps
    d.raw_f16 = ptr(raw_f16)
    if stats1 is not None:
        assert hw % STATS_ROWS == 0 and (x2 is None) == (stats2 is None)
        assert stats1.dtype == F32 and stats1.numel() >= (n * hw // STATS_ROWS) * 2 * c1
        assert stats2 is None or (stats2.dtype == F32 and stats2.numel() >= (n * hw // STATS_ROWS) * 2 * c2)
        d.stats1, d.stats2 = stats1.data_ptr(), ptr(stats2)
    else:
        assert stats2 is None
    assert raw_f16 is None or (raw_f16.dtype == F16 and raw_f16.is_contiguous()
                               and raw_f16.numel() == n * hw * (c1 + c2) * (2 if split_raw else 1))
    assert not split_out or (out_f16 is not None and out_f16.is_contiguous() and out_f16.numel() == 2 * n * hw * (c1 + c2))
    d.split_out_f16, d.split_raw_f16 = int(split_out), int(split_raw)
    assert workspace.numel() >= n * GN_WORKSPACE_SLABS * groups * 2
    check(_lib().seva_groupnorm_f16(C.byref(d), stream_ptr(x1.device)), "seva_groupnorm_f16")


@_audited("out_f16")
def layernorm(x: torch.Tensor, gamma: torch.Tensor, beta: torch.Tensor, out_f16: torch.Tensor,
              eps: float = 1e-5) -> None:
    require_cuda(x, out_f16)
    c = x.shape[-1]
    rows = x.numel() // c
    if out_f16.dtype == F32:
        assert out_f16.data_ptr() != x.data_ptr()
        check(_lib().seva_layernorm_f32(x.data_ptr(), gamma.data_ptr(), beta.data_ptr(),
                                        out_f16.data_ptr(), rows, c, eps, stream_ptr(x.device)),
              "seva_layernorm_f32")
        return
    if out_f16.dtype == U8:
        assert out_f16.dim() == 2 and out_f16.stride(1) == 1 and out_f16.shape[0] == rows
        check(_lib().seva_layernorm_fp8(x.data_ptr(), gamma.data_ptr(), beta.data_ptr(),
                                        out_f16.data_ptr(), rows, c, eps, out_f16.stride(0), stream_ptr(x.device)),
              "seva_layernorm_fp8")
        return
    assert out_f16.dtype == F16
    check(_lib().seva_layernorm_f16(x.data_ptr(), gamma.data_ptr(), beta.data_ptr(),
                                    out_f16.data_ptr(), rows, c, eps, stream_ptr(x.device)),
          "seva_layernorm_f16")


@_audited("out_f16")
def layernorm_split(x: torch.Tensor, gamma: torch.Tensor, beta: torch.Tensor, out_f16: torch.Tensor, eps: float = 1e-5) -> None:
    require_cuda(x, out_f16)
    c = x.shape[-1]
    rows = x.numel() // c
    assert x.dtype == F32 and x.is_contiguous() and out_f16.dtype == F16 and out_f16.is_contiguous() and out_f16.numel() == 2 * rows * c
    check(_lib().seva_layernorm_f16_split(x.data_ptr(), gamma.data_ptr(), beta.data_ptr(), out_f16.data_ptr(), rows, c, eps,
                                          stream_ptr(x.device)), "seva_layernorm_f16_split")


def quantize_weight_fp8(w: torch.Tensor):
    w = w.float()
    amax = w.abs().amax(dim=1).clamp_min(1e-30)
    e = torch.ceil(torch.log2(amax / 448.0)).clamp(-126, 127)
    q = (w * torch.exp2(-e)[:, None]).clamp(-448.0, 448.0).to(torch.float8_e4m3fn)
    return q.view(torch.uint8).contiguous(), (e + 127).to(torch.uint8).contiguous()


# ... 392 lines not shown
```

Baseline: 11.03 denoising steps/s.

## Fuse next block's LayerNorm into the fused feed-forward epilogue

Adds a variant of the fused FF kernel that, after computing the output rows, also applies the following block's LayerNorm and writes an f16 normalized copy. The model then passes this precomputed tensor into the next self-attention, which skips its own LayerNorm launch and the extra read of the f32 activation. The cost is a row-wide reduction in the FF epilogue, which adds cross-wave work and register and LDS pressure there. The kernel body moves into an include file compiled twice, once per mode.

```diff
diff --git a/include/seva_hip.h b/include/seva_hip.h
--- a/include/seva_hip.h
+++ b/include/seva_hip.h
@@ -79,6 +79,14 @@
   const void* w2_exp;
 } seva_ff_desc;
 int seva_ff_fused_f16(const seva_ff_desc* d, seva_stream_t stream);
+typedef struct seva_ff_next_ln {
+  const float* gamma;
+  const float* beta;
+  void* out_f16;
+  int64_t ldo;
+  float eps;
+} seva_ff_next_ln;
+int seva_ff_fused_f16_ln(const seva_ff_desc* d, const seva_ff_next_ln* next, seva_stream_t stream);
 int seva_ff_fused_fp8(const seva_ff_desc* d, seva_stream_t stream);
 
 #define SEVA_ATTN_LONG_MIN_LQ 2048
diff --git a/stable-virtual-camera_amd/csrc/ff_fused.hip b/stable-virtual-camera_amd/csrc/ff_fused.hip
--- a/stable-virtual-camera_amd/csrc/ff_fused.hip
+++ b/stable-virtual-camera_amd/csrc/ff_fused.hip
@@ -1,5 +1,6 @@
 #include "gemm_common.h"
 #include "ff_fp8.h"
+#include "ln_row.h"
 
 #include <atomic>
 
@@ -23,6 +24,18 @@
   float ln_eps;
 };
 
+struct FfNextLn {
+  const float* gamma;
+  const float* beta;
+  half_t* out;
+  int64_t ldo;
+  float eps;
+};
+struct FfLnArgs {
+  FfArgs f;
+  FfNextLn n;
+};
+
 struct Ff8Args {
   FfArgs f;
   const uint8_t* w1_exp;
@@ -39,244 +52,12 @@
 }
 
 
-template <int C>
-__global__ __launch_bounds__(512, 2) void ff_fused8_kernel(FfArgs p) {
-  constexpr int KS = C / 32, NK1 = C / 64, NJ2 = C / 16, NJH = NJ2 / 2, NCH = C / 16;
-  constexpr int W1_BYTES = 128 * 128, W2_BYTES = C * 128;
-  constexpr int W2_PASSES = C / 64;
-  constexpr int W2_PER_KT = (W2_PASSES + NK1 - 1) / NK1;
-  static_assert(NJ2 % 2 == 0, "output blocks split over the two waves of a row group");
-
-  extern __shared__ __attribute__((aligned(16))) char smem[];
-  constexpr int W1_RING = 3;
-  char* const lds_w1 = smem;
-  char* const lds_w2 = smem + W1_RING * W1_BYTES;
-  float* const lds_b1 = (float*)(smem + W1_RING * W1_BYTES + 2 * W2_BYTES);
-  char* const lds_x = smem + W1_RING * W1_BYTES + 2 * W2_BYTES + 8 * C * 4;
-  const unsigned lds_base_u32 = __builtin_amdgcn_readfirstlane(lds_addr_u32(smem));
-
-  const int lane = threadIdx.x & 63;
-  const int wave = __builtin_amdgcn_readfirstlane(threadIdx.x >> 6);
-  const int mr = wave & 3, h = wave >> 2;
-  const int fr = lane & 15, fg = lane >> 4;
-  const int sr = lane >> 3, sp = lane & 7;
-
-  const int tm = xcd_remap(blockIdx.x, p.tiles_m);
-  const int64_t m0 = (int64_t)tm * 128 + mr * 32;
-
-  half8_t areg[2][KS];
-  if (p.ln_x) {
-#pragma unroll
-    for (int i = 0; i < 2; ++i) {
-      int64_t m = m0 + 16 * i + fr;
-      if (m >= p.M) m = p.M - 1;
-      const float* xr = p.ln_x + m * p.ldx + 8 * fg;
-      f32x4 v[KS][2];
-#pragma unroll
-      for (int ks = 0; ks < KS; ++ks) {
-        v[ks][0] = first_read(*(const f32x4*)(xr + 32 * ks));
-        v[ks][1] = first_read(*(const f32x4*)(xr + 32 * ks + 4));
-      }
-      float sum = 0.f;
-#pragma unroll
-      for (int ks = 0; ks < KS; ++ks)
-#pragma unroll
-        for (int e = 0; e < 2; ++e) sum += v[ks][e][0] + v[ks][e][1] + v[ks][e][2] + v[ks][e][3];
-      sum += __shfl_xor(sum, 16, 64);
-      asm volatile("" : "+v"(sum));
-      sum += __shfl_xor(sum, 32, 64);
-      asm volatile("" : "+v"(sum));
-      const float mean = sum / (float)C;
-      float ss = 0.f;
-#pragma unroll
-      for (int ks = 0; ks < KS; ++ks)
-#pragma unroll
-        for (int e = 0; e < 2; ++e)
-#pragma unroll
-          for (int r = 0; r < 4; ++r) {
-            const float dlt = v[ks][e][r] - mean;
-            ss += dlt * dlt;
-          }
-      ss += __shfl_xor(ss, 16, 64);
-      asm volatile("" : "+v"(ss));
-      ss += __shfl_xor(ss, 32, 64);
-      asm volatile("" : "+v"(ss));
-      const float rstd = rsqrtf(ss / (float)C + p.ln_eps);
-#pragma unroll
-      for (int ks = 0; ks < KS; ++ks) {
-        half_t y[8];
-#pragma unroll
-        for (int e = 0; e < 2; ++e) {
-          const f32x4 g4 = first_read(*(const f32x4*)(p.ln_gamma + 32 * ks + 8 * fg + 4 * e));
-          const f32x4 b4 = first_read(*(const f32x4*)(p.ln_beta + 32 * ks + 8 * fg + 4 * e));
-#pragma unroll
-          for (int r = 0; r < 4; ++r) y[4 * e + r] = (half_t)((v[ks][e][r] - mean) * rstd * g4[r] + b4[r]);
-        }
-        areg[i][ks] = half8_t{y[0], y[1], y[2], y[3], y[4], y[5], y[6], y[7]};
-      }
-    }
-  } else {
-#pragma unroll
-    for (int i = 0; i < 2; ++i) {
-      int64_t m = m0 + 16 * i + fr;
-      if (m >= p.M) m = p.M - 1;
-      const half_t* ap = p.a + m * p.lda + 8 * fg;
-#pragma unroll
-      for (int ks = 0; ks < KS; ++ks) areg[i][ks] = *(const half8_t*)(ap + 32 * ks);
-    }
-  }
-  f32x4 acc2[2][NJH];
-#pragma unroll
-  for (int i = 0; i < 2; ++i) {
-    int64_t m = m0 + 16 * i + fr;
-    if (m >= p.M) m = p.M - 1;
-#pragma unroll
-    for (int jj = 0; jj < NJH; ++jj)
-      acc2[i][jj] = p.residual ? *(const f32x4*)(p.residual + m * p.ldr + 16 * (h * NJH + jj) + 4 * fg) : f32x4{0.f, 0.f, 0.f, 0.f};
-  }
-  for (int i = threadIdx.x; i < 2 * C; i += 512) *(f32x4*)(lds_b1 + 4 * i) = *(const f32x4*)(p.b1 + 4 * i);
-#pragma unroll
-  for (int i = 0; i < 2; ++i) {
-#pragma unroll
-    for (int ks = 0; ks < KS; ++ks) asm volatile("" : "+v"(areg[i][ks]));
-#pragma unroll
-    for (int jj = 0; jj < NJH; ++jj) asm volatile("" : "+v"(acc2[i][jj]));
-  }
-
-  auto w1_key = [](int row) { return ((row >> 1) & 1) | (((row >> 3) & 3) << 1); };
-  const half_t* w1_src[2];
-#pragma unroll
-  for (int i = 0; i < 2; ++i) {
-    const int row = wave * 16 + 8 * i + sr;
-    w1_src[i] = p.w1 + (int64_t)row * C + (sp ^ w1_key(row)) * 8;
-  }
-  const half_t* w2_src[2];
-#pragma unroll
-  for (int i = 0; i < 2; ++i) {
-    const int row = wave * (C / 8) + 8 * i + sr;
-    w2_src[i] = p.w2 + (int64_t)row * (4 * C) + (sp ^ ((row >> 1) & 7)) * 8;
-  }
-  auto stage_w1 = [&](int buf, int hc, int kt) {
-    const unsigned dst = lds_base_u32 + buf * W1_BYTES + wave * 16 * 128;
-    const int64_t off = (int64_t)hc * 128 * C + kt * 64;
-#pragma unroll
-    for (int i = 0; i < 2; ++i) glds16_raw(w1_src[i] + off, dst + i * 1024);
-  };
-  auto stage_w2_part = [&](int buf, int hc, int part) {
-    const unsigned dst = lds_base_u32 + W1_RING * W1_BYTES + buf * W2_BYTES + wave * (C / 8) * 128;
-#pragma unroll
-    for (int u = 0; u < W2_PER_KT; ++u) {
-      const int i = part * W2_PER_KT + u;
-      if (i < W2_PASSES) glds16_raw(w2_src[i & 1] + (int64_t)(i >> 1) * 16 * (4 * C) + hc * 64, dst + i * 1024);
-    }
-  };
-
-  int w1_off[2], w2_off[2];
-#pragma unroll
-  for (int s = 0; s < 2; ++s) {
-    const int rb = 64 * h + 8 * (fr >> 2) + (fr & 3);
-    w1_off[s] = rb * 128 + (((4 * s + fg) ^ w1_key(rb)) << 4);
-    const int r2 = 16 * (h * NJH) + fr;
-    w2_off[s] = r2 * 128 + (((4 * s + fg) ^ ((r2 >> 1) & 7)) << 4);
-  }
-  char* const x_mine = lds_x + ((mr * 2 + h) * 2) * 1024 + lane * 16;
-  const char* const x_q0 = lds_x + (mr * 2 * 2) * 1024 + lane * 16;
-
-  constexpr int NTILES = NCH * NK1;
-  auto stage_w1_seq = [&](int g) { stage_w1(g % W1_RING, g / NK1, g % NK1); };
-  auto wait_all_but = [&](int n) {
-    if (n >= 3) wait_vm<3>();
-    else if (n == 2) wait_vm<2>();
-    else if (n == 1) wait_vm<1>();
-    else wait_vm<0>();
-  };
-  __syncthreads();
-  stage_w1_seq(0);
-#pragma unroll
-  for (int part = 0; part < NK1; ++part) stage_w2_part(0, 0, part);
-  if (NTILES > 1) stage_w1_seq(1);
-  if (NTILES > 1) wait_vm<2>();
-  else wait_vm<0>();
-  lds_barrier();
-
-  int g = 0;
-  for (int hc = 0; hc < NCH; ++hc) {
-    f32x4 acc1[2][4];
-#pragma unroll
-    for (int e = 0; e < 2; ++e) {
-      const float* bp = lds_b1 + hc * 128 + 64 * h + 8 * fg + 4 * e;
-      acc1[0][e] = acc1[1][e] = *(const f32x4*)bp;
-      acc1[0][2 + e] = acc1[1][2 + e] = *(const f32x4*)(bp + 32);
-    }
-#pragma unroll
-    for (int kt = 0; kt < NK1; ++kt) {
-      int issued = 0;
-      if (g + 2 < NTILES) {
-        stage_w1_seq(g + 2);
-        issued += 2;
-      }
-      if (hc + 1 < NCH && kt * W2_PER_KT < W2_PASSES) {
-        stage_w2_part((hc + 1) & 1, hc + 1, kt);
-        issued += (kt + 1) * W2_PER_KT <= W2_PASSES ? W2_PER_KT : W2_PASSES - kt * W2_PER_KT;
-      }
-      const char* const tb = lds_w1 + (g % W1_RING) * W1_BYTES;
-      half8_t bfr[2][4];
-#pragma unroll
-      for (int s = 0; s < 2; ++s)
-#pragma unroll
-        for (int j = 0; j < 4; ++j) bfr[s][j] = *(const half8_t*)(tb + w1_off[s] + (32 * (j >> 1) + 4 * (j & 1)) * 128);
-#pragma unroll
-      for (int s = 0; s < 2; ++s)
-#pragma unroll
-        for (int i = 0; i < 2; ++i)
-#pragma unroll
-          for (int j = 0; j < 4; ++j)
-            acc1[i][j] = __builtin_amdgcn_mfma_f32_16x16x32_f16(bfr[s][j], areg[i][2 * kt + s], acc1[i][j], 0, 0, 0);
-      wait_all_but(issued);
-      lds_barrier();
-      ++g;
-    }
-#pragma unroll
-    for (int i = 0; i < 2; ++i) {
-      const f32x4 o0 = geglu4(acc1[i][0], acc1[i][2]);
-      const f32x4 o1 = geglu4(acc1[i][1], acc1[i][3]);
-      *(half8_t*)(x_mine + i * 1024) = half8_t{(half_t)o0[0], (half_t)o0[1], (half_t)o0[2], (half_t)o0[3],
-                                               (half_t)o1[0], (half_t)o1[1], (half_t)o1[2], (half_t)o1[3]};
-    }
-    lds_barrier();
-    half8_t hq[2][2];
-#pragma unroll
-    for (int q = 0; q < 2; ++q)
-#pragma unroll
-      for (int i = 0; i < 2; ++i) hq[q][i] = *(const half8_t*)(x_q0 + (q * 2 + i) * 1024);
-    const char* const t2 = lds_w2 + (hc & 1) * W2_BYTES;
-#pragma unroll
-    for (int jj = 0; jj < NJH; ++jj) {
-      const half8_t w0 = *(const half8_t*)(t2 + w2_off[0] + jj * (16 * 128));
-      const half8_t w1f = *(const half8_t*)(t2 + w2_off[1] + jj * (16 * 128));
-#pragma unroll
-      for (int i = 0; i < 2; ++i) {
-        acc2[i][jj] = __builtin_amdgcn_mfma_f32_16x16x32_f16(w0, hq[0][i], acc2[i][jj], 0, 0, 0);
-        acc2[i][jj] = __builtin_amdgcn_mfma_f32_16x16x32_f16(w1f, hq[1][i], acc2[i][jj], 0, 0, 0);
-      }
-    }
-    lds_barrier();
-  }
-
-#pragma unroll
-  for (int i = 0; i < 2; ++i) {
-    const int64_t m = m0 + 16 * i + fr;
-    const bool ok = m < p.M;
-#pragma unroll
-    for (int jj = 0; jj < NJH; ++jj) {
-      const int f = 16 * (h * NJH + jj) + 4 * fg;
-      const f32x4 v = acc2[i][jj] + first_read(*(const f32x4*)(p.b2 + f));
-      if (!ok) continue;
-      if (p.out_f32) *(f32x4*)(p.out_f32 + m * p.ldo32 + f) = v;
-      if (p.out_f16) *(half4_t*)(p.out_f16 + m * p.ldo16 + f) = to_f16x4(v);
-    }
-  }
-}
+#define FF8_NEXT_LN 0
+#include "ff_fused8_kernel.inc"
+#undef FF8_NEXT_LN
+#define FF8_NEXT_LN 1
+#include "ff_fused8_kernel.inc"
+#undef FF8_NEXT_LN
 
 
 template <int C>
@@ -599,10 +380,11 @@
 }
 
 struct FfWork { double flops, bytes; };
-FfWork ff_work(const seva_ff_desc* d, double a_bytes, double w_bytes) {
+FfWork ff_work(const seva_ff_desc* d, double a_bytes, double w_bytes, bool next_ln = false) {
   const double C = (double)d->C, M = (double)d->M;
   return {2.0 * M * C * (8.0 * C) + 2.0 * M * (4.0 * C) * C,
-          M * C * ((d->ln_x ? 4.0 : a_bytes) + (d->residual ? 4.0 : 0.0) + (d->out_f32 ? 4.0 : 0.0) + (d->out_f16 ? 2.0 : 0.0)) + w_bytes};
+          M * C * ((d->ln_x ? 4.0 : a_bytes) + (d->residual ? 4.0 : 0.0) + (d->out_f32 ? 4.0 : 0.0) + (d->out_f16 ? 2.0 : 0.0) +
+                   (next_ln ? 2.0 : 0.0)) + w_bytes};
 }
 
 template <class Args>
@@ -615,6 +397,11 @@
 int ff_launch8(const FfArgs& a, hipStream_t s) {
   static std::atomic<uint64_t> attr_devs{0};
   return ff_launch(ff_fused8_kernel<C>, "ff_fused8_kernel", 3 * 128 * 128 + 2 * C * 128 + 8 * C * 4 + 16 * 1024, attr_devs, a, a.tiles_m, s);
+}
+template <int C>
+int ff_launch8_ln(const FfLnArgs& a, hipStream_t s) {
+  static std::atomic<uint64_t> attr_devs{0};
+  return ff_launch(ff_fused8_ln_kernel<C>, "ff_fused8_ln_kernel", 3 * 128 * 128 + 2 * C * 128 + 8 * C * 4 + 16 * 1024, attr_devs, a, a.f.tiles_m, s);
 }
 template <int C>
 int ff_launch8_fp8(const Ff8Args& a, hipStream_t s) {
@@ -626,13 +413,28 @@
 
 }
 
-extern "C" int seva_ff_fused_f16(const seva_ff_desc* d, seva_stream_t stream) {
+extern "C" int seva_ff_fused_f16_ln(const seva_ff_desc* d, const seva_ff_next_ln* next, seva_stream_t stream) {
   if (const int rc = validate_ff<false>(d, "ff_fused")) return rc;
+  if (next) {
+    SEVA_REQUIRE(next->gamma && next->beta && next->out_f16, "ff_fused: next_ln: null pointer");
+    SEVA_REQUIRE(next->ldo >= d->C && next->ldo % 4 == 0, "ff_fused: next_ln: ldo=%lld invalid (>= C, multiple of 4)", (long long)next->ldo);
+    SEVA_REQUIRE(((uintptr_t)next->gamma | (uintptr_t)next->beta | (uintptr_t)next->out_f16) % 16 == 0,
+                 "ff_fused: next_ln: pointers must be 16-byte aligned");
+  }
   const FfArgs a = ff_args(d);
   hipStream_t s = (hipStream_t)stream;
   const double C = (double)d->C;
-  const FfWork w = ff_work(d, 2.0, 2.0 * (8.0 * C * C + 4.0 * C * C));
+  const FfWork w = ff_work(d, 2.0, 2.0 * (8.0 * C * C + 4.0 * C * C), next != nullptr);
   SevaProfScope prof(0, w.flops, s, w.bytes);
+  if (next) {
+    const FfLnArgs q{a, FfNextLn{next->gamma, next->beta, (half_t*)next->out_f16, next->ldo, next->eps}};
+    switch (d->C) {
+      case 64: return ff_launch8_ln<64>(q, s);
+      case 128: return ff_launch8_ln<128>(q, s);
+      case 256: return ff_launch8_ln<256>(q, s);
+      default: return ff_launch8_ln<320>(q, s);
+    }
+  }
   switch (d->C) {
     case 64: return ff_launch8<64>(a, s);
     case 128: return ff_launch8<128>(a, s);
@@ -640,6 +442,8 @@
     default: return ff_launch8<320>(a, s);
   }
 }
+
+extern "C" int seva_ff_fused_f16(const seva_ff_desc* d, seva_stream_t stream) { return seva_ff_fused_f16_ln(d, nullptr, stream); }
 
 extern "C" int seva_ff_fused_fp8(const seva_ff_desc* d, seva_stream_t stream) {
   if (const int rc = validate_ff<true>(d, "ff_fused_fp8")) return rc;
diff --git a/stable-virtual-camera_amd/csrc/ff_fused8_kernel.inc b/stable-virtual-camera_amd/csrc/ff_fused8_kernel.inc
--- /dev/null
+++ b/stable-virtual-camera_amd/csrc/ff_fused8_kernel.inc
@@ -0,0 +1,291 @@
+template <int C>
+#if FF8_NEXT_LN
+__global__ __launch_bounds__(512, 2) void ff_fused8_ln_kernel(FfLnArgs q) {
+  const FfArgs& p = q.f;
+  const FfNextLn& nl = q.n;
+#else
+__global__ __launch_bounds__(512, 2) void ff_fused8_kernel(FfArgs p) {
+#endif
+  constexpr int KS = C / 32, NK1 = C / 64, NJ2 = C / 16, NJH = NJ2 / 2, NCH = C / 16;
+  constexpr int W1_BYTES = 128 * 128, W2_BYTES = C * 128;
+  constexpr int W2_PASSES = C / 64;
+  constexpr int W2_PER_KT = (W2_PASSES + NK1 - 1) / NK1;
+  static_assert(NJ2 % 2 == 0, "output blocks split over the two waves of a row group");
+
+  extern __shared__ __attribute__((aligned(16))) char smem[];
+  constexpr int W1_RING = 3;
+  char* const lds_w1 = smem;
+  char* const lds_w2 = smem + W1_RING * W1_BYTES;
+  float* const lds_b1 = (float*)(smem + W1_RING * W1_BYTES + 2 * W2_BYTES);
+  char* const lds_x = smem + W1_RING * W1_BYTES + 2 * W2_BYTES + 8 * C * 4;
+  const unsigned lds_base_u32 = __builtin_amdgcn_readfirstlane(lds_addr_u32(smem));
+
+  const int lane = threadIdx.x & 63;
+  const int wave = __builtin_amdgcn_readfirstlane(threadIdx.x >> 6);
+  const int mr = wave & 3, h = wave >> 2;
+  const int fr = lane & 15, fg = lane >> 4;
+  const int sr = lane >> 3, sp = lane & 7;
+
+  const int tm = xcd_remap(blockIdx.x, p.tiles_m);
+  const int64_t m0 = (int64_t)tm * 128 + mr * 32;
+
+  half8_t areg[2][KS];
+  if (p.ln_x) {
+#pragma unroll
+    for (int i = 0; i < 2; ++i) {
+      int64_t m = m0 + 16 * i + fr;
+      if (m >= p.M) m = p.M - 1;
+      const float* xr = p.ln_x + m * p.ldx + 8 * fg;
+      f32x4 v[KS][2];
+#pragma unroll
+      for (int ks = 0; ks < KS; ++ks) {
+        v[ks][0] = first_read(*(const f32x4*)(xr + 32 * ks));
+        v[ks][1] = first_read(*(const f32x4*)(xr + 32 * ks + 4));
+      }
+      float sum = 0.f;
+#pragma unroll
+      for (int ks = 0; ks < KS; ++ks)
+#pragma unroll
+        for (int e = 0; e < 2; ++e) sum += v[ks][e][0] + v[ks][e][1] + v[ks][e][2] + v[ks][e][3];
+      sum += __shfl_xor(sum, 16, 64);
+      asm volatile("" : "+v"(sum));
+      sum += __shfl_xor(sum, 32, 64);
+      asm volatile("" : "+v"(sum));
+      const float mean = sum / (float)C;
+      float ss = 0.f;
+#pragma unroll
+      for (int ks = 0; ks < KS; ++ks)
+#pragma unroll
+        for (int e = 0; e < 2; ++e)
+#pragma unroll
+          for (int r = 0; r < 4; ++r) {
+            const float dlt = v[ks][e][r] - mean;
+            ss += dlt * dlt;
+          }
+      ss += __shfl_xor(ss, 16, 64);
+      asm volatile("" : "+v"(ss));
+      ss += __shfl_xor(ss, 32, 64);
+      asm volatile("" : "+v"(ss));
+      const float rstd = rsqrtf(ss / (float)C + p.ln_eps);
+#pragma unroll
+      for (int ks = 0; ks < KS; ++ks) {
+        half_t y[8];
+#pragma unroll
+        for (int e = 0; e < 2; ++e) {
+          const f32x4 g4 = first_read(*(const f32x4*)(p.ln_gamma + 32 * ks + 8 * fg + 4 * e));
+          const f32x4 b4 = first_read(*(const f32x4*)(p.ln_beta + 32 * ks + 8 * fg + 4 * e));
+#pragma unroll
+          for (int r = 0; r < 4; ++r) y[4 * e + r] = (half_t)((v[ks][e][r] - mean) * rstd * g4[r] + b4[r]);
+        }
+        areg[i][ks] = half8_t{y[0], y[1], y[2], y[3], y[4], y[5], y[6], y[7]};
+      }
+    }
+  } else {
+#pragma unroll
+    for (int i = 0; i < 2; ++i) {
+      int64_t m = m0 + 16 * i + fr;
+      if (m >= p.M) m = p.M - 1;
+      const half_t* ap = p.a + m * p.lda + 8 * fg;
+#pragma unroll
+      for (int ks = 0; ks < KS; ++ks) areg[i][ks] = *(const half8_t*)(ap + 32 * ks);
+    }
+  }
+  f32x4 acc2[2][NJH];
+#pragma unroll
+  for (int i = 0; i < 2; ++i) {
+    int64_t m = m0 + 16 * i + fr;
+    if (m >= p.M) m = p.M - 1;
+#pragma unroll
+    for (int jj = 0; jj < NJH; ++jj)
+      acc2[i][jj] = p.residual ? *(const f32x4*)(p.residual + m * p.ldr + 16 * (h * NJH + jj) + 4 * fg) : f32x4{0.f, 0.f, 0.f, 0.f};
+  }
+  for (int i = threadIdx.x; i < 2 * C; i += 512) *(f32x4*)(lds_b1 + 4 * i) = *(const f32x4*)(p.b1 + 4 * i);
+#pragma unroll
+  for (int i = 0; i < 2; ++i) {
+#pragma unroll
+    for (int ks = 0; ks < KS; ++ks) asm volatile("" : "+v"(areg[i][ks]));
+#pragma unroll
+    for (int jj = 0; jj < NJH; ++jj) asm volatile("" : "+v"(acc2[i][jj]));
+  }
+
+  auto w1_key = [](int row) { return ((row >> 1) & 1) | (((row >> 3) & 3) << 1); };
+  const half_t* w1_src[2];
+#pragma unroll
+  for (int i = 0; i < 2; ++i) {
+    const int row = wave * 16 + 8 * i + sr;
+    w1_src[i] = p.w1 + (int64_t)row * C + (sp ^ w1_key(row)) * 8;
+  }
+  const half_t* w2_src[2];
+#pragma unroll
+  for (int i = 0; i < 2; ++i) {
+    const int row = wave * (C / 8) + 8 * i + sr;
+    w2_src[i] = p.w2 + (int64_t)row * (4 * C) + (sp ^ ((row >> 1) & 7)) * 8;
+  }
+  auto stage_w1 = [&](int buf, int hc, int kt) {
+    const unsigned dst = lds_base_u32 + buf * W1_BYTES + wave * 16 * 128;
+    const int64_t off = (int64_t)hc * 128 * C + kt * 64;
+#pragma unroll
+    for (int i = 0; i < 2; ++i) glds16_raw(w1_src[i] + off, dst + i * 1024);
+  };
+  auto stage_w2_part = [&](int buf, int hc, int part) {
+    const unsigned dst = lds_base_u32 + W1_RING * W1_BYTES + buf * W2_BYTES + wave * (C / 8) * 128;
+#pragma unroll
+    for (int u = 0; u < W2_PER_KT; ++u) {
+      const int i = part * W2_PER_KT + u;
+      if (i < W2_PASSES) glds16_raw(w2_src[i & 1] + (int64_t)(i >> 1) * 16 * (4 * C) + hc * 64, dst + i * 1024);
+    }
+  };
+
+  int w1_off[2], w2_off[2];
+#pragma unroll
+  for (int s = 0; s < 2; ++s) {
+    const int rb = 64 * h + 8 * (fr >> 2) + (fr & 3);
+    w1_off[s] = rb * 128 + (((4 * s + fg) ^ w1_key(rb)) << 4);
+    const int r2 = 16 * (h * NJH) + fr;
+    w2_off[s] = r2 * 128 + (((4 * s + fg) ^ ((r2 >> 1) & 7)) << 4);
+  }
+  char* const x_mine = lds_x + ((mr * 2 + h) * 2) * 1024 + lane * 16;
+  const char* const x_q0 = lds_x + (mr * 2 * 2) * 1024 + lane * 16;
+
+  constexpr int NTILES = NCH * NK1;
+  auto stage_w1_seq = [&](int g) { stage_w1(g % W1_RING, g / NK1, g % NK1); };
+  auto wait_all_but = [&](int n) {
+    if (n >= 3) wait_vm<3>();
+    else if (n == 2) wait_vm<2>();
+    else if (n == 1) wait_vm<1>();
+    else wait_vm<0>();
+  };
+  __syncthreads();
+  stage_w1_seq(0);
+#pragma unroll
+  for (int part = 0; part < NK1; ++part) stage_w2_part(0, 0, part);
+  if (NTILES > 1) stage_w1_seq(1);
+  if (NTILES > 1) wait_vm<2>();
+  else wait_vm<0>();
+  lds_barrier();
+
+  int g = 0;
+  for (int hc = 0; hc < NCH; ++hc) {
+    f32x4 acc1[2][4];
+#pragma unroll
+    for (int e = 0; e < 2; ++e) {
+      const float* bp = lds_b1 + hc * 128 + 64 * h + 8 * fg + 4 * e;
+      acc1[0][e] = acc1[1][e] = *(const f32x4*)bp;
+      acc1[0][2 + e] = acc1[1][2 + e] = *(const f32x4*)(bp + 32);
+    }
+#pragma unroll
+    for (int kt = 0; kt < NK1; ++kt) {
+      int issued = 0;
+      if (g + 2 < NTILES) {
+        stage_w1_seq(g + 2);
+        issued += 2;
+      }
+      if (hc + 1 < NCH && kt * W2_PER_KT < W2_PASSES) {
+        stage_w2_part((hc + 1) & 1, hc + 1, kt);
+        issued += (kt + 1) * W2_PER_KT <= W2_PASSES ? W2_PER_KT : W2_PASSES - kt * W2_PER_KT;
+      }
+      const char* const tb = lds_w1 + (g % W1_RING) * W1_BYTES;
+      half8_t bfr[2][4];
+#pragma unroll
+      for (int s = 0; s < 2; ++s)
+#pragma unroll
+        for (int j = 0; j < 4; ++j) bfr[s][j] = *(const half8_t*)(tb + w1_off[s] + (32 * (j >> 1) + 4 * (j & 1)) * 128);
+#pragma unroll
+      for (int s = 0; s < 2; ++s)
+#pragma unroll
+        for (int i = 0; i < 2; ++i)
+#pragma unroll
+          for (int j = 0; j < 4; ++j)
+            acc1[i][j] = __builtin_amdgcn_mfma_f32_16x16x32_f16(bfr[s][j], areg[i][2 * kt + s], acc1[i][j], 0, 0, 0);
+      wait_all_but(issued);
+      lds_barrier();
+      ++g;
+    }
+#pragma unroll
+    for (int i = 0; i < 2; ++i) {
+      const f32x4 o0 = geglu4(acc1[i][0], acc1[i][2]);
+      const f32x4 o1 = geglu4(acc1[i][1], acc1[i][3]);
+      *(half8_t*)(x_mine + i * 1024) = half8_t{(half_t)o0[0], (half_t)o0[1], (half_t)o0[2], (half_t)o0[3],
+                                               (half_t)o1[0], (half_t)o1[1], (half_t)o1[2], (half_t)o1[3]};
+    }
+    lds_barrier();
+    half8_t hq[2][2];
+#pragma unroll
+    for (int q = 0; q < 2; ++q)
+#pragma unroll
+      for (int i = 0; i < 2; ++i) hq[q][i] = *(const half8_t*)(x_q0 + (q * 2 + i) * 1024);
+    const char* const t2 = lds_w2 + (hc & 1) * W2_BYTES;
+#pragma unroll
+    for (int jj = 0; jj < NJH; ++jj) {
+      const half8_t w0 = *(const half8_t*)(t2 + w2_off[0] + jj * (16 * 128));
+      const half8_t w1f = *(const half8_t*)(t2 + w2_off[1] + jj * (16 * 128));
+#pragma unroll
+      for (int i = 0; i < 2; ++i) {
+        acc2[i][jj] = __builtin_amdgcn_mfma_f32_16x16x32_f16(w0, hq[0][i], acc2[i][jj], 0, 0, 0);
+        acc2[i][jj] = __builtin_amdgcn_mfma_f32_16x16x32_f16(w1f, hq[1][i], acc2[i][jj], 0, 0, 0);
+      }
+    }
+    lds_barrier();
+  }
+
+#if !FF8_NEXT_LN
+#pragma unroll
+  for (int i = 0; i < 2; ++i) {
+    const int64_t m = m0 + 16 * i + fr;
+    const bool ok = m < p.M;
+#pragma unroll
+    for (int jj = 0; jj < NJH; ++jj) {
+      const int f = 16 * (h * NJH + jj) + 4 * fg;
+      const f32x4 v = acc2[i][jj] + first_read(*(const f32x4*)(p.b2 + f));
+      if (!ok) continue;
+      if (p.out_f32) *(f32x4*)(p.out_f32 + m * p.ldo32 + f) = v;
+      if (p.out_f16) *(half4_t*)(p.out_f16 + m * p.ldo16 + f) = to_f16x4(v);
+    }
+  }
+#else
+  constexpr int NV = C / 64, LP = C + 4;
+  static_assert(C % 64 == 0 && 64 * LP * 4 <= 3 * 128 * 128 + 2 * C * 128, "a 64-row pass fits in the W1 ring + W2 buffers");
+  float* const lds_t = (float*)smem;
+  const int sub = lane & 15;
+  int c_rt = C;
+  asm("" : "+s"(c_rt));
+  f32x4 gm[NV], bt[NV];
+#pragma unroll
+  for (int k = 0; k < NV; ++k) {
+    gm[k] = first_read(*(const f32x4*)(nl.gamma + 64 * k + 4 * sub));
+    bt[k] = first_read(*(const f32x4*)(nl.beta + 64 * k + 4 * sub));
+  }
+#pragma unroll
+  for (int i = 0; i < 2; ++i) {
+    const int64_t m = m0 + 16 * i + fr;
+    const bool ok = m < p.M;
+    float* const trow = lds_t + (16 * mr + fr) * LP;
+#pragma unroll
+    for (int jj = 0; jj < NJH; ++jj) {
+      const int f = 16 * (h * NJH + jj) + 4 * fg;
+      const f32x4 v = acc2[i][jj] + first_read(*(const f32x4*)(p.b2 + f));
+      *(f32x4*)(trow + f) = v;
+      if (!ok) continue;
+      if (p.out_f32) *(f32x4*)(p.out_f32 + m * p.ldo32 + f) = v;
+      if (p.out_f16) *(half4_t*)(p.out_f16 + m * p.ldo16 + f) = to_f16x4(v);
+    }
+    lds_barrier();
+#pragma clang loop unroll(disable)
+    for (int rr = 0; rr < 2; ++rr) {
+      const int lr = (int)(threadIdx.x >> 4) + 32 * rr;
+      const int64_t row = (int64_t)tm * 128 + 32 * (lr >> 4) + 16 * i + (lr & 15);
+      f32x4 x[NV];
+#pragma unroll
+      for (int k = 0; k < NV; ++k) x[k] = first_read(*(const f32x4*)(lds_t + lr * LP + 64 * k + 4 * sub));
+      float mean, rstd;
+      ln_row_stats<NV>(x, sub, C / 4, c_rt, nl.eps, mean, rstd);
+      if (row < p.M) {
+        half_t* const orow = nl.out + row * nl.ldo;
+#pragma unroll
+        for (int k = 0; k < NV; ++k) *(half4_t*)(orow + 64 * k + 4 * sub) = ln_quad_f16(x[k], mean, rstd, gm[k], bt[k]);
+      }
+    }
+    if (i == 0) lds_barrier();
+  }
+#endif
+}
diff --git a/stable-virtual-camera_amd/csrc/ln_row.h b/stable-virtual-camera_amd/csrc/ln_row.h
--- /dev/null
+++ b/stable-virtual-camera_amd/csrc/ln_row.h
@@ -0,0 +1,51 @@
+#pragma once
+
+#include "seva_common.h"
+
+__device__ __forceinline__ float group16_sum(float v) {
+#pragma unroll
+  for (int o = 8; o > 0; o >>= 1) v += __shfl_xor(v, o, 64);
+  return v;
+}
+
+__device__ __forceinline__ float ln_centred(float x, float mean) {
+  float d = x - mean;
+  asm("" : "+v"(d));
+  return d;
+}
+
+template <int NV>
+__device__ __forceinline__ void ln_row_stats(const f32x4 (&v)[NV], int sub, int cq, int c, float eps, float& mean, float& rstd) {
+  float s = 0.f;
+#pragma unroll
+  for (int k = 0; k < NV; ++k)
+    if (sub + 16 * k < cq) s += v[k][0] + v[k][1] + v[k][2] + v[k][3];
+  mean = group16_sum(s) / (float)c;
+  float ss = 0.f;
+#pragma unroll
+  for (int k = 0; k < NV; ++k)
+    if (sub + 16 * k < cq) {
+#pragma unroll
+      for (int r = 0; r < 4; ++r) {
+        const float d = ln_centred(v[k][r], mean);
+        ss = __builtin_fmaf(d, d, ss);
+      }
+    }
+  rstd = rsqrtf(group16_sum(ss) / (float)c + eps);
+}
+
+__device__ __forceinline__ float ln_value(float x, float mean, float rstd, float g, float b) { return __builtin_fmaf(ln_centred(x, mean) * rstd, g, b); }
+
+__device__ __forceinline__ half4_t ln_quad_f16(f32x4 x, float mean, float rstd, f32x4 g4, f32x4 b4) {
+  float t[4];
+#pragma unroll
+  for (int r = 0; r < 4; ++r) t[r] = ln_centred(x[r], mean) * rstd;
+  unsigned p[2];
+#pragma unroll
+  for (int e = 0; e < 2; ++e) {
+    asm("v_fma_mixlo_f16 %0, %1, %2, %3" : "=v"(p[e]) : "v"(g4[2 * e]), "v"(t[2 * e]), "v"(b4[2 * e]));
+    asm("v_fma_mixhi_f16 %0, %1, %2, %3" : "+v"(p[e]) : "v"(g4[2 * e + 1]), "v"(t[2 * e + 1]), "v"(b4[2 * e + 1]));
+  }
+  typedef unsigned u32x2 __attribute__((ext_vector_type(2)));
+  return __builtin_bit_cast(half4_t, u32x2{p[0], p[1]});
+}
diff --git a/stable-virtual-camera_amd/csrc/norm.hip b/stable-virtual-camera_amd/csrc/norm.hip
--- a/stable-virtual-camera_amd/csrc/norm.hip
+++ b/stable-virtual-camera_amd/csrc/norm.hip
@@ -1,4 +1,5 @@
 #include "seva_common.h"
+#include "ln_row.h"
 
 #include <stdlib.h>
 
@@ -290,12 +291,6 @@
 
 constexpr int LN_MAXV = 20;
 
-__device__ __forceinline__ float group16_sum(float v) {
-#pragma unroll
-  for (int o = 8; o > 0; o >>= 1) v += __shfl_xor(v, o, 64);
-  return v;
-}
-
 template <int NV, int LN_ROWS, int OUT = 0, bool SPLIT = false>
 __global__ __launch_bounds__(256) void layernorm_kernel(const float* __restrict__ x,
                                                         const float* __restrict__ gamma,
@@ -330,22 +325,8 @@
   for (int it = 0; it < LN_ROWS; ++it) {
     const int64_t row = base + 16 * it;
     if (it + 1 < LN_ROWS) load_row(row + 16, nxt);
-    float s = 0.f;
-#pragma unroll
-    for (int k = 0; k < NV; ++k)
-      if (sub + 16 * k < cq) s += v[k][0] + v[k][1] + v[k][2] + v[k][3];
-    const float mean = group16_sum(s) / (float)c;
-    float ss = 0.f;
-#pragma unroll
-    for (int k = 0; k < NV; ++k)
-      if (sub + 16 * k < cq) {
-#pragma unroll
-        for (int r = 0; r < 4; ++r) {
-          const float d = v[k][r] - mean;
-          ss += d * d;
-        }
-      }
-    const float rstd = rsqrtf(group16_sum(ss) / (float)c + eps);
+    float mean, rstd;
+    ln_row_stats<NV>(v, sub, cq, c, eps, mean, rstd);
     if (row < rows) {
       half_t* orow = out + row * ld_out;
 #pragma unroll
@@ -357,19 +338,21 @@
           if constexpr (OUT != 0) {
             float y[4];
 #pragma unroll
-            for (int r = 0; r < 4; ++r) y[r] = (v[k][r] - mean) * rstd * g4[r] + b4[r];
+            for (int r = 0; r < 4; ++r) y[r] = ln_value(v[k][r], mean, rstd, g4[r], b4[r]);
             if constexpr (OUT == 1) *(int*)((uint8_t*)out + row * ld_out + i * 4) = pack_fp8x4(y[0], y[1], y[2], y[3]);
             else *(f32x4*)((float*)out + row * ld_out + i * 4) = f32x4{y[0], y[1], y[2], y[3]};
-          } else {
+          } else if constexpr (SPLIT) {
             half4_t h, l;
 #pragma unroll
             for (int r = 0; r < 4; ++r) {
-              const float y = (v[k][r] - mean) * rstd * g4[r] + b4[r];
+              const float y = ln_value(v[k][r], mean, rstd, g4[r], b4[r]);
               h[r] = (half_t)y;
-              if constexpr (SPLIT) l[r] = (half_t)(y - (float)h[r]);
+              l[r] = (half_t)(y - (float)h[r]);
             }
             *(half4_t*)(orow + i * 4) = h;
-            if constexpr (SPLIT) *(half4_t*)(orow + c + i * 4) = l;
+            *(half4_t*)(orow + c + i * 4) = l;
+          } else {
+            *(half4_t*)(orow + i * 4) = ln_quad_f16(v[k], mean, rstd, g4, b4);
           }
         }
       }
diff --git a/stable-virtual-camera_amd/seva/_engine.py b/stable-virtual-camera_amd/seva/_engine.py
--- a/stable-virtual-camera_amd/seva/_engine.py
+++ b/stable-virtual-camera_amd/seva/_engine.py
@@ -159,6 +159,7 @@
         self.pv8 = self.attention == "fp8"
         self.fp8_pad = env_flag("SEVA_FP8_PAD", "is1")
         self.ff_fused = env_flag("SEVA_FF_FUSED", "not0", True)
+        self.ff_next_ln = env_flag("SEVA_FF_NEXT_LN", "is1")
         self.ff = self._fp8_option("ff", ff, "SEVA_FP8_FF")
         self.ff8 = self.ff == "fp8"
         self.conv_splitk = env_flag("SEVA_CONV_SPLITK", "not0", True)
@@ -372,8 +373,27 @@
         step = self.slice_frames * unit
         return step if step < rows else rows
 
-    def _ff(self, x32, ln_pfx, ff_pfx, rows, c, *, residual, out_f32=None, out_f16=None, unit=1):
+    def _ff_plain_fused(self, ff_pfx: str, c: int, out_f16) -> bool:
         W = self.W
+        if ff_pfx + ".w1f8" in W or ff_pfx + ".w18" in W:
+            return False
+        if "ff" in self.split or (out_f16 is not None and "proj_out" in self.split):
+            return False
+        return self.ff_fused and c in ops.FF_FUSED_CHANNELS
+
+    def _takes_plain_ln(self, at_pfx: str, rows: int, c: int, hw: int, regime: str) -> bool:
+        if "qkv" in self.split or at_pfx + ".qkv8" in self.W:
+            return False
+        return not (regime == "frame" and self.slice_attn and self._slice_rows(rows, c, hw) < rows)
+
+    def _emits_next_ln(self, ff_pfx: str, at_pfx: str, rows: int, c: int, hw: int, regime: str, out_f16=None) -> bool:
+        return (self.ff_next_ln and getattr(ops, "FF_NEXT_LN", False) and self._ff_plain_fused(ff_pfx, c, out_f16)
+                and self._takes_plain_ln(at_pfx, rows, c, hw, regime))
+
+    def _ff(self, x32, ln_pfx, ff_pfx, rows, c, *, residual, out_f32=None, out_f16=None, unit=1, next_ln=None):
+        W = self.W
+        if next_ln is not None and not self._ff_plain_fused(ff_pfx, c, out_f16):
+            raise SevaNativeError(f"{ff_pfx}: only the fused f16 feed-forward writes the next LayerNorm")
         if ff_pfx + ".w1f8" in W:
             ops.ff_fused_fp8(None, W[ff_pfx + ".w1f8"], W[ff_pfx + ".w1f8e"], W[ff_pfx + ".b1"], W[ff_pfx + ".w2f8"],
                              W[ff_pfx + ".w2f8e"], W[ff_pfx + ".b2"], residual=residual, out_f32=out_f32, out_f16=out_f16,
@@ -399,9 +419,10 @@
                                                        out_f32=out_f32, out_f16=out_f16, alg_k=4 * c if sp_ff else 0)
             return
         if self.ff_fused and c in ops.FF_FUSED_CHANNELS:
+            more = {} if next_ln is None else {"next_ln": (W[next_ln[0] + ".g"], W[next_ln[0] + ".b"], next_ln[1])}
             ops.ff_fused(None, W[ff_pfx + ".w1"], W[ff_pfx + ".b1"], W[ff_pfx + ".w2"], W[ff_pfx + ".b2"],
                          residual=residual, out_f32=out_f32, out_f16=out_f16,
-                         ln_x=x32, ln_gamma=W[ln_pfx + ".g"], ln_beta=W[ln_pfx + ".b"], ln_eps=1e-5)
+                         ln_x=x32, ln_gamma=W[ln_pfx + ".g"], ln_beta=W[ln_pfx + ".b"], ln_eps=1e-5, **more)
             return
         step = self._slice_rows(rows, c, unit)
         a_buf = self._buf("ln16", (step, c), F16)
@@ -471,10 +492,12 @@
         return out
 
     def _self_attention(self, x32, ln_pfx, at_pfx, rows, c, heads, *, regime, n, hw, T, residual,
-                        row_add, rpg, ldra, out_f32):
+                        row_add, rpg, ldra, out_f32, a=None):
         W = self.W
         c3 = 3 * c
         sp_qkv = "qkv" in self.split
+        if a is not None and not self._takes_plain_ln(at_pfx, rows, c, hw, regime):
+            raise SevaNativeError(f"{at_pfx}: this self-attention does not take a plain f16 LayerNorm operand")
         if sp_qkv and regime == "frame" and self.slice_attn and self._slice_rows(rows, c, hw) < rows:
             raise SevaNativeError("the split-precision QKV projection does not run frame-sliced (SEVA_SLICE_ATTN)")
         if regime == "frame" and self.slice_attn and self._slice_rows(rows, c, hw) < rows:
@@ -500,7 +523,8 @@
             a8 = self._ln(x32, ln_pfx, rows, c, fp8=True)
             ops.gemm(a8, W[at_pfx + ".qkv8"], w_exp=W[at_pfx + ".qkv8e"], out_f16=qkv, col_scale=QK_SCALE_LOG2E, col_scale_n=c)
         else:
-            a = self._ln(x32, ln_pfx, rows, c, split=sp_qkv)
+            if a is None:
+                a = self._ln(x32, ln_pfx, rows, c, split=sp_qkv)
             ops.gemm(a, W[at_pfx + ".qkv"], out_f16=qkv, col_scale=QK_SCALE_LOG2E, col_scale_n=c, alg_k=c if sp_qkv else 0)
         att = self._buf("att", (rows, c), F16)
         q, k, v = qkv[:, :c], qkv[:, c:2 * c], qkv[:, 2 * c:]
@@ -558,21 +582,22 @@
         collapse = lc == 1
         ldra_frame, ldra_scene = self.ctx_total, T * self.ctx_total
         last16 = None
+        regime = "joint" if spec.joint else "frame"
+        cur_ln = None
         for i in range(spec.depth):
             b = f"{pfx}.transformer_blocks.{i}"
             m = f"{pfx}.time_mix_blocks.{i}"
-            regime = "joint" if spec.joint else "frame"
             audit_mark(b)
             h1 = self._buf("t_h1", (rows, c), F32)
             if collapse:
                 ra = ctxvec[:, self.ctx_off[b + ".attn2"]:]
                 rpg, ldra = (T * hw, ldra_scene) if spec.joint else (hw, ldra_frame)
                 self._self_attention(cur, b + ".norm1", b + ".attn1", rows, c, heads, regime=regime, n=n,
-                                     hw=hw, T=T, residual=cur, row_add=ra, rpg=rpg, ldra=ldra, out_f32=h1)
+                                     hw=hw, T=T, residual=cur, row_add=ra, rpg=rpg, ldra=ldra, out_f32=h1, a=cur_ln)
             else:
                 h0 = self._buf("t_h0", (rows, c), F32)
                 self._self_attention(cur, b + ".norm1", b + ".attn1", rows, c, heads, regime=regime, n=n,
-                                     hw=hw, T=T, residual=cur, row_add=None, rpg=0, ldra=0, out_f32=h0)
+                                     hw=hw, T=T, residual=cur, row_add=None, rpg=0, ldra=0, out_f32=h0, a=cur_ln)
                 if spec.joint:
                     self._cross_attention_general(
                         h0, b + ".norm2", b + ".attn2", rows, c, heads, ctx16, lc, nb0=n // T, nb1=1,
@@ -586,16 +611,18 @@
             self._ff(h1, b + ".norm3", b + ".ff", rows, c, residual=h1, out_f32=h2, unit=hw)
             audit_mark(m)
             m1 = self._buf("t_m1", (rows, c), F32)
-            self._ff(h2, m + ".norm_in", m + ".ff_in", rows, c, residual=h2, out_f32=m1, unit=hw)
+            m1_ln = self._buf("ln16n", (rows, c), F16) if self._emits_next_ln(m + ".ff_in", m + ".attn1", rows, c, hw, "temporal") else None
+            self._ff(h2, m + ".norm_in", m + ".ff_in", rows, c, residual=h2, out_f32=m1, unit=hw,
+                     next_ln=None if m1_ln is None else (m + ".norm1", m1_ln))
             m2 = self._buf("t_m2", (rows, c), F32)
             if collapse:
                 ra = ctxvec[:, self.ctx_off[m + ".attn2"]:]
                 self._self_attention(m1, m + ".norm1", m + ".attn1", rows, c, heads, regime="temporal", n=n,
-                                     hw=hw, T=T, residual=m1, row_add=ra, rpg=T * hw, ldra=ldra_scene, out_f32=m2)
+                                     hw=hw, T=T, residual=m1, row_add=ra, rpg=T * hw, ldra=ldra_scene, out_f32=m2, a=m1_ln)
             else:
                 m0 = self._buf("t_m0", (rows, c), F32)
                 self._self_attention(m1, m + ".norm1", m + ".attn1", rows, c, heads, regime="temporal", n=n,
-                                     hw=hw, T=T, residual=m1, row_add=None, rpg=0, ldra=0, out_f32=m0)
+                                     hw=hw, T=T, residual=m1, row_add=None, rpg=0, ldra=0, out_f32=m0, a=m1_ln)
                 self._cross_attention_general(
                     m0, m + ".norm2", m + ".attn2", rows, c, heads, ctx16, lc, nb0=n // T, nb1=hw, lq=T,
                     q_strides=(T * hw * c, c, hw * c), o_strides=(T * hw * c, c, hw * c),
@@ -603,7 +630,12 @@
             final = i == spec.depth - 1
             nxt = None if final else self._buf("t_h", (rows, c), F32)
             last16 = self._buf("t_h16", (rows, 2 * c if sp_out else c), F16)
-            self._ff(m2, m + ".norm3", m + ".ff", rows, c, residual=h2, out_f32=nxt, out_f16=last16, unit=hw)
+            b_nxt = f"{pfx}.transformer_blocks.{i + 1}"
+            cur_ln = None
+            if not final and self._emits_next_ln(m + ".ff", b_nxt + ".attn1", rows, c, hw, regime, out_f16=last16):
+                cur_ln = self._buf("ln16n", (rows, c), F16)
+            self._ff(m2, m + ".norm3", m + ".ff", rows, c, residual=h2, out_f32=nxt, out_f16=last16, unit=hw,
+                     next_ln=None if cur_ln is None else (b_nxt + ".norm1", cur_ln))
             cur = nxt
         audit_mark(pfx)
         out = self._buf("out:" + pfx, (n, hw, c), F32)
diff --git a/stable-virtual-camera_amd/seva/_native.py b/stable-virtual-camera_amd/seva/_native.py
--- a/stable-virtual-camera_amd/seva/_native.py
+++ b/stable-virtual-camera_amd/seva/_native.py
@@ -47,6 +47,10 @@
     ]
 
 
+class FfNextLn(C.Structure):
+    _fields_ = [("gamma", c_void_p), ("beta", c_void_p), ("out_f16", c_void_p), ("ldo", c_int64), ("eps", c_float)]
+
+
 class AttnDesc(C.Structure):
     _fields_ = [
         ("q", c_void_p), ("k", c_void_p), ("v", c_void_p), ("out", c_void_p),
@@ -115,6 +119,7 @@
     "seva_gemm_f16_split_out": (c_int, [POINTER(GemmDesc), c_void_p]),
     "seva_gemm_fp8": (c_int, [POINTER(GemmDesc), c_void_p]),
     "seva_ff_fused_f16": (c_int, [POINTER(FfDesc), c_void_p]),
+    "seva_ff_fused_f16_ln": (c_int, [POINTER(FfDesc), POINTER(FfNextLn), c_void_p]),
     "seva_ff_fused_fp8": (c_int, [POINTER(FfDesc), c_void_p]),
     "seva_attention_f16": (c_int, [POINTER(AttnDesc), c_void_p]),
     "seva_attn_v_fp8_size": (c_int, [c_int32, c_int32, c_int32, POINTER(c_int64), POINTER(c_int64)]),
diff --git a/stable-virtual-camera_amd/seva/ops.py b/stable-virtual-camera_amd/seva/ops.py
--- a/stable-virtual-camera_amd/seva/ops.py
+++ b/stable-virtual-camera_amd/seva/ops.py
@@ -73,6 +73,8 @@
         return
     for name in AUDITED[op]:
         t = a.get(name)
+        if isinstance(t, tuple):
+            t = t[-1]
         if t is not None:
             for label, off, rows, cols, pitch in _audit_views(op, name, t, a):
                 _AUDIT.output(op, label, t, off, rows, cols, pitch)
@@ -334,6 +336,7 @@
 
 
 FF_FUSED_CHANNELS = (64, 128, 256, 320)
+FF_NEXT_LN = True
 
 
 def _ff_desc(a, w1, b1, w2, b2, M, c, residual, out_f32, out_f16, ln_x, ln_gamma, ln_beta, ln_eps, w1_exp=None, w2_exp=None) -> nv.FfDesc:
@@ -350,11 +353,12 @@
     return d
 
 
-@_audited("out_f32", "out_f16")
+@_audited("out_f32", "out_f16", "next_ln")
 def ff_fused(a: torch.Tensor | None, w1: torch.Tensor, b1: torch.Tensor, w2: torch.Tensor, b2: torch.Tensor, *,
              residual: torch.Tensor | None = None, out_f32: torch.Tensor | None = None,
              out_f16: torch.Tensor | None = None, ln_x: torch.Tensor | None = None,
-             ln_gamma: torch.Tensor | None = None, ln_beta: torch.Tensor | None = None, ln_eps: float = 1e-5) -> None:
+             ln_gamma: torch.Tensor | None = None, ln_beta: torch.Tensor | None = None, ln_eps: float = 1e-5,
+             next_ln: tuple | None = None, next_ln_eps: float = 1e-5) -> None:
     src = ln_x if ln_x is not None else a
     require_cuda(src, w1, w2)
     M, c = src.shape
@@ -362,7 +366,16 @@
     assert w1.dtype == F16 and w2.dtype == F16 and w1.shape == (8 * c, c) and w2.shape == (c, 4 * c)
     assert w1.is_contiguous() and w2.is_contiguous() and c in FF_FUSED_CHANNELS
     d = _ff_desc(a, w1, b1, w2, b2, M, c, residual, out_f32, out_f16, ln_x, ln_gamma, ln_beta, ln_eps)
-    check(_lib().seva_ff_fused_f16(C.byref(d), stream_ptr(src.device)), "seva_ff_fused_f16")
+    if next_ln is None:
+        check(_lib().seva_ff_fused_f16(C.byref(d), stream_ptr(src.device)), "seva_ff_fused_f16")
+        return
+    g, b, o = next_ln
+    require_cuda(o)
+    assert g.dtype == F32 and b.dtype == F32 and g.numel() == c and b.numel() == c
+    assert o.dtype == F16 and o.dim() == 2 and o.shape[0] == M and o.shape[1] >= c and o.stride(1) == 1
+    n = nv.FfNextLn()
+    n.gamma, n.beta, n.out_f16, n.ldo, n.eps = g.data_ptr(), b.data_ptr(), o.data_ptr(), o.stride(0), next_ln_eps
+    check(_lib().seva_ff_fused_f16_ln(C.byref(d), C.byref(n), stream_ptr(src.device)), "seva_ff_fused_f16_ln")
 
 
 FF8_STEP = 128
```

Result: no change. 11.03 denoising steps/s (median of 3 runs) (-0.1%).
